# nirschl-lab/stain2stain

Hardware: AMD Instinct MI355X
Metric: paired 256x256 stain tiles/sec (full CFM optimisation step) (higher is better)
Workload: dtype bf16

## Files before the change

include/stain2stain_hip.h:

```cpp
#ifndef STAIN2STAIN_HIP_H
#define STAIN2STAIN_HIP_H

#ifdef __cplusplus
extern "C" {
#endif

#define S2S_OK 0
#define S2S_ERR_SHAPE (-1)
#define S2S_ERR_ALIGN (-2)
#define S2S_ERR_DTYPE (-3)
#define S2S_ERR_LAUNCH (-4)
#define S2S_ERR_NULL (-5)

#define S2S_BF16 0
#define S2S_F32 1

int s2s_conv3x3_stat_blocks(int dtype, int B, int H, int W, int Cout);
int s2s_conv3x3_nhwc(int dtype, const void* x0, int ld0, int c0, const void* x1, int ld1, int c1,
                     const void* w_packed, const float* bias, void* y, int ldy, float* stat_part,
                     const float* ep_scale, const float* ep_shift, int relu, int B, int H, int W, int Cout,
                     void* stream);

int s2s_conv3x3_ksplit(int dtype, int B, int H, int W, int Cout, int cin);
int s2s_conv3x3_nhwc_k(int dtype, const void* x0, int ld0, int c0, const void* x1, int ld1, int c1,
                       const void* w_packed, const float* bias, void* y, int ldy, float* stat_part,
                       const float* ep_scale, const float* ep_shift, int relu, float* kwork, int B, int H, int W,
                       int Cout, void* stream);
int s2s_conv3x3_stat_rows(int dtype, int B, int H, int W, int Cout, int c0, int c1, int ld0, int ld1, int has_bias);
int s2s_conv3x3_staged(int dtype, int B, int H, int W, int Cout, int c0, int c1, int ld0, int ld1, int ldy, int stats);
int s2s_conv3x3_family(int dtype, int B, int H, int W, int Cout, int c0, int c1, int ld0, int ld1, int ldy, int has_bias,
                       int has_affine, int stats, int stat_rows, int kwork);
int s2s_conv3x3_plan(int dtype, int B, int H, int W, int Cout, int c0, int c1, int ld0, int ld1, int ldy, int has_bias,
                     int has_affine, int stats, int stat_rows, int kwork, int* out);
int s2s_conv3x3_nhwc_s(int dtype, const void* x0, int ld0, int c0, const void* x1, int ld1, int c1, const void* w_packed,
                       const float* bias, void* y, int ldy, float* stat_part, int stat_rows, const float* ep_scale,
                       const float* ep_shift, int relu, float* kwork, int B, int H, int W, int Cout, void* stream);
int s2s_debug_conv_clock(long* out_host, int n);

int s2s_conv3x3_wgrad_splits(int dtype, int B, int H, int W, int Cin, int Cout);
int s2s_conv3x3_wgrad_plan(int dtype, int B, int H, int W, int Cin, int Cout, int what);
int s2s_conv3x3_wgrad_nhwc(int dtype, const void* dy, int lddy, int Cout, const void* x0, int ld0, int c0,
                           const void* x1, int ld1, int c1, float* part, float* grad_oihw, int accumulate,
                           int B, int H, int W, void* stream);
int s2s_conv3x3_wgrad_phase(int dtype, const void* dy, int lddy, int Cout, const void* x0, int ld0, int c0,
                            const void* x1, int ld1, int c1, float* part, float* grad_oihw, int accumulate,
                            int B, int H, int W, int phases, void* stream);
int s2s_conv3x3_wgrad_phase_variant(int dtype, const void* dy, int lddy, int Cout, const void* x0, int ld0, int c0,
                                    const void* x1, int ld1, int c1, float* part, float* grad_oihw, int accumulate,
                                    int B, int H, int W, int phases, int variant, void* stream);

int s2s_stem_stat_blocks(int B, int H, int W);
int s2s_stem_conv3x3_fwd(int dtype, const float* x_nchw, const float* w_oihw, const float* bias, void* y, int ldy,
                         float* stat_part, int B, int H, int W, int Cin, int Cout, void* stream);
int s2s_stem_wgrad_blocks(int B, int H, int W);
int s2s_stem_conv3x3_wgrad(int dtype, const void* dy, int lddy, const float* x_nchw, float* part, float* dw_oihw,
                           float* dbias, int accumulate, int B, int H, int W, int Cin, int Cout, void* stream);
int s2s_stem_conv3x3_wgrad_ref(int dtype, const void* dy, int lddy, const float* x_nchw, float* part, float* dw_oihw,
                               float* dbias, int accumulate, int B, int H, int W, int Cin, int Cout, void* stream);
int s2s_stem_wgrad_family(int dtype, int lddy, int B, int H, int W, int Cin, int Cout, int reference);
int s2s_head_family(int dtype, int B, int H, int W, int C, int Cout, int forward);
int s2s_head_conv1x1_fwd(int dtype, const void* x, int ldx, const float* w, const float* bias, float* y_nchw, int B,
                         int H, int W, int C, int Cout, void* stream);
int s2s_head_wgrad_blocks(int B, int H, int W);
int s2s_head_conv1x1_bwd(int dtype, const float* dy_nchw, const void* x, int ldx, const float* w, void* dx, int lddx,
                         float* part, float* dw, float* dbias, int accumulate, int B, int H, int W, int C, int Cout,
                         void* stream);

int s2s_head_loss_blocks(int B, int H, int W);
int s2s_head_loss_family(int dtype, int B, int H, int W, int C, int Cout);
int s2s_head_loss_fused(int dtype, const void* x, int ldx, const float* w, const float* bias, const float* u_nchw,
                        float* v_nchw, void* dx, int lddx, float grad_scale, float* part, double* lpart, float* dw,
                        float* dbias, float* loss, int accumulate, int B, int H, int W, int C, int Cout, void* stream);

int s2s_tail_blocks(int B, int H, int W);
int s2s_tail_family(int dtype, int B, int H, int W, int C, int Cout);
int s2s_tail_fwd_loss(int dtype, const void* raw, int ldx, const float* scale, const float* shift, const float* mean,
                      const float* invstd, const float* w, const float* bias, const float* u_nchw, float* v_nchw,
                      float* g_nchw, float grad_scale, float* part, double* lpart, float* bnwork, float* dw,
                      float* dbias, float* loss, float* dgamma, float* dbeta, float* conv_dbias, int accumulate, int B,
                      int H, int W, int C, int Cout, void* stream);
int s2s_tail_bwd_apply(int dtype, const void* raw, int ldx, const float* g_nchw, const float* w, const float* scale,
                       const float* shift, const float* mean, const float* invstd, const float* gamma,
                       const float* bnwork, void* dx, int lddx, int B, int H, int W, int C, int Cout, void* stream);

int s2s_bn_finalize(const float* part, int nblk, int C, long count, const float* gamma, const float* beta,
                    float* running_mean, float* running_var, long* num_batches_tracked, float momentum, float eps,
                    float* mean, float* invstd, float* scale, float* shift, void* stream);
int s2s_bn_finalize_b(const float* part, int nblk, int C, long count, const float* gamma, const float* beta,
                      float* running_mean, float* running_var, long* num_batches_tracked, float momentum, float eps,
                      float* mean, float* invstd, float* scale, float* shift, const float* conv_bias, void* stream);
int s2s_bn_eval_prepare(int C, const float* gamma, const float* beta, const float* running_mean,
                        const float* running_var, float eps, float* scale, float* shift, void* stream);
int s2s_bn_relu_apply(int dtype, const void* x, int ldx, const float* scale, const float* shift, void* y, int ldy,
                      void* pool, int ldp, int B, int H, int W, int C, void* stream);
int s2s_maxpool2(int dtype, const void* x, int ldx, void* pool, int ldp, int B, int H, int W, int C, void* stream);
int s2s_bn_bwd_blocks(int B, int H, int W, int C);
int s2s_bn_relu_bwd(int dtype, const void* g1, int ldg1, const void* gp, int ldgp, const float* scale,
                    const float* shift, const void* x, int ldx, const float* mean, const float* invstd, const float* gamma, float* dgamma,
                    float* dbeta, float* dbias_conv, int accumulate, void* dx, int lddx, float* work, int B, int H,
                    int W, int C, void* stream);
int s2s_bn_partial_sums(const float* part, int nblk, int C, float* sums, void* stream);
int s2s_bn_relu_bwd_phase(int dtype, const void* g1, int ldg1, const void* gp, int ldgp, const float* scale,
                          const float* shift, const void* x, int ldx, const float* mean, const float* invstd,
                          const float* gamma, float* dgamma, float* dbeta, float* dbias_conv, int accumulate, void* dx,
                          int lddx, float* work, int B, int H, int W, int C, long count_total, int phases, void* stream);

int s2s_upsample2x_bilinear_ac_fwd(int dtype, const void* x, int ldx, const float* bias_nc, void* y, int ldy, int B,
                                   int Hin, int Win, int Hout, int Wout, int C, void* stream);
int s2s_upsample2x_bn_relu_fwd(int dtype, const void* x, int ldx, const float* scale, const float* shift,
                               const float* bias_nc, void* y, int ldy, int B, int Hin, int Win, int Hout, int Wout, int C,
                               void* stream);
int s2s_upsample2x_bilinear_ac_fwd_ref(int dtype, const void* x, int ldx, const float* bias_nc, void* y, int ldy, int B,
                                       int Hin, int Win, int Hout, int Wout, int C, void* stream);
int s2s_upsample2x_fwd_family(int ldx, int ldy, int B, int Hin, int Win, int Hout, int Wout, int C, int reference);
int s2s_upsample2x_bilinear_ac_bwd(int dtype, const void* dy, int lddy, void* dx, int lddx, int B, int Hin, int Win,
                                   int Hout, int Wout, int C, void* stream);
int s2s_upsample2x_bilinear_ac_bwd_ref(int dtype, const void* dy, int lddy, void* dx, int lddx, int B, int Hin,
                                       int Win, int Hout, int Wout, int C, void* stream);
int s2s_upsample2x_bwd_family(int lddy, int lddx, int B, int Hin, int Win, int Hout, int Wout, int C, int reference);
int s2s_pixel_sum(int dtype, const void* x, int ldx, float* out_nc, int B, int HW, int C, int accumulate,
                  void* stream);

int s2s_time_embedding(const float* t, float* out, int B, int dim, void* stream);
int s2s_linear_fwd(const float* x, const float* w, const float* bias, float* y, int B, int K, int N, void* stream);
int s2s_linear_bwd(const float* dy, const float* x, const float* w, float* dx, float* dw, float* db, int accumulate,
                   int B, int K, int N, void* stream);
int s2s_silu_fwd(const float* h, float* a, int n, void* stream);
int s2s_silu_bwd(const float* h, const float* da, float* dh, int n, void* stream);
int s2s_cfm_sample(const float* x0, const float* x1, const float* t, const float* eps, float sigma, float* xt,
                   float* ut, int B, long per_sample, void* stream);
int s2s_mse_loss(const float* v, const float* u, float* dv, float grad_scale, float* loss, double* work, long count,
                 void* stream);
int s2s_ode_error_norm(const float* e, const float* y0, const float* y1, float atol, float rtol, float* out,
                       double* work, long n, void* stream);
int s2s_axpy(float* x, const float* y, float a, long n, void* stream);
int s2s_dp_partials(long n);
int s2s_dp_init(int phase, const float* y, const float* k1, const float* fa, double* state, double* part, float* out,
                float* t_out, int* status, float atol, float rtol, int B, long n, void* stream);
int s2s_dp_stage(int i, const float* y, const float* k1, const float* k2, const float* k3, const float* k4,
                 const float* k5, const float* k6, const double* state, float* out, float* t_out, int B, long n,
                 void* stream);
int s2s_dp_error(const float* k1, const float* k2, const float* k3, const float* k4, const float* k5, const float* k6,
                 const float* k7, const float* y, const float* y_new, const double* state, double* part, float atol,
                 float rtol, int B, long n, void* stream);
int s2s_dp_control(double* state, const double* part, int* status, int max_steps, int B, long n, void* stream);
int s2s_dp_commit(float* y, const float* y_new, float* k1, const float* k7, const double* state, int B, long n,
                  void* stream);
int s2s_rk_stage(const float* x, const float* k1, const float* k2, const float* k3, float c1, float c2, float c3, int nk,
                 float* out, float* t_out, const float* table, const int* counter, int stages, int stage, int table_len,
                 int B, long n, void* stream);
int s2s_rk_combine(float* x, const float* k1, const float* k2, const float* k3, const float* k4, float c1, float c2,
                   float c3, float c4, int nk, int* counter, int B, long n, void* stream);
int s2s_fill_f32(float* x, float v, long n, void* stream);
int s2s_euler_tick(float* t, int n, const float* table, int* counter, void* stream);

int s2s_adam_step(float* p, const float* g, float* m, float* v, long n, int step, float lr, float beta1, float beta2,
                  float eps, float weight_decay, float grad_scale, void* stream);
int s2s_adam_step_dev(float* p, const float* g, float* m, float* v, long n, const float* hyper, void* stream);
long s2s_adam_multi_blocks(long n);
int s2s_adam_multi(const void* desc, int ntensors, long total, int step, float lr, float beta1, float beta2, float eps,
                   float weight_decay, float grad_scale, void* stream);
int s2s_adam_ema_step(float* p, const float* g, float* m, float* v, float* ema, long n, int step, float lr, float beta1,
                      float beta2, float eps, float weight_decay, float grad_scale, float ema_weight, void* stream);
int s2s_adam_ema_step_dev(float* p, const float* g, float* m, float* v, float* ema, long n, const float* hyper,
                          const float* ema_weight, void* stream);
long s2s_ema_multi_blocks(long n);
int s2s_ema_multi(const void* desc, int ntensors, long total, const float* weight, void* stream);
long s2s_pack_conv3x3_fwd_elems(int Cout, int Cin);
long s2s_pack_conv3x3_dgrad_elems(int Cout, int Cin);
int s2s_pack_conv3x3(int dtype, const float* w_oihw, void* w_fwd, void* w_dgrad, int Cout, int Cin, void* stream);
int s2s_pack_conv3x3_batched(int dtype, const void* desc, int nlayers, long total, void* stream);
int s2s_nchw_to_nhwc(int dtype, const float* x_nchw, void* y, int ldy, int B, int C, int H, int W, void* stream);
int s2s_nhwc_to_nchw(int dtype, const void* x, int ldx, float* y_nchw, int accumulate, int B, int C, int H, int W,
                     void* stream);

int s2s_paired_crop_flip_normalize(const void* src_u8, const void* tgt_u8, const int* params, float* out_src,
                                   float* out_tgt, int B, int Hs, int Ws, int S, void* stream);
int s2s_pil_resize_bilinear_normalize(const void* src_u8, void* tmp_u8, const int* bounds_h, const int* kk_h,
                                      int ksize_h, const int* bounds_v, const int* kk_v, int ksize_v, void* out_u8,
                                      float* out_f, int B, int Hs, int Ws, int Ho, int Wo, void* stream);

int s2s_region_gather(const void* img_u8, long pitch, int H, int W, int band_top, int band_h, const int* origins,
                      float* out, int B, int T, void* stream);
int s2s_region_blend(const float* tiles, int c0, const float* tiles1, int c1, const int* origins, int n, int T,
                     int overlap, float* acc, int band_rows, int H, int W, int r0, int r1, void* stream);
int s2s_region_finalize(float* acc, int band_rows, int W, int C, int r0, int r1, void* out_u8, long pitch_u8,
                        float* out_f, long pitch_f, int out_top, void* stream);

// ... 318 lines not shown
```

stain2stain_amd/csrc/conv3x3_mfma.hip:

```cpp
#include "common.h"
#include <stdlib.h>
#include <type_traits>
#include <utility>

#ifdef S2S_ABLATE
#define S2S_ABL(cond) (cond)
#define S2S_DBG_MASK (~0)
#else
#define S2S_ABL(cond) false
#define S2S_DBG_MASK 64
#endif

struct Conv3x3Args {
  const void* x0;
  const void* x1;
  const void* w;
  const float* bias;
  void* y;
  float* stat_part;
  const float* ep_scale;
  const float* ep_shift;
  int ld0, c0, ld1, c1, ldy;
  int B, H, W, Cout, tilesY, tilesX, nchunk;
  int relu;
  int act;
  float act_slope;
  void* y2;
  int ldy2;
  float* kpart;
  int ksplit;
  int lgc;
  int lgh, lgw;
  int bias_mod;
  int xsp, xsn;
  long stat_rows;
  long stat_rows_req;
  int dbg;
};

namespace {

template <int... Is, typename F>
__device__ __forceinline__ void static_for_impl(std::integer_sequence<int, Is...>, F&& f) {
  (f(std::integral_constant<int, Is>{}), ...);
}
template <int N, typename F>
__device__ __forceinline__ void static_for(F&& f) {
  static_for_impl(std::make_integer_sequence<int, N>{}, f);
}

constexpr int ROWB = 80;
constexpr int STEM_HALO_BYTES = 3 * 18 * 18 * 4;

template <typename T> struct Piece;
template <> struct Piece<float> {
  f32x4 a, b;
  __device__ __forceinline__ void zero() {
#pragma unroll
    for (int i = 0; i < 4; ++i) { a[i] = 0.f; b[i] = 0.f; }
  }
  __device__ __forceinline__ void load(const float* p) {
    a = *reinterpret_cast<const f32x4*>(p);
    b = *reinterpret_cast<const f32x4*>(p + 4);
  }
  __device__ __forceinline__ void to_lds(char* hi, int img_stride, int off) const {
    bf16x8 h, m, l;
#pragma unroll
    for (int i = 0; i < 8; ++i) {
      const float x = i < 4 ? a[i] : b[i - 4];
      h[i] = (bf16_t)x;
      const float r1 = x - (float)h[i];
      m[i] = (bf16_t)r1;
      l[i] = (bf16_t)(r1 - (float)m[i]);
    }
    *reinterpret_cast<bf16x8*>(hi + off) = h;
    *reinterpret_cast<bf16x8*>(hi + img_stride + off) = m;
    *reinterpret_cast<bf16x8*>(hi + 2 * img_stride + off) = l;
  }
};

template <typename T, int TH, int TW, int BN, int WM, int WN, int LDS_MAIN>
__device__ __forceinline__ void conv_epilogue(const Conv3x3Args& a, f32x16 (&acc)[(TH * TW / WM) / 32][(BN / WN) / 32],
                                              char* smem, int img, int y0, int x0p, int n0) {
  constexpr bool SPLIT = std::is_same<T, float>::value;
  constexpr int BM = TH * TW, WTM = BM / WM, WTN = BN / WN, MI = WTM / 32, NI = WTN / 32;
  T* __restrict__ yout = static_cast<T*>(a.y);
  const int tid = threadIdx.x, lane = tid & 63, wave = tid >> 6;
  const int wm = wave / WN, wn = wave % WN;
  const int r = lane & 31, h = lane >> 5;
  constexpr int RS = BN * (int)sizeof(T) + (SPLIT ? 16 : 64);
  constexpr int EP = (BM * RS + WM * 2 * BN * 4 <= LDS_MAIN) ? 1 : ((BM / 2) * RS + WM * 2 * BN * 4 <= LDS_MAIN ? 2 : 4);
  static_assert(WM % EP == 0 || EP == 1, "epilogue passes split the wave rows");
  constexpr int PM = BM / EP;
  char* const otile = smem;
  float* const red = reinterpret_cast<float*>(smem + PM * RS);
  const bool want_stats = a.stat_part != nullptr;
  float s1[NI], s2[NI];
#pragma unroll
  for (int ni = 0; ni < NI; ++ni) { s1[ni] = 0.f; s2[ni] = 0.f; }
#pragma unroll
  for (int ep = 0; ep < EP; ++ep) {
    if (ep > 0) __syncthreads();
    if (wm / (WM / EP) == ep || EP == 1) {
#pragma unroll
      for (int ni = 0; ni < NI; ++ni) {
        const int nl = wn * WTN + ni * 32 + r;
        const int n = n0 + nl;
        const bool nok = n < a.Cout;
        const float bias = (nok && a.bias) ? a.bias[n % a.bias_mod] : 0.f;
        const float esc = (nok && a.ep_scale) ? a.ep_scale[n] : 1.f;
        const float esh = (nok && a.ep_shift) ? a.ep_shift[n] : 0.f;
#pragma unroll
        for (int mi = 0; mi < MI; ++mi) {
          float v[16];
#pragma unroll
          for (int j = 0; j < 16; ++j) {
            const int row = (j & 3) + 8 * (j >> 2) + 4 * h;
            const int m = wm * WTM + mi * 32 + row;
            const int py = m / TW, px = m - py * TW;
// ... 434 lines not shown
  constexpr int BM = TH * TW, WTM = BM / WM, WTN = BN / WN, MI = WTM / 16, NI = WTN / 16;
  static_assert(NI % 2 == 0, "channel blocks are exchanged in pairs");
  T* __restrict__ yout = static_cast<T*>(a.y);
  const int lane = tid & 63, wave = tid >> 6;
  const int wm = wave / WN, wn = wave % WN;
  const int cl = lane & 15, q = lane >> 4;
  float esc[NI][4], esh[NI][4];
#pragma unroll
  for (int ni = 0; ni < NI; ++ni)
#pragma unroll
    for (int j = 0; j < 4; ++j) {
      const int n = n0 + wn * WTN + ni * 16 + 4 * q + j;
      const bool nok = n < a.Cout;
      esc[ni][j] = (AFFINE && nok) ? a.ep_scale[n] : 1.f;
      esh[ni][j] = (AFFINE && nok) ? a.ep_shift[n] : 0.f;
    }
  const int nlane = n0 + wn * WTN + (q & 1) * 16 + (q >> 1) * 8;
  float s1l[STATS ? NI / 2 : 1][8], s2l[STATS ? NI / 2 : 1][8];
  float (*const s1)[8] = CARRY ? cs1 : s1l;
  float (*const s2)[8] = CARRY ? cs2 : s2l;
  if constexpr (STATS && !CARRY) {
#pragma unroll
    for (int pr = 0; pr < NI / 2; ++pr)
#pragma unroll
      for (int k = 0; k < 8; ++k) { s1[pr][k] = 0.f; s2[pr][k] = 0.f; }
  }
#pragma unroll
  for (int mi = 0; mi < MI; ++mi) {
    const int m = wm * WTM + mi * 16 + cl;
    const int py = m / TW, px = m - py * TW;
    const int gy = y0 + py, gx = x0p + px;
    const bool pok = gy < a.H && gx < a.W;
    const long opix = ((long)img * om.OH + gy * om.os + om.oy) * om.OW + gx * om.os + om.ox;
#pragma unroll
    for (int ni = 0; ni < NI; ni += 2) {
      unsigned w[2][2];
#pragma unroll
      for (int b = 0; b < 2; ++b) {
        bf16x4 pk;
#pragma unroll
        for (int j = 0; j < 4; ++j) {
          float t = acc[mi][ni + b][j] + bias[ni + b][j];
          if (AFFINE) {
            t = t * esc[ni + b][j] + esh[ni + b][j];
            if (a.relu) t = fmaxf(t, 0.f);
          } else if (a.act) {
            t = t > 0.f ? t : a.act_slope * t;
          }
          pk[j] = (bf16_t)t;
        }
        const uint2 u = __builtin_bit_cast(uint2, pk);
        w[b][0] = u.x; w[b][1] = u.y;
      }
      const auto r0 = __builtin_amdgcn_permlane16_swap(w[0][0], w[1][0], false, false);
      const auto r1 = __builtin_amdgcn_permlane16_swap(w[0][1], w[1][1], false, false);
      const uint4 out = make_uint4(r0[0], r1[0], r0[1], r1[1]);
      const int n = nlane + ni * 16;
      if constexpr (STATS) {
        if (pok && n < a.Cout) {
          const bf16x8 val = __builtin_bit_cast(bf16x8, out);
#pragma unroll
          for (int k = 0; k < 8; ++k) {
            const float t = (float)val[k];
            s1[ni / 2][k] += t;
            s2[ni / 2][k] = fmaf(t, t, s2[ni / 2][k]);
          }
        }
      }
      if (pok && n < a.Cout) {
        if (!S2S_ABL(a.dbg & 8)) *reinterpret_cast<uint4*>(yout + opix * a.ldy + n) = out;
        if (a.y2) {
          const bf16x8 val = __builtin_bit_cast(bf16x8, out);
          bf16x8 r8;
#pragma unroll
          for (int k = 0; k < 8; ++k) r8[k] = (float)val[k] > 0.f ? val[k] : (bf16_t)0.f;
          *reinterpret_cast<bf16x8*>(static_cast<T*>(a.y2) + opix * a.ldy2 + n) = r8;
        }
      }
    }
  }
  if constexpr (STATS && !CARRY) conv_stats_flush<BN, WN>(a, s1, s2, n0, tid, stat_row);
}

__device__ long g_clk[8192 * 4];
template <int TH, int TW, int BN, int WM, int WN, int NS>
__global__ __launch_bounds__(256, 2) void conv3x3_dma16_kernel(Conv3x3Args a) {
  long c0_ = 0, w0_ = 0;
  if ((a.dbg & 64) && threadIdx.x == 0) { c0_ = __builtin_readcyclecounter(); w0_ = wall_clock64(); }
  using T = bf16_t;
  constexpr int HP = TW + 4, HH_ = TH + 2, ROWS = HH_ * HP;
  constexpr int NGA = (ROWS + 15) / 16, HG = (NGA + 3) / 4;
  constexpr int A_BYTES = HG * 4 * 1024;
  constexpr int BG = BN / 64;
  constexpr int B_BYTES = BN * 64;
  constexpr int BM = TH * TW, WTM = BM / WM, WTN = BN / WN, MI = WTM / 16, NI = WTN / 16;
  constexpr int RB = TW / 16;
  static_assert(WM * WN == 4 && BN % 64 == 0 && NS >= 3 && NS <= 8 && TW % 16 == 0 && WTM % TW == 0, "configuration");

  extern __shared__ __attribute__((aligned(16))) char smem[];
  char* const ldsA = smem;
  char* const ldsB = smem + 2 * A_BYTES;

  const T* __restrict__ x0 = static_cast<const T*>(a.x0);
  const T* __restrict__ x1 = static_cast<const T*>(a.x1);
  const char* __restrict__ wp = static_cast<const char*>(a.w);

  const int tid = threadIdx.x, lane = tid & 63;
  const int wave = __builtin_amdgcn_readfirstlane(tid >> 6);
  const int wm = wave / WN, wn = wave % WN;
  const int cl = lane & 15, kp = lane >> 4;

  int bt = blockIdx.x, by = blockIdx.y;
  if (a.xsp) {
    const unsigned L = blockIdx.x + gridDim.x * blockIdx.y;
    const unsigned xcd = L & 7, k = L >> 3;
    const unsigned xp = xcd % (unsigned)a.xsp, xn = xcd / (unsigned)a.xsp;
    const unsigned P = gridDim.x / (unsigned)a.xsp, Nn = gridDim.y / (unsigned)a.xsn;
    const unsigned kp_ = k / Nn, kn_ = k - kp_ * Nn;
    bt = (int)(xp * P + kp_); by = (int)(xn * Nn + kn_);
  }
  const int tile_id = bt;
  const int tx = bt % a.tilesX; bt /= a.tilesX;
  const int ty = bt % a.tilesY;
  const int img = bt / a.tilesY;
  const int y0 = ty * TH, x0p = tx * TW;
  const int n0 = by * BN;
  const int ctot = a.c0 + a.c1;
  const int c_lo = (int)(((long)blockIdx.z * a.nchunk) / gridDim.z), c_hi = (int)(((long)(blockIdx.z + 1) * a.nchunk) / gridDim.z);

  const int drow = lane >> 2, dslot = lane & 3;
  auto akey = [](int col) { return ((col >> 2) & 1) << 1; };
  int apix[HG], apc[HG];
#pragma unroll
  for (int j = 0; j < HG; ++j) {
    const int row = (wave + 4 * j) * 16 + drow;
    const int hy = row / HP, hx = row - hy * HP;
    const int gy = y0 - 1 + hy, gx = x0p - 1 + hx;
    apix[j] = (row < ROWS && hx < TW + 2 && gy >= 0 && gy < a.H && gx >= 0 && gx < a.W)
                  ? (img * a.H + gy) * a.W + gx : -1;
    apc[j] = (dslot ^ akey(hx)) * 8;
  }
  const char* wptr[BG];
  int wstep[BG];
#pragma unroll
  for (int j = 0; j < BG; ++j) {
    const int n = (wave + 4 * j) * 16 + drow;
    const bool ok = n0 + n < a.Cout;
    wptr[j] = ok ? wp + (long)c_lo * 9 * a.Cout * 64 + ((long)(n0 + n) * 32 + ((dslot ^ ((-(n >> 2)) & 3)) * 8)) * 2 : g_zero_page;
    wstep[j] = ok ? a.Cout * 64 : 0;
  }
  auto dma_halo = [&](int c) {
    char* dst = ldsA + (c & 1) * A_BYTES + wave * 1024;
#pragma unroll
    for (int j = 0; j < HG; ++j) {
      const int ch = c * 32 + apc[j];
      const void* g = g_zero_page;
      if (apix[j] >= 0) {
        if (ch < a.c0) g = x0 + (long)apix[j] * a.ld0 + ch;
        else if (ch < ctot) g = x1 + (long)apix[j] * a.ld1 + (ch - a.c0);
      }
      dma16(g, dst + j * 4096);
    }
  };
  auto dma_w = [&](int slot) {
    char* dst = ldsB + slot * B_BYTES + wave * 1024;
#pragma unroll
    for (int j = 0; j < BG; ++j) {
      dma16(wptr[j], dst + j * 4096);
      wptr[j] += wstep[j];
    }
  };

  int aofs[RB][3];
#pragma unroll
  for (int rb = 0; rb < RB; ++rb)
#pragma unroll
    for (int kw = 0; kw < 3; ++kw) {
      const int px = rb * 16 + cl + kw;
      aofs[rb][kw] = ((wm * (WTM / TW)) * HP + px) * 64 + ((kp ^ akey(px)) << 4);
    }
  const int nrow = wn * WTN + cl;
  const int bofs = nrow * 64 + ((kp ^ ((-(nrow >> 2)) & 3)) << 4);

  f32x4 acc[MI][NI];
#pragma unroll
  for (int mi = 0; mi < MI; ++mi)
#pragma unroll
    for (int ni = 0; ni < NI; ++ni)
#pragma unroll
      for (int j = 0; j < 4; ++j) acc[mi][ni][j] = 0.f;

  auto compute = [&](auto tapc, const char* Ab, const char* Bb) {
    constexpr int tap = decltype(tapc)::value;
    constexpr int kh = tap / 3, kw = tap % 3;
    bf16x8 af[MI], bfr[NI];
#pragma unroll
    for (int mi = 0; mi < MI; ++mi)
      af[mi] = *reinterpret_cast<const bf16x8*>(Ab + aofs[mi % RB][kw] + (kh + mi / RB) * HP * 64);
#pragma unroll
    for (int ni = 0; ni < NI; ++ni) bfr[ni] = *reinterpret_cast<const bf16x8*>(Bb + bofs + ni * 1024);
#pragma unroll
    for (int mi = 0; mi < MI; ++mi)
#pragma unroll
      for (int ni = 0; ni < NI; ++ni)
        acc[mi][ni] = __builtin_amdgcn_mfma_f32_16x16x32_bf16(bfr[ni], af[mi], acc[mi][ni], 0, 0, 0);
  };
  dma_halo(c_lo);
  static_for<NS - 1>([&](auto k) { dma_w(decltype(k)::value); });
  wait_vm<0>();
  __builtin_amdgcn_s_barrier();

  int c = c_lo;
  for (; c + 1 < c_hi; ++c) {
    const char* Ab = ldsA + (c & 1) * A_BYTES;
    const int it0 = (c - c_lo) * 9;
    static_for<9>([&](auto tapc) {
      constexpr int tap = decltype(tapc)::value;
      if (tap == 0) { if (!S2S_ABL(a.dbg & 4)) dma_halo(c + 1); else { static_for<HG>([&](auto) { dma16(g_zero_page, ldsA + ((c + 1) & 1) * A_BYTES + wave * 1024); }); } }
      if (!S2S_ABL(a.dbg & 1)) dma_w((it0 + tap + NS - 1) % NS);
      else if (!S2S_ABL(a.dbg & 512)) { static_for<BG>([&](auto) { dma16(g_zero_page, ldsB + wave * 1024); }); }
      if (!S2S_ABL(a.dbg & 2)) compute(tapc, Ab, ldsB + ((it0 + tap) % NS) * B_BYTES);
      __builtin_amdgcn_sched_barrier(0);
      if (!S2S_ABL(a.dbg & 256)) wait_vm<(NS - 2) * BG + (tap <= NS - 3 ? HG : 0)>();
      if (!S2S_ABL(a.dbg & 32)) __builtin_amdgcn_s_barrier();
#ifdef S2S_ABLATE
      if ((a.dbg & 1024) && tap == 8) {
        char* nb = ldsA + ((c + 1) & 1) * A_BYTES;
        const float sc = 1.0f + a.act_slope, sh = a.act_slope, fl = a.act_slope - 3.0e38f;
#pragma unroll
        for (int j = 0; j < HG; ++j) {
          bf16x8* p8 = reinterpret_cast<bf16x8*>(nb + (tid + 256 * j) * 16);
          bf16x8 v = *p8;
#pragma unroll
          for (int k = 0; k < 8; ++k) v[k] = (bf16_t)fmaxf(fmaf((float)v[k], sc, sh), fl);
          *p8 = v;
        }
        asm volatile("s_waitcnt lgkmcnt(0)" ::: "memory");
        __builtin_amdgcn_s_barrier();
      }
#endif
    });
  }
  float biasr[NI][4];
#pragma unroll
  for (int ni = 0; ni < NI; ++ni)
#pragma unroll
    for (int j = 0; j < 4; ++j) {
      const int n = n0 + wn * WTN + ni * 16 + 4 * kp + j;
      biasr[ni][j] = (a.bias && n < a.Cout) ? a.bias[n] : 0.f;
    }
  {
    const char* Ab = ldsA + (c & 1) * A_BYTES;
    const int it0 = (c - c_lo) * 9;
    static_for<9>([&](auto tapc) {
      constexpr int tap = decltype(tapc)::value;
      if (tap + NS - 1 < 9) dma_w((it0 + tap + NS - 1) % NS);
      compute(tapc, Ab, ldsB + ((it0 + tap) % NS) * B_BYTES);
      __builtin_amdgcn_sched_barrier(0);
      constexpr int last_issued = (tap + NS - 1 < 9) ? tap + NS - 1 : 8;
      constexpr int younger = last_issued - (tap + 1) > 0 ? last_issued - (tap + 1) : 0;
      wait_vm<younger * BG>();
      __builtin_amdgcn_s_barrier();
    });
  }
  if (S2S_ABL(a.dbg & 16)) return;
  if (a.kpart) {
    float* const kpz = a.kpart + (long)blockIdx.z * ((long)a.B * a.H * a.W) * a.Cout;
#pragma unroll
    for (int mi = 0; mi < MI; ++mi) {
      const int m = wm * WTM + mi * 16 + cl;
      const int py = m / TW, px = m - py * TW;
      const int gy = y0 + py, gx = x0p + px;
      if (gy < a.H && gx < a.W) {
        float* const row = kpz + (((long)img * a.H + gy) * a.W + gx) * a.Cout;
#pragma unroll
        for (int ni = 0; ni < NI; ++ni) {
          const int n = n0 + wn * WTN + ni * 16 + 4 * kp;
          if (n < a.Cout) *reinterpret_cast<f32x4*>(row + n) = acc[mi][ni];
        }
      }
    }
    return;
  }
  const OutMap om{1, 0, 0, a.H, a.W};
  if (a.stat_part) conv_epilogue16_direct<TH, TW, BN, WM, WN, false, true>(a, acc, biasr, img, y0, x0p, n0, tid, om, (long)tile_id * WM + wm);
  else if (a.ep_scale) conv_epilogue16_direct<TH, TW, BN, WM, WN, true>(a, acc, biasr, img, y0, x0p, n0, tid, om);
  else conv_epilogue16_direct<TH, TW, BN, WM, WN, false>(a, acc, biasr, img, y0, x0p, n0, tid, om);
  if ((a.dbg & 64) && threadIdx.x == 0 && blockIdx.y == 0 && blockIdx.x < 8192) { g_clk[blockIdx.x * 4 + 0] = c0_; g_clk[blockIdx.x * 4 + 1] = __builtin_readcyclecounter(); g_clk[blockIdx.x * 4 + 2] = w0_; g_clk[blockIdx.x * 4 + 3] = wall_clock64(); }
}

template <int TH, int TW, int BN, int WM, int WN, int NS, int STATS>
__global__ __launch_bounds__(256, 2) void conv3x3_pers16_kernel(Conv3x3Args a, int ntiles, int GX, int GY) {
  using T = bf16_t;
  constexpr int HP = TW + 4, HH_ = TH + 2, ROWS = HH_ * HP;
  constexpr int NGA = (ROWS + 15) / 16, HG = (NGA + 3) / 4;
  constexpr int A_BYTES = HG * 4 * 1024;
  constexpr int BG = BN / 64;
  constexpr int B_BYTES = BN * 64;
  constexpr int BM = TH * TW, WTM = BM / WM, WTN = BN / WN, MI = WTM / 16, NI = WTN / 16;
  constexpr int RB = TW / 16;
  constexpr int NST = MI * (NI / 2) + (STATS == 1 ? (NI / 2) * 16 : 0);
  static_assert((NS - 2) * BG + HG + NST <= 63, "vmcnt is a 6-bit counter");
  static_assert(WM * WN == 4 && BN % 64 == 0 && NS == 4 && TW % 16 == 0 && WTM % TW == 0, "configuration");

  extern __shared__ __attribute__((aligned(16))) char smem[];
  char* const ldsA = smem;
  char* const ldsB = smem + 2 * A_BYTES;
  const T* __restrict__ x0 = static_cast<const T*>(a.x0);
  const T* __restrict__ x1 = static_cast<const T*>(a.x1);
  const char* __restrict__ wp = static_cast<const char*>(a.w);

  const int tid = threadIdx.x, lane = tid & 63;
  const int wave = __builtin_amdgcn_readfirstlane(tid >> 6);
  const int wm = wave / WN, wn = wave % WN;
  const int cl = lane & 15, kp = lane >> 4;
  const int ctot = a.c0 + a.c1;
  const int drow = lane >> 2, dslot = lane & 3;

  int ageo[HG];
#pragma unroll
  for (int j = 0; j < HG; ++j) {
    const int row = (wave + 4 * j) * 16 + drow;
    const int hy = row / HP, hx = row - hy * HP;
    ageo[j] = (((row < ROWS && hx < TW + 2) ? hy : 0x4000) << 16) | (hx << 8) | ((dslot ^ (((hx >> 2) & 1) << 1)) * 8);
  }
  int aofs[RB][3];
#pragma unroll
  for (int rb = 0; rb < RB; ++rb)
#pragma unroll
    for (int kw = 0; kw < 3; ++kw) {
      const int px = rb * 16 + cl + kw;
      aofs[rb][kw] = ((wm * (WTM / TW)) * HP + px) * 64 + ((kp ^ (((px >> 2) & 1) << 1)) << 4);
    }
  const int nrow = wn * WTN + cl;
  const int bofs = nrow * 64 + ((kp ^ ((-(nrow >> 2)) & 3)) << 4);
  int wrow_off[BG];
#pragma unroll
  for (int j = 0; j < BG; ++j) {
    const int n = (wave + 4 * j) * 16 + drow;
    wrow_off[j] = (n * 32 + ((dslot ^ ((-(n >> 2)) & 3)) * 8)) * 2;
  }

  struct Tile { int img, y0, x0p, n0, id; };
  auto locate = [&](int L) {
    int bt, by;
    if (a.xsp) {
      const unsigned xcd = (unsigned)L & 7u, k = (unsigned)L >> 3;
      const unsigned xp = xcd % (unsigned)a.xsp, xn = xcd / (unsigned)a.xsp;
// ... 71 lines not shown
  };

  const int G = gridDim.x;
  int L = blockIdx.x;
  Tile cur = locate(L);
  bool has_next = L + G < ntiles;
  Tile nxt = cur;
  if (has_next) nxt = locate(L + G);
  int apix_cur[HG];
  halo_pix(cur, true, apix_cur);
  wq_start(cur.n0, true);
  dma_halo(apix_cur, 0, 0);
  static_for<NS - 1>([&](auto k) { dma_w(decltype(k)::value); });
  wait_vm<0>();
  __builtin_amdgcn_s_barrier();

  int gc = 0;
  auto chunk = [&](auto firstc, int c) {
    constexpr bool FIRST = decltype(firstc)::value;
    const char* Ab = ldsA + (gc & 1) * A_BYTES;
    const int it0 = gc * 9;
    const bool last = c + 1 == a.nchunk;
    static_for<9>([&](auto tapc) {
      constexpr int tap = decltype(tapc)::value;
      if (tap == 0) {
        if (!last) dma_halo(apix_cur, c + 1, (gc + 1) & 1);
        else {
          int apix_nxt[HG];
          halo_pix(nxt, has_next, apix_nxt);
          dma_halo(apix_nxt, 0, (gc + 1) & 1);
        }
      }
      if (tap == 9 - (NS - 1) && last) wq_start(nxt.n0, has_next);
      dma_w((it0 + tap + NS - 1) % NS);
      compute(tapc, Ab, ldsB + ((it0 + tap) % NS) * B_BYTES);
      __builtin_amdgcn_sched_barrier(0);
      wait_vm<(NS - 2) * BG + (tap <= NS - 3 ? HG : 0) + ((FIRST && tap <= 1) ? NST : 0)>();
      __builtin_amdgcn_s_barrier();
    });
    ++gc;
  };
  float cs1[STATS == 2 ? NI / 2 : 1][8], cs2[STATS == 2 ? NI / 2 : 1][8];
  if constexpr (STATS == 2) {
#pragma unroll
    for (int pr = 0; pr < NI / 2; ++pr)
#pragma unroll
      for (int k = 0; k < 8; ++k) { cs1[pr][k] = 0.f; cs2[pr][k] = 0.f; }
  }
  for (;;) {
    __builtin_amdgcn_sched_barrier(0);
#pragma unroll
    for (int mi = 0; mi < MI; ++mi)
#pragma unroll
      for (int ni = 0; ni < NI; ++ni)
#pragma unroll
        for (int j = 0; j < 4; ++j) acc[mi][ni][j] = 0.f;
    __builtin_amdgcn_sched_barrier(0);
    chunk(std::true_type{}, 0);
    for (int c = 1; c < a.nchunk; ++c) chunk(std::false_type{}, c);
    {
      const OutMap om{1, 0, 0, a.H, a.W};
      const float nobias[NI][4] = {};
      if constexpr (STATS == 2)
        conv_epilogue16_direct<TH, TW, BN, WM, WN, false, true, true>(a, acc, nobias, cur.img, cur.y0, cur.x0p, cur.n0, tid, om, -1, cs1, cs2);
      else
        conv_epilogue16_direct<TH, TW, BN, WM, WN, false, STATS == 1>(a, acc, nobias, cur.img, cur.y0, cur.x0p, cur.n0, tid, om, (long)cur.id * WM + wm);
      if (!(cur.y0 + TH <= a.H && cur.x0p + TW <= a.W && cur.n0 + BN <= a.Cout)) wait_vm<0>();
    }
    if (!has_next) break;
    L += G;
    cur = nxt;
    halo_pix(cur, true, apix_cur);
    has_next = L + G < ntiles;
    if (has_next) nxt = locate(L + G);
  }
  if constexpr (STATS == 2) conv_stats_flush<BN, WN>(a, cs1, cs2, cur.n0, tid, (long)blockIdx.x * WM + wm);
}

struct TileCfg { int th, tw, bn, wm; bool pers; };
constexpr TileCfg kBf16Cfg[8] = {{8, 32, 128, 2, false}, {8, 32, 64, 4, true}, {4, 32, 128, 2, true}, {4, 32, 64, 2, true},
                                 {16, 16, 128, 2, false}, {16, 16, 64, 4, true}, {8, 16, 128, 2, true}, {8, 16, 64, 2, true}};
constexpr TileCfg kF32Cfg[2] = {{4, 32, 64, 2, false}, {8, 16, 64, 2, false}};
constexpr int kMinBlocks = 448;

inline long cfg_blocks(const TileCfg& c, int B, int H, int W, int Cout) {
  return (long)B * cdiv(H, c.th) * cdiv(W, c.tw) * cdiv(Cout, c.bn);
}

int select_cfg(int dtype, int B, int H, int W, int Cout) {
  if (dtype == S2S_F32) return W <= 16 ? 1 : 0;
  const int first = W <= 16 ? 4 : 0;
  int best = -1;
  long best_blocks = -1;
  for (int i = first; i < first + 4; ++i) {
    const TileCfg& c = kBf16Cfg[i];
    if (c.bn == 128 && (Cout <= 64 || (Cout % 128 != 0 && Cout % 128 <= 64 && Cout < 512))) continue;
    const long nb = cfg_blocks(c, B, H, W, Cout);
    if (nb >= kMinBlocks) return i;
    if (nb > best_blocks) { best_blocks = nb; best = i; }
  }
  return best;
}

enum Conv3x3Family {
  kStageResident,
  kStageStream,
  kPersCarry,
  kPers,
  kTap,
  kSplitF32,
};
struct Conv3x3Plan {
  int rc;
  int family;
  int cfg;
  int gx, gy;
  int grid;
  int xsp, xsn;
  int ksplit;
  long stat_rows;
};

template <int ID>
int launch_pers16(Conv3x3Args& a, const Conv3x3Plan& p, hipStream_t s) {
  constexpr TileCfg c = kBf16Cfg[ID];
  constexpr int TH = c.th, TW = c.tw, BN = c.bn, WM = c.wm, WN = 4 / WM, NS = 4;
  constexpr int ROWS = (TH + 2) * (TW + 4);
  constexpr int HG = ((ROWS + 15) / 16 + 3) / 4;
  constexpr int lds = 2 * HG * 4 * 1024 + NS * BN * 64;
  static_assert(lds <= 80 * 1024, "two workgroups per CU");
  a.tilesY = cdiv(a.H, TH);
  a.tilesX = cdiv(a.W, TW);
  auto kern_s = conv3x3_pers16_kernel<TH, TW, BN, WM, WN, NS, 1>;
  auto kern_c = conv3x3_pers16_kernel<TH, TW, BN, WM, WN, NS, 2>;
  auto kern_d = conv3x3_pers16_kernel<TH, TW, BN, WM, WN, NS, 0>;
  static unsigned long long attr_s = 0, attr_c = 0, attr_d = 0;
  if (int rc = s2s_allow_dyn_lds(reinterpret_cast<const void*>(kern_s), lds, &attr_s)) return rc;
  if (int rc = s2s_allow_dyn_lds(reinterpret_cast<const void*>(kern_c), lds, &attr_c)) return rc;
  if (int rc = s2s_allow_dyn_lds(reinterpret_cast<const void*>(kern_d), lds, &attr_d)) return rc;
  auto kern = p.family == kPersCarry ? kern_c : a.stat_part ? kern_s : kern_d;
  hipLaunchKernelGGL(kern, dim3(p.grid), dim3(256), lds, s, a, p.gx * p.gy, p.gx, p.gy);
  S2S_LAUNCH_CHECK();
  return S2S_OK;
}

template <int STATS, bool DEFER_EP, bool RESIDENT, bool AFFINE = false>
__global__ __launch_bounds__(512, 1) void conv3x3_stage_kernel(Conv3x3Args a, int njobs, int GX, int GY) {
  using T = bf16_t;
  constexpr int TH = 16, TW = 32, BN = 64, WM = 8, WN = 1;
  constexpr int HP = TW + 4, ROWS = (TH + 2) * HP;
  constexpr int NGA = (ROWS + 15) / 16, HG = (NGA + WM - 1) / WM;
  constexpr int A_BYTES = NGA * 1024;
  constexpr int B_BYTES = BN * 64, NGB = 9 * 4, BGW = (NGB + WM - 1) / WM;
  constexpr int STAGE = A_BYTES + 9 * B_BYTES;
  constexpr int WTM = TH * TW / WM, MI = WTM / 16, NI = BN / 16, RB = TW / 16;
  constexpr int NST = MI * (NI / 2);
  static_assert(NST <= 8, "one deferred store unit per tap");

  extern __shared__ __attribute__((aligned(16))) char smem[];
  const T* __restrict__ x0 = static_cast<const T*>(a.x0);
  const T* __restrict__ x1 = static_cast<const T*>(a.x1);
  const char* __restrict__ wp = static_cast<const char*>(a.w);

  const int tid = threadIdx.x, lane = tid & 63;
  const int wave = __builtin_amdgcn_readfirstlane(tid >> 6);
  const int wm = wave;
  const int cl = lane & 15, kp = lane >> 4;
  const int drow = lane >> 2, dslot = lane & 3;
  const int ctot = a.c0 + a.c1;

  int ageo[HG];
#pragma unroll
  for (int j = 0; j < HG; ++j) {
    const int row = (wave + WM * j) * 16 + drow;
    const int hy = row / HP, hx = row - hy * HP;
    ageo[j] = (((row < ROWS && hx < TW + 2) ? hy : 0x4000) << 16) | (hx << 8) | ((dslot ^ (((hx >> 2) & 1) << 1)) * 8);
  }
  int aofs[RB][3];
#pragma unroll
  for (int rb = 0; rb < RB; ++rb)
#pragma unroll
    for (int kw = 0; kw < 3; ++kw) {
      const int px = rb * 16 + cl + kw;
      aofs[rb][kw] = ((wm * (WTM / TW)) * HP + px) * 64 + ((kp ^ (((px >> 2) & 1) << 1)) << 4);
    }
  int bofs = cl * 64 + ((kp ^ ((-(cl >> 2)) & 3)) << 4);

  struct Tile { int img, y0, x0p, n0; };
  auto locate = [&](int L) {
    int bt, by;
    if (a.xsp) {
      const unsigned xcd = (unsigned)L & 7u, k = (unsigned)L >> 3, P = (unsigned)GX >> 3;
      if constexpr (RESIDENT) { by = (int)(k / P); bt = (int)(xcd * P + (k - (unsigned)by * P)); }
      else { const unsigned kq = k / (unsigned)GY; by = (int)(k - kq * (unsigned)GY); bt = (int)(xcd * P + kq); }
    } else if constexpr (RESIDENT) {
      by = L / GX; bt = L - by * GX;
    } else {
      bt = L / GY; by = L - bt * GY;
    }
    Tile t;
    const int tx = bt % a.tilesX; bt /= a.tilesX;
    const int ty = bt % a.tilesY;
    t.img = bt / a.tilesY;
    t.y0 = ty * TH; t.x0p = tx * TW; t.n0 = by * BN;
    return t;
  };
  constexpr unsigned OOB = 0xffffff00u;
  const __amdgpu_buffer_rsrc_t rs_w = __builtin_amdgcn_make_buffer_rsrc(const_cast<char*>(wp), 0, (int)((long)a.nchunk * 9 * a.Cout * 64), 0x00020000);
  const __amdgpu_buffer_rsrc_t rs_x0 = __builtin_amdgcn_make_buffer_rsrc(const_cast<T*>(x0), 0, (int)((((long)a.B * a.H * a.W - 1) * a.ld0 + a.c0) * 2), 0x00020000);
  const __amdgpu_buffer_rsrc_t rs_x1 = __builtin_amdgcn_make_buffer_rsrc(const_cast<T*>(a.c1 ? x1 : x0), 0, a.c1 ? (int)((((long)a.B * a.H * a.W - 1) * a.ld1 + a.c1) * 2) : 0, 0x00020000);
  const int wrow = (wave & 3) * 16 + drow;
  const unsigned wsw = (unsigned)wrow * 64u + (unsigned)((dslot ^ ((-(wrow >> 2)) & 3)) << 4);
  auto dma_weights = [&](int n0, int c, int st) {
    char* dst = smem + st * STAGE + A_BYTES + wave * 1024;
    const unsigned voff = n0 + wrow < a.Cout ? wsw : OOB;
#pragma unroll
    for (int j = 0; j < BGW; ++j) {
      if (wave + WM * j >= NGB || S2S_ABL(a.dbg & 1)) continue;
      const int tap = (wave >> 2) + (WM / 4) * j;
      __builtin_amdgcn_raw_ptr_buffer_load_lds(rs_w, (lds_void_t*)(dst + j * (WM * 1024)), 16, voff,
                                               ((c * 9 + tap) * a.Cout + n0) * 64, 0, 0);
    }
  };
  auto halo_pix = [&](const Tile& t, int (&apix)[HG]) {
#pragma unroll
    for (int j = 0; j < HG; ++j) {
      const int gy = t.y0 - 1 + (ageo[j] >> 16), gx = t.x0p - 1 + ((ageo[j] >> 8) & 0xff);
      apix[j] = (gy >= 0 && gy < a.H && gx >= 0 && gx < a.W) ? (t.img * a.H + gy) * a.W + gx : -1;
    }
  };
  auto dma_halo = [&](const int (&apix)[HG], int c, int st) {
    char* dst = smem + st * STAGE + wave * 1024;
    const bool second = c * 32 >= a.c0;
    const int ld2 = (second ? a.ld1 : a.ld0) * 2, ch0 = c * 32 - (second ? a.c0 : 0);
    const int left = ctot - c * 32;
#pragma unroll
    for (int j = 0; j < HG; ++j) {
      if (wave + WM * j >= NGA || S2S_ABL(a.dbg & 4)) continue;
      const int pc = ageo[j] & 0xff;
      const unsigned voff = (apix[j] >= 0 && pc < left) ? (unsigned)apix[j] * (unsigned)ld2 + (unsigned)(pc * 2) : OOB;
      if (second) __builtin_amdgcn_raw_ptr_buffer_load_lds(rs_x1, (lds_void_t*)(dst + j * (WM * 1024)), 16, voff, ch0 * 2, 0, 0);
      else __builtin_amdgcn_raw_ptr_buffer_load_lds(rs_x0, (lds_void_t*)(dst + j * (WM * 1024)), 16, voff, ch0 * 2, 0, 0);
    }
  };

  f32x4 acc[MI][NI];
  auto afrag = [&](auto tapc, int mi) {
    constexpr int tap = decltype(tapc)::value;
    constexpr int kh = tap / 3, kw = tap % 3;
    return *reinterpret_cast<const bf16x8*>(smem + aofs[mi % RB][kw] + (kh + mi / RB) * HP * 64);
  };
  auto bfrag = [&](auto tapc, int ni) {
    constexpr int tap = decltype(tapc)::value;
    return *reinterpret_cast<const bf16x8*>(smem + bofs + (A_BYTES + tap * B_BYTES + ni * 1024));
  };

  T* __restrict__ yout = static_cast<T*>(a.y);
  uint4 outv[MI][NI / 2];
  float cs1[STATS == 2 ? NI / 2 : 1][8], cs2[STATS == 2 ? NI / 2 : 1][8];
  auto stats_zero = [&]() {
    if constexpr (STATS == 2) {
#pragma unroll
      for (int pr = 0; pr < NI / 2; ++pr)
#pragma unroll
        for (int k = 0; k < 8; ++k) { cs1[pr][k] = 0.f; cs2[pr][k] = 0.f; }
    }
  };
  stats_zero();
  float esc[AFFINE ? NI : 1][4], esh[AFFINE ? NI : 1][4];
  auto load_affine = [&](int n0) {
    if constexpr (AFFINE) {
#pragma unroll
      for (int ni = 0; ni < NI; ++ni) {
        const int n = n0 + ni * 16 + 4 * kp;
        const bool ok = n < a.Cout;
        const f32x4 sc = ok ? *reinterpret_cast<const f32x4*>(a.ep_scale + n) : f32x4{1.f, 1.f, 1.f, 1.f};
        const f32x4 sh = ok ? *reinterpret_cast<const f32x4*>(a.ep_shift + n) : f32x4{0.f, 0.f, 0.f, 0.f};
        const f32x4 bi = (ok && a.bias) ? *reinterpret_cast<const f32x4*>(a.bias + n) : f32x4{0.f, 0.f, 0.f, 0.f};
#pragma unroll
        for (int j = 0; j < 4; ++j) { esc[ni][j] = sc[j]; esh[ni][j] = fmaf(bi[j], sc[j], sh[j]); }
      }
    }
  };
  auto pack = [&]() {
#pragma unroll
    for (int mi = 0; mi < MI; ++mi)
#pragma unroll
      for (int pr = 0; pr < NI / 2; ++pr) {
        unsigned w[2][2];
#pragma unroll
        for (int b = 0; b < 2; ++b) {
          bf16x4 pk;
#pragma unroll
          for (int j = 0; j < 4; ++j) {
            float t = acc[mi][2 * pr + b][j];
            if constexpr (AFFINE) {
              t = fmaf(t, esc[2 * pr + b][j], esh[2 * pr + b][j]);
              if (a.relu) t = fmaxf(t, 0.f);
            }
            pk[j] = (bf16_t)t;
          }
          const uint2 u = __builtin_bit_cast(uint2, pk);
          w[b][0] = u.x; w[b][1] = u.y;
        }
        const auto r0 = __builtin_amdgcn_permlane16_swap(w[0][0], w[1][0], false, false);
        const auto r1 = __builtin_amdgcn_permlane16_swap(w[0][1], w[1][1], false, false);
        outv[mi][pr] = make_uint4(r0[0], r1[0], r0[1], r1[1]);
      }
  };
  typedef unsigned u32x4_t __attribute__((ext_vector_type(4)));
  const __amdgpu_buffer_rsrc_t rs_y = __builtin_amdgcn_make_buffer_rsrc(yout, 0, (int)((((long)a.B * a.H * a.W - 1) * a.ldy + a.Cout) * 2), 0x00020000);
  const int nl = (kp & 1) * 16 + (kp >> 1) * 8;
  const unsigned vst = (unsigned)(cl * a.ldy + nl) * 2u;
  auto store_unit = [&](auto uc, const Tile& t) {
    constexpr int u = decltype(uc)::value, mi = u / (NI / 2), pr = u % (NI / 2);
    const int gy = t.y0 + wm * (WTM / TW) + mi / RB, gx0 = t.x0p + (mi % RB) * 16, nb = t.n0 + pr * 32;
    const bool ok = gy < a.H && gx0 + cl < a.W && nb + nl < a.Cout;
    if constexpr (STATS == 2) {
      const bf16x8 val = __builtin_bit_cast(bf16x8, outv[mi][pr]);
#pragma unroll
      for (int k = 0; k < 8; ++k) {
        const float v = ok ? (float)val[k] : 0.f;
        cs1[pr][k] += v;
        cs2[pr][k] = fmaf(v, v, cs2[pr][k]);
      }
    }
    if (!S2S_ABL(a.dbg & 8))
      __builtin_amdgcn_raw_buffer_store_b128(__builtin_bit_cast(u32x4_t, outv[mi][pr]), rs_y, ok ? vst : OOB,
                                             (((t.img * a.H + gy) * a.W + gx0) * a.ldy + nb) * 2, 0);
  };

  auto chunk = [&](auto deferc, const Tile& prv) {
    constexpr bool DEFER = decltype(deferc)::value;
    bf16x8 af[2][MI], bfr[NI];
    using T0 = std::integral_constant<int, 0>;
#pragma unroll
    for (int ni = 0; ni < NI; ++ni) bfr[ni] = bfrag(T0{}, ni);
#pragma unroll
    for (int mi = 0; mi < MI; ++mi) af[0][mi] = afrag(T0{}, mi);
    __builtin_amdgcn_sched_group_barrier(0x100, MI + NI, 0);
    static_for<9>([&](auto tapc) {
      constexpr int tap = decltype(tapc)::value, cb = tap & 1;
      using TN = std::integral_constant<int, (tap < 8 ? tap + 1 : 8)>;
#pragma unroll
      for (int ni = 0; ni < NI; ++ni) {
#pragma unroll
        for (int mi = 0; mi < MI; ++mi) {
          acc[mi][ni] = __builtin_amdgcn_mfma_f32_16x16x32_bf16(bfr[ni], af[cb][mi], acc[mi][ni], 0, 0, 0);
          if (tap < 8 && ni == 0) af[cb ^ 1][mi] = afrag(TN{}, mi);
        }
        if (tap < 8) bfr[ni] = bfrag(TN{}, ni);
      }
      if constexpr (DEFER && tap < NST) store_unit(std::integral_constant<int, (tap < NST ? tap : 0)>{}, prv);
      if constexpr (tap < 8) {
#pragma unroll
        for (int k = 0; k < MI; ++k) {
          __builtin_amdgcn_sched_group_barrier(0x008, 1, 0);
          __builtin_amdgcn_sched_group_barrier(0x100, 1, 0);
        }
        __builtin_amdgcn_sched_group_barrier(0x100, 1, 0);
#pragma unroll
        for (int k = 1; k < NI; ++k) {
          __builtin_amdgcn_sched_group_barrier(0x008, MI, 0);
          __builtin_amdgcn_sched_group_barrier(0x100, 1, 0);
        }
      }
    });
  };

  for (int i = 0, d = 3 * (int)((blockIdx.x >> 3) & 15); i < d; ++i) __builtin_amdgcn_s_sleep(8);
  const int G = gridDim.x;
  int L = blockIdx.x;
  Tile cur = locate(L);
  bool has_next = L + G < njobs;
  Tile nxt = cur, prv = cur;
  if (has_next) nxt = locate(L + G);
  int apix[HG];
  halo_pix(cur, apix);
  dma_halo(apix, 0, 0);
  dma_weights(cur.n0, 0, 0);
  if constexpr (RESIDENT) dma_weights(cur.n0, a.nchunk > 1 ? 1 : 0, 1);
  load_affine(cur.n0);
  bool pend = false, pend_full = false;
  bool ynst = false;
  int st = 0;
  unsigned long long seen = 0;

  auto step = [&](int c, auto mayc) {
    constexpr bool MAY_DEFER = decltype(mayc)::value;
    if (ynst) wait_vm<NST>(); else wait_vm<0>();
    __builtin_amdgcn_s_barrier();
    ynst = false;
    if (c + 1 < a.nchunk) {
      dma_halo(apix, c + 1, st ^ 1);
      if constexpr (!RESIDENT) dma_weights(cur.n0, c + 1, st ^ 1);
    } else if (has_next) {
      halo_pix(nxt, apix);
      dma_halo(apix, 0, st ^ 1);
      if constexpr (!RESIDENT) dma_weights(nxt.n0, 0, st ^ 1);
    }
    if (S2S_ABL(a.dbg & 2)) {
    } else if (MAY_DEFER && pend) {
      chunk(std::true_type{}, prv);
      ynst = pend_full;
      pend = false;
    } else {
      chunk(std::false_type{}, prv);
    }
    __builtin_amdgcn_sched_barrier(0);
    {
      const int d = st ? -STAGE : STAGE;
#pragma unroll
      for (int rb = 0; rb < RB; ++rb)
#pragma unroll
        for (int kw = 0; kw < 3; ++kw) aofs[rb][kw] += d;
      bofs += d;
    }
    st ^= 1;
  };
  for (;;) {
    __builtin_amdgcn_sched_barrier(0);
#pragma unroll
    for (int mi = 0; mi < MI; ++mi)
#pragma unroll
      for (int ni = 0; ni < NI; ++ni)
#pragma unroll
        for (int j = 0; j < 4; ++j) acc[mi][ni][j] = 0.f;
    __builtin_amdgcn_sched_barrier(0);
    step(0, std::integral_constant<bool, DEFER_EP>{});
    for (int c = 1; c < a.nchunk; ++c) step(c, std::false_type{});
    if (!S2S_ABL(a.dbg & 16)) {
      pack();
      prv = cur;
      const bool full = cur.y0 + TH <= a.H && cur.x0p + TW <= a.W && cur.n0 + BN <= a.Cout;
      if constexpr (DEFER_EP) {
        pend = true;
        pend_full = full;
      } else {
        static_for<NST>([&](auto uc) { store_unit(uc, prv); });
        ynst = full;
      }
    }
    if (!has_next) break;
    if (nxt.n0 != cur.n0) {
      load_affine(nxt.n0);
      if constexpr (STATS == 2) {
        conv_stats_flush<BN, WN>(a, cs1, cs2, cur.n0, tid, (long)blockIdx.x * WM + wm);
        seen |= 1ull << (cur.n0 / BN);
        stats_zero();
        ynst = false;
      }
      if constexpr (RESIDENT) {
        __builtin_amdgcn_s_barrier();
        dma_weights(nxt.n0, 0, 0);
        dma_weights(nxt.n0, a.nchunk > 1 ? 1 : 0, 1);
        ynst = false;
      }
    }
    L += G;
    cur = nxt;
    has_next = L + G < njobs;
    if (has_next) nxt = locate(L + G);
  }
  if (pend) static_for<NST>([&](auto uc) { store_unit(uc, prv); });
  if constexpr (STATS == 2) {
    conv_stats_flush<BN, WN>(a, cs1, cs2, cur.n0, tid, (long)blockIdx.x * WM + wm);
    seen |= 1ull << (cur.n0 / BN);
    stats_zero();
    for (int by = 0; by < GY; ++by) {
      if (!((seen >> by) & 1)) conv_stats_flush<BN, WN>(a, cs1, cs2, by * BN, tid, (long)blockIdx.x * WM + wm);
    }
  }
}

inline int stage_grid(const Conv3x3Args& a, bool stats, bool split) {
  static const int on = [] { const char* e = getenv("S2S_CONV_STAGE"); return e ? atoi(e) : 1; }();
  if (!on || (a.c1 && a.c0 % 32) || (a.bias && !a.ep_scale) || (a.ep_scale && stats) || split || a.act || a.y2 ||
      (a.dbg & 64)) return 0;
  if ((double)a.B * a.H * a.W * a.ld0 * 2 >= 4.0e9 || (double)a.B * a.H * a.W * (a.c1 ? a.ld1 : 0) * 2 >= 4.0e9 ||
      (double)a.B * a.H * a.W * a.ldy * 2 >= 2.0e9) return 0;
  const long GX = (long)a.B * cdiv(a.H, 16) * cdiv(a.W, 32), GY = cdiv(a.Cout, 64);
  const long njobs = GX * GY;
  constexpr int slots = 256;
  if (njobs < 2L * slots || njobs > 0x7fffffffL) return 0;
  if (a.c0 + a.c1 > 64 && GY > 1 && on < 2) return 0;
  if (stats && a.c0 + a.c1 > 64 && (GY > 32 || (32 % GY))) return 0;
  if (stats && GY > 64) return 0;
  return slots;
}

inline int launch_stage(Conv3x3Args& a, const Conv3x3Plan& p, hipStream_t s) {
  constexpr int lds = 2 * (41 * 1024 + 9 * 4096);
  static_assert(lds <= 160 * 1024, "LDS budget");
  a.tilesY = cdiv(a.H, 16);
  a.tilesX = cdiv(a.W, 32);
  const bool resident = p.family == kStageResident;
  const int form = a.stat_part ? 1 : (a.ep_scale ? 2 : 0);
  auto kern = form == 1 ? (resident ? conv3x3_stage_kernel<2, false, true> : conv3x3_stage_kernel<2, false, false>)
            : form == 2 ? (resident ? conv3x3_stage_kernel<0, false, true, true> : conv3x3_stage_kernel<0, false, false, true>)
                        : (resident ? conv3x3_stage_kernel<0, true, true> : conv3x3_stage_kernel<0, true, false>);
  static unsigned long long attr[6] = {0, 0, 0, 0, 0, 0};
  if (int rc = s2s_allow_dyn_lds(reinterpret_cast<const void*>(kern), lds, &attr[form * 2 + (resident ? 1 : 0)])) return rc;
  hipLaunchKernelGGL(kern, dim3(p.grid), dim3(512), lds, s, a, p.gx * p.gy, p.gx, p.gy);
  S2S_LAUNCH_CHECK();
  return S2S_OK;
}

template <int ID>
int launch_dma16(Conv3x3Args& a, const Conv3x3Plan& p, hipStream_t s) {
  constexpr TileCfg c = kBf16Cfg[ID];
  constexpr int TH = c.th, TW = c.tw, BN = c.bn, WM = c.wm, WN = 4 / WM, NS = 4;
  constexpr int ROWS = (TH + 2) * (TW + 4);
  constexpr int HG = ((ROWS + 15) / 16 + 3) / 4;
  constexpr int lds = 2 * HG * 4 * 1024 + NS * BN * 64;
  static_assert(lds <= 160 * 1024, "LDS budget");
  a.tilesY = cdiv(a.H, TH);
  a.tilesX = cdiv(a.W, TW);
  auto kern = conv3x3_dma16_kernel<TH, TW, BN, WM, WN, NS>;
  static unsigned long long attr_devs = 0;
  if (int rc = s2s_allow_dyn_lds(reinterpret_cast<const void*>(kern), lds, &attr_devs)) return rc;
  hipLaunchKernelGGL(kern, dim3(p.gx, p.gy, p.ksplit), dim3(256), lds, s, a);
  S2S_LAUNCH_CHECK();
  return S2S_OK;
}

template <int TH, int TW, int BN, int WM, int WN, int NS, int KS, int PAD, int MODE = 0, bool SPARSE = false>
__global__ __launch_bounds__(256, 2) void convkxk_dma16_kernel(Conv3x3Args a) {
  static_assert(MODE == 0 || KS == 2, "the fused layouts exist for the 2x2-tap forms");
  using T = bf16_t;
  constexpr int TAPS = KS * KS;
  static_assert(KS >= 2 && KS <= 5, "the halo row has four spare columns");
  constexpr int HP = TW + 4, HH_ = TH + KS - 1, ROWS = HH_ * HP;
  constexpr int NGA = (ROWS + 15) / 16, HG = (NGA + 3) / 4;
  constexpr int A_BYTES = HG * 4 * 1024;
  constexpr int BG = BN / 64;
  constexpr int B_BYTES = BN * 64;
  constexpr int BM = TH * TW, WTM = BM / WM, WTN = BN / WN, MI = WTM / 16, NI = WTN / 16;
  constexpr int RB = TW / 16;
  static_assert(WM * WN == 4 && BN % 64 == 0 && NS == 4 && TW % 16 == 0 && WTM % TW == 0, "configuration");

  extern __shared__ __attribute__((aligned(16))) char smem[];
  char* const ldsA = smem;
  char* const ldsB = smem + 2 * A_BYTES;
  const T* __restrict__ x0 = static_cast<const T*>(a.x0);
  const char* __restrict__ wp = static_cast<const char*>(a.w);

  const int tid = threadIdx.x, lane = tid & 63;
  const int wave = __builtin_amdgcn_readfirstlane(tid >> 6);
  const int wm = wave / WN, wn = wave % WN;
  const int cl = lane & 15, kp = lane >> 4;
  int bt = blockIdx.x;
  const int tx = bt % a.tilesX; bt /= a.tilesX;
  const int ty = bt % a.tilesY;
  const int img = bt / a.tilesY;
  const int y0 = ty * TH, x0p = tx * TW;
  const int n0 = blockIdx.y * BN;
  const int phase = MODE == 2 ? (int)blockIdx.z / a.ksplit : 0, zk = (int)blockIdx.z - phase * a.ksplit;
  const int pad_y = MODE == 2 ? (phase >> 1) : PAD, pad_x = MODE == 2 ? (phase & 1) : PAD;
  const int Hi = MODE == 2 ? a.H : a.H + KS - 1 - 2 * PAD, Wi = MODE == 2 ? a.W : a.W + KS - 1 - 2 * PAD;
  const int c_lo = (int)(((long)zk * a.nchunk) / a.ksplit), c_hi = (int)(((long)(zk + 1) * a.nchunk) / a.ksplit);
  const int wrows = MODE == 2 ? 4 * a.Cout : a.Cout, wrow0 = (MODE == 2 ? phase * a.Cout : 0) + n0;

  const int drow = lane >> 2, dslot = lane & 3;
  int apix[HG], apc[HG];
#pragma unroll
  for (int j = 0; j < HG; ++j) {
    const int row = (wave + 4 * j) * 16 + drow;
    const int hy = row / HP, hx = row - hy * HP;
    const int gy = y0 - pad_y + hy, gx = x0p - pad_x + hx;
    const bool inside = row < ROWS && hx < TW + KS - 1 && gy >= 0 && gy < Hi && gx >= 0 && gx < Wi;
    if (MODE == 1) apix[j] = inside ? ((gy << 16) | gx) : -1;
    else apix[j] = inside ? (img * Hi + gy) * Wi + gx : -1;
    apc[j] = (dslot ^ (((hx >> 2) & 1) << 1)) * 8;
  }
  const char* wptr[BG];
  int wstep[BG];
#pragma unroll
  for (int j = 0; j < BG; ++j) {
    const int n = (wave + 4 * j) * 16 + drow;
    const bool ok = n0 + n < a.Cout;
    wptr[j] = ok ? wp + (long)c_lo * TAPS * wrows * 64 + ((long)(wrow0 + n) * 32 + ((dslot ^ ((-(n >> 2)) & 3)) * 8)) * 2 : g_zero_page;
    wstep[j] = ok ? wrows * 64 : 0;
  }
  auto dma_halo = [&](int c) {
    char* dst = ldsA + (c & 1) * A_BYTES + wave * 1024;
#pragma unroll
    for (int j = 0; j < HG; ++j) {
      const int ch = c * 32 + apc[j];
      const void* g = g_zero_page;
      if (MODE == 1) {
        if (apix[j] >= 0 && ch < a.c0) {
          const int rs = ch >> a.lgc, cc = ch & ((1 << a.lgc) - 1);
          const int py = 2 * (apix[j] >> 16) + (rs >> 1) - 1, px = 2 * (apix[j] & 0xffff) + (rs & 1) - 1;
          if ((unsigned)py < (unsigned)(2 * a.H) && (unsigned)px < (unsigned)(2 * a.W))
            g = x0 + ((long)(img * 2 * a.H + py) * (2 * a.W) + px) * a.ld0 + cc;
        }
      } else if (apix[j] >= 0 && ch < a.c0) {
        g = x0 + (long)apix[j] * a.ld0 + ch;
      }
      dma16(g, dst + j * 4096);
// ... 463 lines not shown
        if constexpr (SPLIT) {
          acc[mi][ni] = __builtin_amdgcn_mfma_f32_32x32x16_bf16(af[1][mi], bfr[1][ni], acc[mi][ni], 0, 0, 0);
          acc[mi][ni] = __builtin_amdgcn_mfma_f32_32x32x16_bf16(af[2][mi], bfr[0][ni], acc[mi][ni], 0, 0, 0);
          acc[mi][ni] = __builtin_amdgcn_mfma_f32_32x32x16_bf16(af[0][mi], bfr[2][ni], acc[mi][ni], 0, 0, 0);
          acc[mi][ni] = __builtin_amdgcn_mfma_f32_32x32x16_bf16(af[1][mi], bfr[0][ni], acc[mi][ni], 0, 0, 0);
          acc[mi][ni] = __builtin_amdgcn_mfma_f32_32x32x16_bf16(af[0][mi], bfr[1][ni], acc[mi][ni], 0, 0, 0);
        }
        acc[mi][ni] = __builtin_amdgcn_mfma_f32_32x32x16_bf16(af[0][mi], bfr[0][ni], acc[mi][ni], 0, 0, 0);
      }
  }
  __syncthreads();
  }
  conv_epilogue<T, TH, TW, BN, WM, WN, LDS_MAIN>(a, acc, smem, img, y0, x0p, n0);
}

template <typename T>
int launch_stem(Conv3x3Args& a, const float* x, const float* w, int Cin, hipStream_t s) {
  constexpr bool SPLIT = std::is_same<T, float>::value;
  constexpr int NIMG = SPLIT ? 3 : 1, BN = 64;
  constexpr int lds_main = NIMG * (256 + BN) * ROWB + STEM_HALO_BYTES;
  constexpr int RS_ = BN * (int)sizeof(T) + (SPLIT ? 16 : 64);
  constexpr int red_ = 4 * 2 * BN * 4;
  constexpr int EP_ = (256 * RS_ + red_ <= lds_main) ? 1 : (128 * RS_ + red_ <= lds_main ? 2 : 4);
  constexpr int lds_epi = (256 / EP_) * RS_ + red_;
  constexpr int lds = lds_main > lds_epi ? lds_main : lds_epi;
  a.tilesY = cdiv(a.H, 16);
  a.tilesX = cdiv(a.W, 16);
  auto kern = stem_mfma_kernel<T, BN>;
  static unsigned long long attr_devs = 0;
  if (int rc = s2s_allow_dyn_lds(reinterpret_cast<const void*>(kern), lds, &attr_devs)) return rc;
  dim3 grid(a.B * a.tilesY * a.tilesX, cdiv(a.Cout, BN));
  hipLaunchKernelGGL(kern, grid, dim3(256), lds, s, a, x, w, Cin);
  S2S_LAUNCH_CHECK();
  return S2S_OK;
}

inline bool pers_eligible(const Conv3x3Args& a, int id, bool split) {
  static const int pers = [] { const char* e = getenv("S2S_CONV_PERS"); return e ? atoi(e) : 1; }();
  const TileCfg& tc = kBf16Cfg[id];
  if (!tc.pers) return false;
  const bool many = cfg_blocks(tc, a.B, a.H, a.W, a.Cout) >= (pers > 1 ? pers : 1024);
  return pers && many && !a.bias && !a.ep_scale && !split && !a.act && !a.y2 && a.nchunk >= 2 && !(a.dbg & 64) &&
         a.c0 % 32 == 0 &&
         (double)a.B * a.H * a.W * a.ld0 * 2 < 4.0e9 && (double)a.B * a.H * a.W * (a.c1 ? a.ld1 : 0) * 2 < 4.0e9;
}

inline void xcd_cut(const Conv3x3Args& a, int GX, int GY, Conv3x3Plan& p) {
  const double act = 2.0 * a.B * a.H * a.W * (a.c0 + a.c1), wb = 2.0 * 9 * (a.c0 + a.c1) * a.Cout;
  double best = 0;
  for (int sp = 8; sp >= 1; sp >>= 1) {
    const int sn = 8 / sp;
    if (GX % sp || GY % sn) continue;
    const double cost = sn * act + sp * wb;
    if (!p.xsp || cost < best) { best = cost; p.xsp = sp; p.xsn = sn; }
  }
}

inline int split_count(long tiles, int nchunk) {
  if (tiles >= 128 || nchunk < 8) return 1;
  long sp = (512 + tiles - 1) / tiles;
  if (sp > nchunk / 4) sp = nchunk / 4;
  if (sp > 16) sp = 16;
  return sp < 2 ? 1 : (int)sp;
}

constexpr long kAnyRows = -1;

Conv3x3Plan conv3x3_plan(int dtype, const Conv3x3Args& a) {
  const bool stats = a.stat_part != nullptr;
  const long req = a.stat_rows_req;
  Conv3x3Plan p{};
  p.rc = S2S_OK; p.xsn = 1; p.ksplit = 1;
  p.cfg = select_cfg(dtype, a.B, a.H, a.W, a.Cout);
  const TileCfg& c = dtype == S2S_F32 ? kF32Cfg[p.cfg] : kBf16Cfg[p.cfg];
  p.gx = a.B * cdiv(a.H, c.th) * cdiv(a.W, c.tw);
  p.gy = cdiv(a.Cout, c.bn);
  if (dtype == S2S_F32) {
    p.family = kSplitF32;
    p.stat_rows = p.gx;
    return p;
  }
  if (a.kpart && !stats) p.ksplit = split_count((long)p.gx * p.gy, a.nchunk);
  const bool split = p.ksplit > 1;
  if (const int wg = stage_grid(a, stats, split)) {
    if (!stats || req == kAnyRows || req == (long)wg * 8) {
      p.family = a.c0 + a.c1 <= 64 ? kStageResident : kStageStream;
      p.gx = a.B * cdiv(a.H, 16) * cdiv(a.W, 32);
      p.gy = cdiv(a.Cout, 64);
      p.grid = wg;
      p.xsp = p.gx % 8 == 0 ? 8 : 0;
      p.stat_rows = (long)wg * 8;
      return p;
    }
  }
  if (pers_eligible(a, p.cfg, split)) {
    const long ntiles = (long)p.gx * p.gy;
    if (ntiles % 8 == 0) xcd_cut(a, p.gx, p.gy, p);
    constexpr int slots = 512;
    int grid = (int)(ntiles < slots ? ntiles : slots);
    if (p.xsp && grid > 8) grid -= grid % 8;
    p.grid = grid < 1 ? 1 : grid;
    const bool carry = stats && p.gy == 1 && (req == kAnyRows || req == (long)p.grid * c.wm);
    p.family = carry ? kPersCarry : kPers;
    p.stat_rows = (long)(carry ? p.grid : p.gx) * c.wm;
  } else {
    static const int xcd_aware = [] { const char* e = getenv("S2S_CONV_XCD"); return e ? atoi(e) : 1; }();
    p.family = kTap;
    p.stat_rows = (long)p.gx * c.wm;
    if (xcd_aware && !split && ((long)p.gx * p.gy) % 8 == 0) xcd_cut(a, p.gx, p.gy, p);
  }
  if (stats && req > 0 && req != p.stat_rows) p.rc = S2S_ERR_SHAPE;
  return p;
}

template <int ID = 0, typename F>
int with_cfg(int id, F&& f) {
  if constexpr (ID < 8) return id == ID ? f(std::integral_constant<int, ID>{}) : with_cfg<ID + 1>(id, f);
  else return S2S_ERR_SHAPE;
}

int dispatch(int dtype, Conv3x3Args& a, hipStream_t s) {
  const Conv3x3Plan p = conv3x3_plan(dtype, a);
  if (p.rc != S2S_OK) return p.rc;
  a.xsp = p.xsp; a.xsn = p.xsn; a.ksplit = p.ksplit; a.stat_rows = p.stat_rows;
  if (p.ksplit == 1) a.kpart = nullptr;
  switch (p.family) {
    case kSplitF32:
      return p.cfg == 1 ? launch_cfg<float, 8, 16, 64, 2, 2>(a, s) : launch_cfg<float, 4, 32, 64, 2, 2>(a, s);
    case kStageResident:
    case kStageStream: return launch_stage(a, p, s);
    case kPersCarry:
    case kPers:
      return with_cfg(p.cfg, [&](auto id) {
        constexpr int ID = decltype(id)::value;
        if constexpr (kBf16Cfg[ID].pers) return launch_pers16<ID>(a, p, s);
        else return S2S_ERR_SHAPE;
      });
    default: return with_cfg(p.cfg, [&](auto id) { return launch_dma16<decltype(id)::value>(a, p, s); });
  }
}

}

int s2s_internal_stem_fwd(int dtype, const float* x_nchw, const float* w_oihw, const float* bias, void* y, int ldy,
                          float* stat_part, int B, int H, int W, int Cin, int Cout, hipStream_t s) {
  Conv3x3Args a{};
  a.x0 = a.x1 = a.w = nullptr; a.bias = bias; a.y = y; a.stat_part = stat_part;
  a.ep_scale = a.ep_shift = nullptr; a.act = 0; a.act_slope = 0.f; a.y2 = nullptr; a.ldy2 = 8; a.bias_mod = Cout;
  a.ld0 = a.c0 = a.ld1 = a.c1 = 0; a.ldy = ldy;
  a.B = B; a.H = H; a.W = W; a.Cout = Cout; a.nchunk = 1; a.relu = 0; a.dbg = 0;
  a.tilesX = a.tilesY = 0;
  if (dtype == S2S_BF16) return launch_stem<bf16_t>(a, x_nchw, w_oihw, Cin, s);
  if (dtype == S2S_F32) return launch_stem<float>(a, x_nchw, w_oihw, Cin, s);
  return S2S_ERR_DTYPE;
}

extern "C" int s2s_debug_conv_clock(long* out, int n) {
  if (!out) return S2S_ERR_NULL;
  if (n <= 0 || n > 8192) return S2S_ERR_SHAPE;
  return hipMemcpyFromSymbol(out, HIP_SYMBOL(g_clk), (size_t)n * 4 * sizeof(long)) == hipSuccess ? S2S_OK
                                                                                                  : S2S_ERR_LAUNCH;
}

static void conv3x3_fill_args(Conv3x3Args& a, int ld0, int c0, int ld1, int c1, const float* bias, int B, int H, int W,
                              int Cout) {
  a.bias = bias;
  a.act = 0; a.act_slope = 0.f; a.y2 = nullptr; a.ldy2 = 8; a.bias_mod = Cout; a.kpart = nullptr; a.ksplit = 1; a.lgc = 0; a.lgh = a.lgw = 0;
  a.ld0 = ld0; a.c0 = c0; a.ld1 = ld1; a.c1 = c1;
  a.B = B; a.H = H; a.W = W; a.Cout = Cout; a.nchunk = cdiv(c0 + c1, 32);
  a.tilesX = a.tilesY = 0;
  { static const int dbg = [] { const char* e = getenv("S2S_CONV_DBG"); return (e ? atoi(e) : 0) & S2S_DBG_MASK; }(); a.dbg = dbg; }
}

static Conv3x3Plan conv3x3_query(int dtype, int B, int H, int W, int Cout, int c0, int c1, int ld0, int ld1, int ldy,
                                 bool bias, bool stats, long stat_rows_req, bool kwork) {
  static float present;
  Conv3x3Args a{};
  conv3x3_fill_args(a, ld0, c0, ld1, c1, bias ? &present : nullptr, B, H, W, Cout);
  a.ldy = ldy;
  a.stat_part = stats ? &present : nullptr;
  a.stat_rows_req = stat_rows_req;
  a.kpart = kwork ? &present : nullptr;
  return conv3x3_plan(dtype, a);
}

extern "C" int s2s_conv3x3_stat_blocks(int dtype, int B, int H, int W, int Cout) {
  if (B <= 0 || H <= 0 || W <= 0 || Cout <= 0) return S2S_ERR_SHAPE;
  if (dtype != S2S_BF16 && dtype != S2S_F32) return S2S_ERR_DTYPE;
  return (int)conv3x3_query(dtype, B, H, W, Cout, 0, 0, 0, 0, 0, false, true, 0, false).stat_rows;
}

extern "C" int s2s_conv3x3_nhwc_k(int dtype, const void* x0, int ld0, int c0, const void* x1, int ld1, int c1,
                                  const void* w_packed, const float* bias, void* y, int ldy, float* stat_part,
                                  const float* ep_scale, const float* ep_shift, int relu, float* kwork, int B, int H,
                                  int W, int Cout, void* stream);
extern "C" int s2s_conv3x3_nhwc_s(int dtype, const void* x0, int ld0, int c0, const void* x1, int ld1, int c1,
                                  const void* w_packed, const float* bias, void* y, int ldy, float* stat_part, int stat_rows,
                                  const float* ep_scale, const float* ep_shift, int relu, float* kwork, int B, int H,
                                  int W, int Cout, void* stream);

extern "C" int s2s_conv3x3_ksplit(int dtype, int B, int H, int W, int Cout, int cin) {
  if (B <= 0 || H <= 0 || W <= 0 || Cout <= 0 || cin <= 0) return S2S_ERR_SHAPE;
  if (dtype != S2S_BF16) return 1;
  return conv3x3_query(dtype, B, H, W, Cout, cin, 0, 0, 0, 0, false, false, 0, true).ksplit;
}

extern "C" int s2s_conv3x3_nhwc(int dtype, const void* x0, int ld0, int c0, const void* x1, int ld1, int c1,
                                const void* w_packed, const float* bias, void* y, int ldy, float* stat_part,
                                const float* ep_scale, const float* ep_shift, int relu, int B, int H, int W,
                                int Cout, void* stream) {
  return s2s_conv3x3_nhwc_k(dtype, x0, ld0, c0, x1, ld1, c1, w_packed, bias, y, ldy, stat_part, ep_scale, ep_shift, relu,
                            nullptr, B, H, W, Cout, stream);
}

extern "C" int s2s_conv3x3_stat_rows(int dtype, int B, int H, int W, int Cout, int c0, int c1, int ld0, int ld1,
                                     int has_bias) {
  const int tiles = s2s_conv3x3_stat_blocks(dtype, B, H, W, Cout);
  if (tiles < 0 || c0 <= 0 || c1 < 0) return tiles;
  return (int)conv3x3_query(dtype, B, H, W, Cout, c0, c1, ld0, ld1, 0, has_bias, true, kAnyRows, false).stat_rows;
}

extern "C" int s2s_conv3x3_staged(int dtype, int B, int H, int W, int Cout, int c0, int c1, int ld0, int ld1, int ldy,
                                  int stats) {
  if (B <= 0 || H <= 0 || W <= 0 || Cout <= 0 || c0 <= 0 || c1 < 0) return S2S_ERR_SHAPE;
  if (dtype != S2S_BF16) return 0;
  const int f = conv3x3_query(dtype, B, H, W, Cout, c0, c1, ld0, ld1, ldy, false, stats != 0, kAnyRows, false).family;
  return f == kStageResident ? 2 : f == kStageStream ? 1 : 0;
}

static Conv3x3Plan conv3x3_query_ep(int dtype, int B, int H, int W, int Cout, int c0, int c1, int ld0, int ld1, int ldy,
                                    int has_bias, int has_affine, int stats, int stat_rows, int kwork) {
  static float present;
  Conv3x3Args a{};
  conv3x3_fill_args(a, ld0, c0, ld1, c1, has_bias ? &present : nullptr, B, H, W, Cout);
  a.ldy = ldy;
  a.ep_scale = has_affine ? &present : nullptr;
  a.ep_shift = a.ep_scale;
  a.stat_part = stats ? &present : nullptr;
  a.stat_rows_req = stat_rows;
  a.kpart = kwork ? &present : nullptr;
  return conv3x3_plan(dtype, a);
}

extern "C" int s2s_conv3x3_family(int dtype, int B, int H, int W, int Cout, int c0, int c1, int ld0, int ld1, int ldy,
                                  int has_bias, int has_affine, int stats, int stat_rows, int kwork) {
  if (B <= 0 || H <= 0 || W <= 0 || Cout <= 0 || c0 <= 0 || c1 < 0) return S2S_ERR_SHAPE;
  if (dtype != S2S_BF16 && dtype != S2S_F32) return S2S_ERR_DTYPE;
  const Conv3x3Plan p = conv3x3_query_ep(dtype, B, H, W, Cout, c0, c1, ld0, ld1, ldy, has_bias, has_affine, stats,
                                         stat_rows, kwork);
  return p.rc != S2S_OK ? p.rc : p.family;
}

extern "C" int s2s_conv3x3_plan(int dtype, int B, int H, int W, int Cout, int c0, int c1, int ld0, int ld1, int ldy,
                                int has_bias, int has_affine, int stats, int stat_rows, int kwork, int* out) {
  if (!out) return S2S_ERR_NULL;
  if (B <= 0 || H <= 0 || W <= 0 || Cout <= 0 || c0 <= 0 || c1 < 0) return S2S_ERR_SHAPE;
  if (dtype != S2S_BF16 && dtype != S2S_F32) return S2S_ERR_DTYPE;
  const Conv3x3Plan p = conv3x3_query_ep(dtype, B, H, W, Cout, c0, c1, ld0, ld1, ldy, has_bias, has_affine, stats,
                                         stat_rows, kwork);
  if (p.rc != S2S_OK) return p.rc;
  const int v[9] = {p.family, p.cfg, p.gx, p.gy, p.grid, p.xsp, p.xsn, p.ksplit, (int)p.stat_rows};
  for (int i = 0; i < 9; ++i) out[i] = v[i];
  return S2S_OK;
}

extern "C" int s2s_conv3x3_nhwc_k(int dtype, const void* x0, int ld0, int c0, const void* x1, int ld1, int c1,
                                  const void* w_packed, const float* bias, void* y, int ldy, float* stat_part,
                                  const float* ep_scale, const float* ep_shift, int relu, float* kwork, int B, int H,
                                  int W, int Cout, void* stream) {
  return s2s_conv3x3_nhwc_s(dtype, x0, ld0, c0, x1, ld1, c1, w_packed, bias, y, ldy, stat_part, 0, ep_scale, ep_shift, relu,
                            kwork, B, H, W, Cout, stream);
}

extern "C" int s2s_conv3x3_nhwc_s(int dtype, const void* x0, int ld0, int c0, const void* x1, int ld1, int c1,
                                  const void* w_packed, const float* bias, void* y, int ldy, float* stat_part, int stat_rows,
                                  const float* ep_scale, const float* ep_shift, int relu, float* kwork, int B, int H,
                                  int W, int Cout, void* stream) {
  if (!x0 || !w_packed || !y) return S2S_ERR_NULL;
  if (B <= 0 || H <= 0 || W <= 0 || Cout <= 0 || c0 <= 0 || c1 < 0) return S2S_ERR_SHAPE;
  if ((c0 % 8) || (c1 % 8) || (ld0 % 8) || (ld1 % 8) || (c1 > 0 && !x1)) return S2S_ERR_SHAPE;
  if ((Cout % 8) || (ldy % 8) || ldy < Cout) return S2S_ERR_SHAPE;
  if ((ep_scale == nullptr) != (ep_shift == nullptr)) return S2S_ERR_NULL;
  const uintptr_t al = 15;
  if (((uintptr_t)x0 & al) || ((uintptr_t)x1 & al) || ((uintptr_t)w_packed & al) || ((uintptr_t)y & al)) return S2S_ERR_ALIGN;
  if (stat_rows < 0) return S2S_ERR_SHAPE;
  Conv3x3Args a{};
  conv3x3_fill_args(a, ld0, c0, ld1, c1, bias, B, H, W, Cout);
  a.x0 = x0; a.x1 = x1; a.w = w_packed; a.y = y; a.stat_part = stat_part; a.stat_rows_req = stat_part ? stat_rows : 0;
  a.ep_scale = ep_scale; a.ep_shift = ep_shift; a.ldy = ldy; a.relu = relu;
  hipStream_t s = static_cast<hipStream_t>(stream);
  if (dtype != S2S_BF16 && dtype != S2S_F32) return S2S_ERR_DTYPE;
  if (dtype == S2S_BF16 && relu && !ep_scale) { a.act = 1; a.act_slope = 0.f; }
  a.kpart = kwork;
  const int rc = dispatch(dtype, a, s);
  if (rc != S2S_OK || !a.kpart) return rc;
  const long npix = (long)B * H * W, pieces = npix * (Cout / 8);
  long nb = (pieces + 255) / 256;
  if (nb > 4096) nb = 4096;
  hipLaunchKernelGGL(convk_splitk_reduce_kernel<bf16_t>, dim3((unsigned)nb), dim3(256), 0, s, a, npix);
  S2S_LAUNCH_CHECK();
  return S2S_OK;
}
extern "C" int s2s_convkxk_stat_blocks(int dtype, int B, int H, int W, int Cout, int ks) {
  if (B <= 0 || H <= 0 || W <= 0 || Cout <= 0 || (ks != 2 && ks != 4)) return S2S_ERR_SHAPE;
  if (dtype == S2S_F32) return W > 16 ? B * cdiv(H, 4) * cdiv(W, 32) : B * cdiv(H, 8) * cdiv(W, 16);
  if (dtype != S2S_BF16) return S2S_ERR_DTYPE;
  if (ks == 2) return B * cdiv(H, 8) * cdiv(W, W > 16 ? 32 : 16);
  return W > 16 ? B * cdiv(H, 4) * cdiv(W, 32) : B * cdiv(H, 8) * cdiv(W, 16);
}

extern "C" int s2s_convkxk_ksplit(int dtype, int B, int H, int W, int Cout, int cin, int ks) {
  if (B <= 0 || H <= 0 || W <= 0 || Cout <= 0 || cin <= 0 || (ks != 2 && ks != 4)) return S2S_ERR_SHAPE;
  if (dtype != S2S_BF16) return 1;
  const bool wide = W > 16, big = Cout > 64;
  const int th = (ks == 4 && wide) ? 4 : 8, tw = wide ? 32 : 16, bn = big ? 128 : 64;
  const long base = (long)B * cdiv(H, th) * cdiv(W, tw) * cdiv(Cout, bn);
  const int nchunk = cdiv(cin, 32);
  const long target = Cout <= 16 ? 1024 : 512;
  if (base >= (Cout <= 16 ? 512 : 192) || nchunk < 8) return 1;
  long sp = (target + base - 1) / base;
  if (sp > nchunk / 4) sp = nchunk / 4;
  if (sp > 32) sp = 32;
  return sp < 2 ? 1 : (int)sp;
}

extern "C" int s2s_convkxk_nhwc(int dtype, const void* x, int ldx, int cin, const void* w_packed, const float* bias,
                                int bias_mod, void* y, int ldy, void* y2, int ldy2, int act, float act_slope,
                                float* stat_part, float* kwork, int B, int H, int W, int Cout, int ks, int pad,
                                void* stream) {
  if (!x || !w_packed || !y) return S2S_ERR_NULL;
  if (dtype != S2S_BF16 && dtype != S2S_F32) return S2S_ERR_DTYPE;
  if (B <= 0 || H <= 0 || W <= 0 || Cout <= 0 || cin <= 0 || (cin % 8) || (ldx % 8) || (Cout % 8) || (ldy % 8) || ldy < Cout) return S2S_ERR_SHAPE;
  if (y2 && ((ldy2 % 8) || ldy2 < Cout)) return S2S_ERR_SHAPE;
  if (bias_mod < 0 || (bias_mod > 0 && Cout % bias_mod)) return S2S_ERR_SHAPE;
  if (!((ks == 2 && (pad == 0 || pad == 1)) || (ks == 4 && (pad == 1 || pad == 2)))) return S2S_ERR_SHAPE;
  if (H + ks - 1 - 2 * pad < 1 || W + ks - 1 - 2 * pad < 1) return S2S_ERR_SHAPE;
  if (((uintptr_t)x & 15) || ((uintptr_t)w_packed & 15) || ((uintptr_t)y & 15) || ((uintptr_t)y2 & 15)) return S2S_ERR_ALIGN;
  if ((long)B * (H + 3) * (W + 3) >= (1L << 31)) return S2S_ERR_SHAPE;
  Conv3x3Args a{};
  a.x0 = x; a.x1 = nullptr; a.w = w_packed; a.bias = bias; a.y = y; a.stat_part = stat_part;
  a.ep_scale = a.ep_shift = nullptr; a.act = act ? 1 : 0; a.act_slope = act_slope; a.y2 = y2; a.ldy2 = ldy2;
  a.bias_mod = bias_mod > 0 ? bias_mod : Cout;
  a.ksplit = kwork ? s2s_convkxk_ksplit(dtype, B, H, W, Cout, cin, ks) : 1;
  a.kpart = a.ksplit > 1 ? kwork : nullptr;
  if (a.kpart && stat_part) return S2S_ERR_SHAPE;
  a.ld0 = ldx; a.c0 = cin; a.ld1 = 8; a.c1 = 0; a.ldy = ldy;
  a.B = B; a.H = H; a.W = W; a.Cout = Cout; a.nchunk = cdiv(cin, 32); a.relu = 0; a.dbg = 0;
  a.tilesX = a.tilesY = 0;
  hipStream_t s = static_cast<hipStream_t>(stream);
  const bool wide = W > 16, big = Cout > 64;
  const int form = ks * 4 + pad;
  if (dtype == S2S_F32) {
    switch (form) {
      case 8:  return wide ? launch_cfg<float, 4, 32, 64, 2, 2, 2, 0>(a, s) : launch_cfg<float, 8, 16, 64, 2, 2, 2, 0>(a, s);
      case 9:  return wide ? launch_cfg<float, 4, 32, 64, 2, 2, 2, 1>(a, s) : launch_cfg<float, 8, 16, 64, 2, 2, 2, 1>(a, s);
      case 17: return wide ? launch_cfg<float, 4, 32, 64, 2, 2, 4, 1>(a, s) : launch_cfg<float, 8, 16, 64, 2, 2, 4, 1>(a, s);
      default: return wide ? launch_cfg<float, 4, 32, 64, 2, 2, 4, 2>(a, s) : launch_cfg<float, 8, 16, 64, 2, 2, 4, 2>(a, s);
    }
  }
  int rc;
  switch (form) {
    case 8:
      if (wide) rc = big ? launch_convkxk<8, 32, 128, 2, 2, 2, 0>(a, s) : launch_convkxk<8, 32, 64, 4, 1, 2, 0>(a, s);
      else rc = big ? launch_convkxk<8, 16, 128, 2, 2, 2, 0>(a, s) : launch_convkxk<8, 16, 64, 2, 2, 2, 0>(a, s);
      break;
    case 9:
      if (wide) rc = big ? launch_convkxk<8, 32, 128, 2, 2, 2, 1>(a, s) : launch_convkxk<8, 32, 64, 4, 1, 2, 1>(a, s);
      else rc = big ? launch_convkxk<8, 16, 128, 2, 2, 2, 1>(a, s) : launch_convkxk<8, 16, 64, 2, 2, 2, 1>(a, s);
      break;
    case 17:
      if (wide) rc = big ? launch_convkxk<4, 32, 128, 2, 2, 4, 1>(a, s) : launch_convkxk<4, 32, 64, 2, 2, 4, 1>(a, s);
      else rc = big ? launch_convkxk<8, 16, 128, 2, 2, 4, 1>(a, s) : launch_convkxk<8, 16, 64, 2, 2, 4, 1>(a, s);
      break;
    default:
      if (wide) rc = big ? launch_convkxk<4, 32, 128, 2, 2, 4, 2>(a, s) : launch_convkxk<4, 32, 64, 2, 2, 4, 2>(a, s);
      else rc = big ? launch_convkxk<8, 16, 128, 2, 2, 4, 2>(a, s) : launch_convkxk<8, 16, 64, 2, 2, 4, 2>(a, s);
  }
  if (rc != S2S_OK || !a.kpart) return rc;
  const long npix = (long)B * H * W, pieces = npix * (Cout / 8);
  long nb = (pieces + 255) / 256;
  if (nb > 4096) nb = 4096;
  hipLaunchKernelGGL(convk_splitk_reduce_kernel<bf16_t>, dim3((unsigned)nb), dim3(256), 0, s, a, npix);
  S2S_LAUNCH_CHECK();
  return S2S_OK;
// ... 171 lines not shown
```

stain2stain_amd/csrc/norm_act.hip:

```cpp
#include "common.h"
#include <type_traits>

namespace {

constexpr int RED_ROWS = 8;

constexpr int PRE_R = 16;
__global__ __launch_bounds__(1024) void prereduce_rows_kernel(float* __restrict__ part, int nrows, int ncols) {
  __shared__ double s1[32][33];
  const int cl = threadIdx.x & 31, rg = threadIdx.x >> 5;
  const int c = blockIdx.x * 32 + cl, r = blockIdx.y;
  double a = 0.0;
  if (c < ncols)
    for (int i = r + PRE_R * rg; i < nrows; i += PRE_R * 32) a += (double)part[(long)i * ncols + c];
  s1[rg][cl] = a;
  __syncthreads();
  if (rg == 0 && c < ncols) {
    for (int k = 1; k < 32; ++k) a += s1[k][cl];
    part[(long)r * ncols + c] = (float)a;
  }
}

inline int prereduce(float* part, int nrows, int ncols, hipStream_t s) {
  if (nrows <= 4 * PRE_R) return nrows;
// ... 615 lines not shown
  return S2S_OK;
}

extern "C" int s2s_maxpool2(int dtype, const void* x, int ldx, void* pool, int ldp, int B, int H, int W, int C,
                            void* stream) {
  if (!x || !pool) return S2S_ERR_NULL;
  if (B <= 0 || H < 2 || W < 2 || C <= 0 || (C % 8) || (ldx % 8) || (ldp % 8)) return S2S_ERR_SHAPE;
  const long total = (long)B * (H / 2) * (W / 2) * (C / 8);
  hipStream_t s = (hipStream_t)stream;
  if (dtype == S2S_BF16)
    hipLaunchKernelGGL(maxpool2_kernel<bf16_t>, dim3(ew_grid(total)), dim3(256), 0, s, (const bf16_t*)x, ldx,
                       (bf16_t*)pool, ldp, B, H, W, C);
  else if (dtype == S2S_F32)
    hipLaunchKernelGGL(maxpool2_kernel<float>, dim3(ew_grid(total)), dim3(256), 0, s, (const float*)x, ldx,
                       (float*)pool, ldp, B, H, W, C);
  else return S2S_ERR_DTYPE;
  S2S_LAUNCH_CHECK();
  return S2S_OK;
}

extern "C" int s2s_bn_bwd_blocks(int B, int H, int W, int C) {
  if (B <= 0 || H <= 0 || W <= 0 || C <= 0) return S2S_ERR_SHAPE;
  return red_blocks(B, H, W, C);
}

extern "C" int s2s_bn_relu_bwd_phase(int dtype, const void* g1, int ldg1, const void* gp, int ldgp, const float* scale,
                               const float* shift, const void* x, int ldx, const float* mean, const float* invstd, const float* gamma,
                               float* dgamma, float* dbeta, float* dbias_conv, int accumulate, void* dx, int lddx,
                               float* work, int B, int H, int W, int C, long count_total, int phases, void* stream) {
  if (phases < 1 || phases > 3 || count_total < (long)B * H * W) return S2S_ERR_SHAPE;
  if ((!g1 && !gp) || !scale || !shift || !x || !mean || !invstd || !gamma || !dgamma || !dbeta || !dx || !work) return S2S_ERR_NULL;
  if (B <= 0 || H <= 0 || W <= 0 || C <= 0 || (C % 8) || (ldx % 8) || (lddx % 8) ||
      (g1 && (ldg1 % 8)) || (gp && (ldgp % 8)))
    return S2S_ERR_SHAPE;
  if ((long)B * ((H + 1) / 2) * ((W + 1) / 2) >= (1L << 31) - (1 << 20)) return S2S_ERR_SHAPE;
  const int nb = red_blocks(B, H, W, C);
  float* part = work;
  float* part2 = work + (long)nb * 2 * C;
  float* c1 = part2 + (long)nb * 2 * C;
  float* c2 = c1 + C;
  const double count = (double)count_total;
  hipStream_t s = (hipStream_t)stream;
  float* const dbias_zero = (dbias_conv && !accumulate) ? dbias_conv : nullptr;
  dbias_conv = nullptr;
  dim3 grid(cdiv(C / 8, host_pcb(C)), nb);
  constexpr int bn_rev = 1;
#define S2S_BN_BWD(TT)                                                                                             \
  if (!(phases & 1)) {                                                                                             \
  } else if (gp) {                                                                                                 \
    hipLaunchKernelGGL(bn_relu_bwd_reduce_kernel<TT>, grid, dim3(256), 0, s, (const TT*)g1, ldg1, (const TT*)gp,   \
                       ldgp, scale, shift, (const TT*)x, ldx, mean, invstd, part, B, H, W, C);                \
  } else {                                                                                                         \
    hipLaunchKernelGGL(bn_relu_bwd_reduce_flat_kernel<TT>, grid, dim3(256), 0, s, (const TT*)g1, ldg1,             \
                       scale, shift, (const TT*)x, ldx, mean, invstd, part, (long)B * H * W, C);              \
  }                                                                                                                \
  if (!(phases & 1)) {                                                                                             \
  } else if (finalize_tpc(nb) == 256)                                                                              \
    hipLaunchKernelGGL(bn_bwd_finalize_kernel<256>, dim3(C), dim3(256), 0, s, part, nb, C, count, dgamma, dbeta,   \
                       accumulate, c1, c2, dbias_zero);                                                            \
  else                                                                                                             \
    hipLaunchKernelGGL(bn_bwd_finalize_kernel<64>, dim3(cdiv(C, 4)), dim3(256), 0, s, part, nb, C, count, dgamma,  \
                       dbeta, accumulate, c1, c2, dbias_zero);                                                     \
  if (!(phases & 2)) {                                                                                             \
  } else if (gp) {                                                                                                 \
    hipLaunchKernelGGL(bn_relu_bwd_apply_kernel<TT>, grid, dim3(256), 0, s, (const TT*)g1, ldg1, (const TT*)gp,    \
                       ldgp, scale, shift, (const TT*)x, ldx, mean, invstd, gamma, c1, c2, (TT*)dx, lddx,     \
                       dbias_conv ? part2 : nullptr, B, H, W, C);                                                  \
  } else {                                                                                                         \
    hipLaunchKernelGGL(bn_relu_bwd_apply_flat_kernel<TT>, grid, dim3(256), 0, s, (const TT*)g1, ldg1,              \
                       scale, shift, (const TT*)x, ldx, mean, invstd, gamma, c1, c2, (TT*)dx, lddx,           \
                       dbias_conv ? part2 : nullptr, (long)B * H * W, C, bn_rev);                                  \
  }
  if (dtype == S2S_BF16) { S2S_BN_BWD(bf16_t) }
  else if (dtype == S2S_F32) { S2S_BN_BWD(float) }
  else return S2S_ERR_DTYPE;
#undef S2S_BN_BWD
  if (dbias_conv && (phases & 2))
    hipLaunchKernelGGL(colsum_finalize_kernel, dim3(cdiv(C, 32)), dim3(1024), 0, s, part2, prereduce(part2, nb, C, s),
                       C, dbias_conv, accumulate);
  S2S_LAUNCH_CHECK();
  return S2S_OK;
}

int s2s_internal_tail_bn_sums(int dtype, const void* raw, int ldx, const float* g_nchw, const float* w, const float* scale,
                              const float* shift, const float* mean, const float* invstd, float* work, float* dgamma,
                              float* dbeta, float* zero_out, int accumulate, int B, int H, int W, int C, int Cout,
                              hipStream_t s) {
  const int nb = red_blocks(B, H, W, C);
  float* const c1 = work + (long)2 * C * nb;
  const long npix = (long)B * H * W;
  dim3 grid(cdiv(C / 8, host_pcb(C)), nb);
  if (dtype == S2S_BF16)
    hipLaunchKernelGGL(bn_relu_bwd_reduce_tail_kernel<bf16_t>, grid, dim3(256), 0, s, g_nchw, w, Cout, H * W, scale, shift,
                       (const bf16_t*)raw, ldx, mean, invstd, work, npix, C);
  else if (dtype == S2S_F32)
    hipLaunchKernelGGL(bn_relu_bwd_reduce_tail_kernel<float>, grid, dim3(256), 0, s, g_nchw, w, Cout, H * W, scale, shift,
                       (const float*)raw, ldx, mean, invstd, work, npix, C);
  else return S2S_ERR_DTYPE;
  if (finalize_tpc(nb) == 256)
    hipLaunchKernelGGL(bn_bwd_finalize_kernel<256>, dim3(C), dim3(256), 0, s, work, nb, C, (double)npix, dgamma, dbeta,
                       accumulate, c1, c1 + C, zero_out);
  else
    hipLaunchKernelGGL(bn_bwd_finalize_kernel<64>, dim3(cdiv(C, 4)), dim3(256), 0, s, work, nb, C, (double)npix, dgamma,
                       dbeta, accumulate, c1, c1 + C, zero_out);
  return S2S_OK;
}

extern "C" int s2s_bn_relu_bwd(int dtype, const void* g1, int ldg1, const void* gp, int ldgp, const float* scale,
                               const float* shift, const void* x, int ldx, const float* mean, const float* invstd, const float* gamma,
                               float* dgamma, float* dbeta, float* dbias_conv, int accumulate, void* dx, int lddx,
                               float* work, int B, int H, int W, int C, void* stream) {
  return s2s_bn_relu_bwd_phase(dtype, g1, ldg1, gp, ldgp, scale, shift, x, ldx, mean, invstd, gamma, dgamma, dbeta,
                               dbias_conv, accumulate, dx, lddx, work, B, H, W, C, (long)B * H * W, 3, stream);
}
```

stain2stain_amd/engine.py:

```python
from __future__ import annotations

from dataclasses import dataclass, field
from typing import Dict, List, Optional, Sequence, Tuple

import contextlib
import threading

import torch
import torch.distributed as dist

from . import ops

BN_EPS = 1e-5
BN_MOMENTUM = 0.1


class SyncBNExchange:

    def __init__(self, process_group=None):
        if not (dist.is_available() and dist.is_initialized()):
            raise RuntimeError("stain2stain_amd: SyncBatchNorm needs an initialised torch.distributed process group")
        self.pg = process_group
        self.world = dist.get_world_size(process_group)
        self._host = dist.get_backend(process_group) != "nccl"
# ... 245 lines not shown


def _conv_bn_relu(cb: ConvBN, x0, x1, dtype, training: bool, want_pool: bool = False, stem: bool = False):
    bias = cb.conv.bias.detach() if cb.conv.bias is not None else None
    if training:
        raw, st, count, sx = _conv_bn_stats(cb, x0, x1, dtype, stem)
        act, pooled = ops.bn_relu_apply(raw, st[2], st[3], want_pool=want_pool)
        return LayerCtx(x0, x1, raw, act, st, count if sx is not None else None, sx), act, pooled
    ss = cb.eval_affine()
    if stem and _stem_as_conv(x0, dtype):
        act, _ = ops.conv3x3(_stem_image(x0, dtype), None, cb.packed(dtype)[0], bias, cb.cout, scale=ss[0], shift=ss[1], relu=True)
        pooled = ops.maxpool2(act) if want_pool else None
    elif stem:
        raw, _ = ops.stem_fwd(x0, cb.conv.weight.detach(), bias, dtype, want_stats=False)
        act, pooled = ops.bn_relu_apply(raw, ss[0], ss[1], want_pool=want_pool)
    else:
        act, _ = ops.conv3x3(x0, x1, cb.packed(dtype)[0], bias, cb.cout, scale=ss[0], shift=ss[1], relu=True)
        pooled = ops.maxpool2(act) if want_pool else None
    return None, act, pooled


def _conv_bn_lazy(cb: ConvBN, x0, x1, dtype):
    raw, st, count, sx = _conv_bn_stats(cb, x0, x1, dtype)
    return LayerCtx(x0, x1, raw, None, st, count if sx is not None else None, sx), LazyAct(raw, st[2], st[3])


def _upsample_into(x, up: torch.Tensor, tbias) -> None:
    if isinstance(x, LazyAct):
        ops.upsample2x_fwd(x.raw, up, tbias, bn_relu=(x.scale, x.shift))
    else:
        ops.upsample2x_fwd(x, up, tbias)


class _SideState(threading.local):
    stream: Optional[torch.cuda.Stream] = None
    keep: Optional[List[torch.Tensor]] = None


_side = _SideState()


@contextlib.contextmanager
def side_scope(stream: Optional[torch.cuda.Stream]):
    prev = _side.stream, _side.keep
    _side.stream, _side.keep = stream, []
    try:
        yield
    finally:
        try:
            join_side(stream)
        finally:
            _side.stream, _side.keep = prev


def current_side() -> Optional[torch.cuda.Stream]:
    return _side.stream


def run_on_side(fn, keep=()) -> None:
    side = _side.stream
    if side is None:
        fn()
        return
    ev = torch.cuda.Event()
    ev.record()
    with torch.cuda.stream(side):
        side.wait_event(ev)
        fn()
    _side.keep.extend(t for t in keep if t is not None)


def join_side(side: Optional[torch.cuda.Stream]) -> None:
    if side is not None:
        torch.cuda.current_stream().wait_stream(side)


def _g(grads: Dict[str, torch.Tensor], name: str) -> torch.Tensor:
    try:
        return grads[name]
    except KeyError as e:
        raise RuntimeError(f"stain2stain_amd: no gradient buffer for parameter {name!r}") from e


def _conv_bn_relu_bwd(cb: ConvBN, lc: LayerCtx, g1, gp, grads, accumulate: bool, need_dx: bool, stem: bool = False):
    p = cb.prefix
    i_conv, i_bn = cb.idx
    dgamma = _g(grads, f"{p}.{i_bn}.weight")
    dbeta = _g(grads, f"{p}.{i_bn}.bias")
    dbias = _g(grads, f"{p}.{i_conv}.bias") if cb.conv.bias is not None else None
    draw = ops.bn_relu_bwd(g1, gp, lc.raw, lc.stats, cb.bn.weight.detach(), dgamma, dbeta, dbias, accumulate,
                           exchange=lc.sync, count_total=lc.count)
    dw = _g(grads, f"{p}.{i_conv}.weight")
    if stem:
        run_on_side(lambda: ops.stem_wgrad(draw, lc.x0, dw, None, accumulate), (draw,))
        return None
    run_on_side(lambda: ops.conv3x3_wgrad(draw, lc.x0, lc.x1, dw, accumulate), (draw,))
    if not need_dx:
        return None
    dx, _ = ops.conv3x3(draw, None, cb.packed(draw.dtype)[1], None, cb.cin)
    return dx


def _conv_bn_tail(cb: ConvBN, x0, dtype):
    raw, st, count, sx = _conv_bn_stats(cb, x0, None, dtype)
    if sx is not None:
        act, _ = ops.bn_relu_apply(raw, st[2], st[3])
        return LayerCtx(x0, None, raw, act, st, count, sx), act
    return LayerCtx(x0, None, raw, None, st), None


def decoder_tail_loss(dec, ctx: DecCtx, u_nchw: torch.Tensor, grads: Dict[str, torch.Tensor], want_v: bool = False,
                      accumulate: bool = False):
    cb = dec.up_blocks[-1][1]
    lc = ctx.layers[-1][1]
    p = cb.prefix
    i_conv, i_bn = cb.idx
    loss, g, v, work = ops.tail_fwd_loss(
        lc.raw, lc.stats, dec.outc.weight.detach(), dec.outc.bias.detach() if dec.outc.bias is not None else None,
        u_nchw, _g(grads, "outc.weight"), _g(grads, "outc.bias") if dec.outc.bias is not None else None,
        _g(grads, f"{p}.{i_bn}.weight"), _g(grads, f"{p}.{i_bn}.bias"),
        _g(grads, f"{p}.{i_conv}.bias") if cb.conv.bias is not None else None, want_v=want_v, accumulate=accumulate)
    ctx.tail = (g, work)
    ctx.v = v
    return loss, v


def _conv_bn_tail_bwd(dec, cb: ConvBN, lc: LayerCtx, tail, grads, accumulate: bool):
    g, work = tail
    draw = ops.tail_bwd_apply(lc.raw, lc.stats, dec.outc.weight.detach(), g, cb.bn.weight.detach(), work)
    dw = _g(grads, f"{cb.prefix}.{cb.idx[0]}.weight")
    run_on_side(lambda: ops.conv3x3_wgrad(draw, lc.x0, lc.x1, dw, accumulate), (draw,))
    dx, _ = ops.conv3x3(draw, None, cb.packed(draw.dtype)[1], None, cb.cin)
    return dx


def encoder_forward(blocks: Sequence[Tuple[ConvBN, ConvBN]], x_nchw: torch.Tensor, dtype: torch.dtype,
                    training: bool, lazy_up: bool = False) -> EncCtx:
    ctx = EncCtx(dtype, x_nchw)
    nlev = len(blocks)
    repack_stale([cb for l, pair in enumerate(blocks) for j, cb in enumerate(pair)
                  if (l, j) != (0, 0) or _stem_as_conv(x_nchw, dtype)], dtype)
    inp = x_nchw
    for l, (c1, c2) in enumerate(blocks):
        lc1, a1, _ = _conv_bn_relu(c1, inp, None, dtype, training, stem=(l == 0))
        if lazy_up and training and nlev > 1 and l == nlev - 1:
            (lc2, a2), pooled = _conv_bn_lazy(c2, a1, None, dtype), None
        else:
            lc2, a2, pooled = _conv_bn_relu(c2, a1, None, dtype, training, want_pool=(l + 1 < nlev))
        ctx.layers.append((lc1, lc2))
        ctx.feats.append(a2)
        inp = pooled
    return ctx


def encoder_backward(blocks: Sequence[Tuple[ConvBN, ConvBN]], ctx: EncCtx, dfeats: Sequence[Optional[torch.Tensor]],
                     grads: Dict[str, torch.Tensor], accumulate: bool = False, on_group_done=None) -> None:
    gpool = None
    nlev = len(blocks)
    for l in range(len(blocks) - 1, -1, -1):
        c1, c2 = blocks[l]
        lc1, lc2 = ctx.layers[l]
        g1 = dfeats[l]
        if g1 is None and gpool is None:
            raise RuntimeError("stain2stain_amd: encoder level without any incoming gradient")
        ga1 = _conv_bn_relu_bwd(c2, lc2, g1, gpool, grads, accumulate, need_dx=True)
        if on_group_done is not None:
            on_group_done()
        gpool = _conv_bn_relu_bwd(c1, lc1, ga1, None, grads, accumulate, need_dx=(l > 0), stem=(l == 0))
        if on_group_done is not None:
            on_group_done()


def decoder_forward(dec, bottleneck: torch.Tensor, skips: Sequence[torch.Tensor], t_emb: torch.Tensor,
                    dtype: torch.dtype, training: bool, with_head: bool = True, fuse_tail: bool = False,
                    lazy_up: bool = False) -> DecCtx:
    fuse_tail = (fuse_tail and training and not with_head and len(dec.up_blocks) > 0
                 and ops.tail_fusable(dec.up_blocks[-1][1].cout, dec.outc.weight.shape[0]))
    ctx = DecCtx(dtype, t_emb)
    repack_stale([cb for pair in dec.up_blocks for cb in pair], dtype)
    tbias = None
    if getattr(dec, "time_mlp", None) is not None:
        l0, l2 = dec.time_mlp[0], dec.time_mlp[2]
        ctx.h1 = ops.linear_fwd(t_emb, l0.weight.detach(), l0.bias.detach())
        ctx.a1 = ops.silu_fwd(ctx.h1)
        ctx.h2 = ops.linear_fwd(ctx.a1, l2.weight.detach(), l2.bias.detach())
        tbias = ops.linear_fwd(ctx.h2, dec.time_proj.weight.detach(), dec.time_proj.bias.detach())
    x = bottleneck
    for i, ((c1, c2), skip) in enumerate(zip(dec.up_blocks, skips)):
        B, Hs, Ws, _ = skip.shape
        up = torch.empty((B, Hs, Ws, x.shape[3]), dtype=dtype, device=skip.device)
        _upsample_into(x, up, tbias if i == 0 else None)
        lc1, a1, _ = _conv_bn_relu(c1, skip, up, dtype, training)
        if fuse_tail and i == len(dec.up_blocks) - 1:
            lc2, a2 = _conv_bn_tail(c2, a1, dtype)
        elif lazy_up and training and i < len(dec.up_blocks) - 1:
            lc2, a2 = _conv_bn_lazy(c2, a1, None, dtype)
        else:
            lc2, a2, _ = _conv_bn_relu(c2, a1, None, dtype, training)
        ctx.lows.append(x); ctx.ups.append(up); ctx.skips.append(skip); ctx.layers.append((lc1, lc2))
        x = a2
    if isinstance(x, LazyAct):
        x = x.materialise()
    ctx.lows.append(x)
    if not with_head:
        return ctx
    ctx.v = ops.head_fwd(x, dec.outc.weight.detach(), dec.outc.bias.detach() if dec.outc.bias is not None else None)
    return ctx


def decoder_backward(dec, ctx: DecCtx, dv: Optional[torch.Tensor], grads: Dict[str, torch.Tensor],
                     accumulate: bool = False, need_dt_emb: bool = False, on_group_done=None,
                     g_head: Optional[torch.Tensor] = None):
    if ctx.tail is not None:
        g = None
    elif g_head is not None:
        g = g_head
    else:
        g = ops.head_bwd(dv, ctx.lows[-1], dec.outc.weight.detach(), _g(grads, "outc.weight"),
                         _g(grads, "outc.bias") if dec.outc.bias is not None else None, accumulate)
    if on_group_done is not None:
        on_group_done()
    nup = len(ctx.layers)
    dskips: List[torch.Tensor] = [None] * len(ctx.layers)
    for i in range(len(ctx.layers) - 1, -1, -1):
        c1, c2 = dec.up_blocks[i]
        lc1, lc2 = ctx.layers[i]
        if ctx.tail is not None and i == nup - 1:
            ga1 = _conv_bn_tail_bwd(dec, c2, lc2, ctx.tail, grads, accumulate)
        else:
            ga1 = _conv_bn_relu_bwd(c2, lc2, g, None, grads, accumulate, need_dx=True)
        if on_group_done is not None:
            on_group_done()
        dcat = _conv_bn_relu_bwd(c1, lc1, ga1, None, grads, accumulate, need_dx=True)
        cs = ctx.skips[i].shape[3]
        dskips[i] = dcat[..., :cs]
        low = ctx.lows[i]
        g = ops.upsample2x_bwd(dcat[..., cs:], low.shape[1], low.shape[2])
        if on_group_done is not None:
            on_group_done()
    dbott = g
    if getattr(dec, "time_mlp", None) is None:
        return dbott, dskips, None
    dtb = ops.pixel_sum(g)
    l0, l2 = dec.time_mlp[0], dec.time_mlp[2]
    dh2 = ops.linear_bwd(dtb, ctx.h2, dec.time_proj.weight.detach(), _g(grads, "time_proj.weight"),
                         _g(grads, "time_proj.bias"), True, accumulate)
    da1 = ops.linear_bwd(dh2, ctx.a1, l2.weight.detach(), _g(grads, "time_mlp.2.weight"),
                         _g(grads, "time_mlp.2.bias"), True, accumulate)
    dh1 = ops.silu_bwd(ctx.h1, da1)
    dt_emb = ops.linear_bwd(dh1, ctx.t_emb, l0.weight.detach(), _g(grads, "time_mlp.0.weight"),
                            _g(grads, "time_mlp.0.bias"), need_dt_emb, accumulate)
    if on_group_done is not None:
        on_group_done()
    return dbott, dskips, dt_emb
```

stain2stain_amd/multitask_trainer.py:

```python
from __future__ import annotations

from typing import Dict, List, Optional, Tuple

import torch
import torch.distributed as dist

from . import engine, evaluation, morphology, ops
from .components import FlowMatchingDecoder, SegmentationDecoder, SharedEncoder
from .ddp import all_reduce_mean_scalar
from .ema import TrainerEMA
from .fused_step import FlatParams


def _layer_groups(named: Dict[str, torch.nn.Parameter], prefix: str, owner: str) -> List[List[Tuple[str, torch.nn.Parameter]]]:
    out = []
    for idx in (("3.", "4."), ("0.", "1.")):
        out.append([(f"{owner}.{n}", p) for n, p in named.items() if any(n.startswith(prefix + i) for i in idx)])
    return out


def _decoder_groups(dec, owner: str) -> List[List[Tuple[str, torch.nn.Parameter]]]:
    named = dict(dec.named_parameters())
    groups = [[(f"{owner}.{n}", p) for n, p in named.items() if n.startswith("outc.")]]
    for i in range(len(dec.ups) - 1, -1, -1):
        groups += _layer_groups(named, f"ups.{i}.conv.double_conv.", owner)
    if getattr(dec, "time_mlp", None) is not None:
        groups.append([(f"{owner}.{n}", p) for n, p in named.items() if n.startswith("time_")])
    return groups


def _encoder_groups(enc, owner: str) -> List[List[Tuple[str, torch.nn.Parameter]]]:
    named = dict(enc.named_parameters())
    groups = []
    for i in range(len(enc.downs) - 1, -1, -1):
        groups += _layer_groups(named, f"downs.{i}.maxpool_conv.1.double_conv.", owner)
    return groups + _layer_groups(named, "inc.double_conv.", owner)


class MultiTaskTrainer:

    def __init__(self, encoder: SharedEncoder, flow_decoder: FlowMatchingDecoder, seg_decoder: SegmentationDecoder,
                 time_emb_dim: int = 256, lr: float = 1e-4, weight_decay: float = 1e-5,
                 betas: Tuple[float, float] = (0.9, 0.999), eps: float = 1e-8, seg_loss_weight: float = 1.0,
                 dice_weight: float = 0.5, dice_smooth: float = 1.0, num_classes: Optional[int] = None,
                 ignore_index: int = -100, sigma: float = 0.0, bucket_mb: float = 4.0, process_group=None,
                 sync_loss: bool = True, max_bucket_mb: float = 16.0, sharded_optimizer: bool = False,
                 ema_decay: Optional[float] = None, ema_buffers: bool = True):
        dev = next(encoder.parameters()).device
        if dev.type != "cuda":
            raise RuntimeError("stain2stain_amd: MultiTaskTrainer needs the networks on a GPU (HIP-only implementation)")
        if not (encoder.compute_dtype == flow_decoder.compute_dtype == seg_decoder.compute_dtype):
            raise ValueError("encoder and decoders must share one precision")
        self.encoder, self.flow_decoder, self.seg_decoder = encoder, flow_decoder, seg_decoder
        self.time_emb_dim, self.sigma = time_emb_dim, sigma
        self.lr, self.wd, self.betas, self.eps = lr, weight_decay, tuple(betas), eps
        self.seg_loss_weight, self.dice_weight, self.dice_smooth = seg_loss_weight, dice_weight, dice_smooth
        self.num_classes, self.ignore_index = num_classes, ignore_index
        self.pg, self.sync_loss = process_group, sync_loss
        self._dtype = encoder.compute_dtype
        groups = _decoder_groups(seg_decoder, "seg_decoder") + _decoder_groups(flow_decoder, "flow_decoder") \
            + _encoder_groups(encoder, "encoder")
        n_named = sum(1 for m in (encoder, flow_decoder, seg_decoder) for _ in m.parameters())
        if sum(len(g) for g in groups) != n_named or any(not g for g in groups):
            raise RuntimeError("parameter grouping does not cover the networks")
        self.fp = FlatParams(groups, bucket_mb, process_group, max_bucket_mb, sharded_optimizer)
        gr = self.fp.grads
        self.grads_enc = {k[len("encoder."):]: v for k, v in gr.items() if k.startswith("encoder.")}
        self.grads_flow = {k[len("flow_decoder."):]: v for k, v in gr.items() if k.startswith("flow_decoder.")}
        self.grads_seg = {k[len("seg_decoder."):]: v for k, v in gr.items() if k.startswith("seg_decoder.")}
        from .ddp import broadcast_from_rank0
        broadcast_from_rank0([b for m in (encoder, flow_decoder, seg_decoder) for b in m.buffers()], process_group)
        self.packer = engine.Conv3x3Packer(list(encoder._blocks) + list(flow_decoder.up_blocks)
                                           + list(seg_decoder.up_blocks), self._dtype)
        self._side = ops.side_stream_for(dev)
        self.overlap_wgrad = True
        self.fuse_tail = True
        self.lazy_up = True
        self._group = 0
        self._eval_owner = object()
        self._generation = evaluation.GenerationEval()
        self._ema = None
        if ema_decay is not None:
            self.fp.enable_ema(ema_decay)
            self._ema = TrainerEMA(self.fp, [encoder, flow_decoder, seg_decoder], ema_buffers)

    @property
    def step_count(self) -> int:
        return self.fp.step_count

    def _group_done(self) -> None:
        self.fp.bucketer.mark_ready_ordered(self._group, self._side if self.overlap_wgrad else None)
        self._group += 1

    def forward_backward(self, source: torch.Tensor, target: torch.Tensor, mask: torch.Tensor,
                         t: Optional[torch.Tensor] = None, want_outputs: bool = False):
        enc, fdec, sdec = self.encoder, self.flow_decoder, self.seg_decoder
        dt = self._dtype
        x0, x1 = source.float().contiguous(), target.float().contiguous()
        B = x0.shape[0]
        if t is None:
            t = torch.rand(B, device=x0.device, dtype=torch.float32)
        t = t.float().contiguous()
        eps_noise = torch.randn_like(x0) if self.sigma != 0.0 else None
        xt, ut = ops.cfm_sample(x0, x1, t, self.sigma, eps_noise)
        lazy = self.lazy_up and not want_outputs
        ectx1 = engine.encoder_forward(enc._blocks, xt, dt, True)
        temb = ops.time_embedding(t, self.time_emb_dim)
        f1 = ectx1.feats
        dctx_f = engine.decoder_forward(fdec, f1[-1], f1[:-1][::-1], temb, dt, True, with_head=False,
                                        fuse_tail=self.fuse_tail and not want_outputs, lazy_up=lazy)
        ectx2 = engine.encoder_forward(enc._blocks, x0, dt, True)
        f2 = ectx2.feats
        dctx_s = engine.decoder_forward(sdec, f2[-1], f2[:-1][::-1], None, dt, True, lazy_up=lazy)
        logits = dctx_s.v
        if dctx_f.lows[-1] is None:
            g_head = None
            flow, v = engine.decoder_tail_loss(fdec, dctx_f, ut, self.grads_flow, want_v=want_outputs)
        else:
            flow, g_head, v = ops.head_loss_fused(dctx_f.lows[-1], fdec.outc.weight.detach(),
                                                  fdec.outc.bias.detach() if fdec.outc.bias is not None else None, ut,
                                                  self.grads_flow["outc.weight"], self.grads_flow.get("outc.bias"),
                                                  want_v=want_outputs)
        w = float(self.seg_loss_weight)
        if self.num_classes is not None:
            tgt = mask[:, 0] if (mask.dim() == 4 and mask.shape[1] == 1) else mask
            seg3, dz = ops.seg_loss_multiclass(logits, tgt.long(), self.ignore_index, self.dice_smooth, self.dice_weight,
                                               want_grad=True, grad_scale=w, validate=False)
        else:
            seg3, dz = ops.seg_loss(logits, mask.float().reshape(logits.shape), self.dice_smooth, self.dice_weight,
                                    want_grad=True, grad_scale=w)
        total = flow + w * seg3[0]
        self.fp.bucketer.start_step()
        self._group = 0
        with engine.side_scope(self._side if self.overlap_wgrad else None):
            L = len(f1) - 1
            dbs, dss, _ = engine.decoder_backward(sdec, dctx_s, dz, self.grads_seg, on_group_done=self._group_done)
            dbf, dsf, _ = engine.decoder_backward(fdec, dctx_f, None, self.grads_flow, g_head=g_head,
                                                  on_group_done=self._group_done)
            engine.encoder_backward(enc._blocks, ectx2, [dss[L - 1 - l] for l in range(L)] + [dbs], self.grads_enc)
            engine.encoder_backward(enc._blocks, ectx1, [dsf[L - 1 - l] for l in range(L)] + [dbf], self.grads_enc,
                                    accumulate=True, on_group_done=self._group_done)
        second = "seg_ce" if self.num_classes is not None else "seg_bce"
        losses = {"total": total, "flow": flow, "seg": seg3[0], "seg_dice": seg3[1], second: seg3[2]}
        return losses, ({"v": v, "logits": logits} if want_outputs else None)

    def optimizer_step(self) -> None:
        engine.join_side(self._side)
        self.fp.adam(self.lr, self.betas, self.eps, self.wd)
        if self._ema is not None:
            self._ema.update_buffers()
        self.packer.repack()
        engine.mutation_epoch[0] += 1
        if self._ema is not None:
            self._ema.after_step()

    def _ema_on(self) -> TrainerEMA:
        if self._ema is None:
            raise RuntimeError("stain2stain_amd: this trainer keeps no EMA (construct it with ema_decay=...)")
        return self._ema

    def ema_model(self) -> Tuple[SharedEncoder, FlowMatchingDecoder, SegmentationDecoder]:
        return tuple(self._ema_on().modules())

    def _ema_container(self) -> torch.nn.ModuleDict:
        enc, fdec, sdec = self._ema_on().copies
        return torch.nn.ModuleDict(dict(encoder=enc, flow_decoder=fdec, seg_decoder=sdec))

    def ema_state_dict(self) -> Dict[str, torch.Tensor]:
        ema = self._ema_on()
        ema.modules()
        return ema.state_dict(self._ema_container().state_dict())

    def load_ema_state_dict(self, sd: Dict[str, torch.Tensor]) -> None:
        self._ema_on().load_state_dict(sd, self._ema_container())

    def step(self, source: torch.Tensor, target: torch.Tensor, mask: torch.Tensor,
             t: Optional[torch.Tensor] = None) -> torch.Tensor:
        losses, _ = self.forward_backward(source, target, mask, t)
        total = losses["total"]
        work = all_reduce_mean_scalar(total, self.pg) if self.sync_loss else None
        self.optimizer_step()
        if work is not None:
            work.wait()
            total = total / dist.get_world_size(self.pg)
        return total

    def evaluate(self, source: torch.Tensor, target: torch.Tensor, mask: torch.Tensor, t: Optional[torch.Tensor] = None,
                 accumulator: Optional[evaluation.EvalAccumulator] = None,
                 use_ema: bool = False, boundary: Optional[dict] = None) -> Dict[str, torch.Tensor]:
        if boundary is not None:
            if self.num_classes is not None:
                raise ValueError("MultiTaskTrainer.evaluate: boundary metrics are defined for the binary mask head only")
            morphology._check_agreement(**{"tolerance": 2, "percentile": 95, **boundary}, what="MultiTaskTrainer.evaluate")
        with ops.workspace_owner(self._eval_owner), evaluation.eval_grad_mode():
            x0, x1 = source.float().contiguous(), target.float().contiguous()
            if t is None:
                t = torch.rand(x0.shape[0], device=x0.device, dtype=torch.float32)
            t = t.float().contiguous()
            eps_noise = torch.randn_like(x0) if self.sigma != 0.0 else None
            xt, ut = ops.cfm_sample(x0, x1, t, self.sigma, eps_noise)
            enc, fdec, sdec = self.ema_model() if use_ema else (self.encoder, self.flow_decoder, self.seg_decoder)
            flow = evaluation.flow_loss(enc, fdec, self.time_emb_dim, xt, t, ut)
            logits = evaluation.mask_logits(enc, sdec, x0)
            d = evaluation.segmentation_values(logits, mask, self.num_classes, self.ignore_index, self.dice_smooth,
                                               self.dice_weight)
            second = "seg_ce" if self.num_classes is not None else "seg_bce"
            out = {"loss": flow + float(self.seg_loss_weight) * d["seg"], "flow_loss": flow, "seg_loss": d["seg"],
                   "seg_dice": d["seg_dice"], second: d[second], "dice_coef": d["dice_coef"], "iou": d["iou"]}
            if boundary is not None:
                B, H, W = logits.shape[0], logits.shape[-2], logits.shape[-1]
                a = morphology.mask_boundary_agreement((logits > 0).reshape(B, H, W), (mask > 0).reshape(B, H, W),
                                                       **boundary)
                out.update({f"boundary/{k}": a[k].mean() for k in ("hd", "assd", "surface_dice")})
        if accumulator is not None:
            accumulator.add(out, x0.shape[0])
        return out

    def evaluate_generation(self, source: torch.Tensor, target: torch.Tensor, num_steps: int = 50,
                            method: str = "euler", graph: bool = False, use_ema: bool = False,
                            accumulator: Optional[evaluation.EvalAccumulator] = None,
                            quantize: bool = True, stain: Optional[dict] = None) -> Dict[str, torch.Tensor]:
        enc, fdec, _ = self.ema_model() if use_ema else (self.encoder, self.flow_decoder, self.seg_decoder)
        with ops.workspace_owner(self._eval_owner), evaluation.eval_grad_mode():
            return evaluation.generation_values(self._generation, bool(use_ema), enc, fdec, self.time_emb_dim, source,
# ... 12 lines not shown
```

stain2stain_amd/ops.py:

```python
from __future__ import annotations

import contextlib
import ctypes
import os
import sys
from typing import Optional, Tuple

import torch

from . import _native
from ._regionio import gpu_rows

BF16, F32 = 0, 1


def _dt(t: torch.Tensor) -> int:
    if t.dtype == torch.bfloat16:
        return BF16
    if t.dtype == torch.float32:
        return F32
    raise RuntimeError(f"stain2stain_amd: unsupported activation dtype {t.dtype}")


_raw_stream = getattr(torch._C, "_cuda_getCurrentRawStream", None)
# ... 145 lines not shown
    return torch.cuda.Stream(device=device)


_SHARED_SIDE = {}


def shared_side_stream(device) -> Optional[torch.cuda.Stream]:
    dev = torch.device(device)
    key = dev.index if dev.index is not None else torch.cuda.current_device()
    if key not in _SHARED_SIDE:
        _SHARED_SIDE[key] = side_stream_for(dev)
    return _SHARED_SIDE[key]


class TimingEvent:

    def __init__(self):
        out = ctypes.c_long(0)
        _native.check(_L().s2s_event_create(1, ctypes.addressof(out)), "event_create")
        self._e = out.value

    def record(self) -> None:
        _native.check(_L().s2s_event_record(self._e, _stream()), "event_record")

    def elapsed_time(self, end: "TimingEvent") -> float:
        ms = ctypes.c_float(0.0)
        _native.check(_L().s2s_event_synchronize(end._e), "event_synchronize")
        _native.check(_L().s2s_event_elapsed_ms(self._e, end._e, ctypes.addressof(ms)), "event_elapsed")
        return float(ms.value)

    def __del__(self):
        try:
            if self._e and not sys.is_finalizing():
                _L().s2s_event_destroy(self._e)
        except Exception:
            pass


def _timing_event():
    if os.environ.get("S2S_TIMING_EVENTS", "1") == "0":
        return torch.cuda.Event(enable_timing=True)
    return TimingEvent()


def profile_stop() -> list:
    global _PROFILE
    out, _PROFILE = _PROFILE or [], None
    return out


def _timed(name: str, work_fn=None):
    def deco(fn):
        def wrapped(*args, **kwargs):
            if _PROFILE is None or (_PROFILE_ONLY is not None and name not in _PROFILE_ONLY):
                return fn(*args, **kwargs)
            e0 = _timing_event()
            e1 = _timing_event()
            e0.record()
            out = fn(*args, **kwargs)
            e1.record()
            _PROFILE.append((name + ("@" + PROFILE_TAG if PROFILE_TAG else ""), work_fn(*args, **kwargs) if work_fn else 0.0, e0, e1))
            return out
        wrapped.__name__ = fn.__name__
        wrapped.__doc__ = fn.__doc__
        return wrapped
    return deco


def _conv_flops(x0, x1, w_packed, bias, cout, **kw) -> float:
    B, H, W, c0 = x0.shape
    cin = c0 + (x1.shape[3] if x1 is not None else 0)
    return 2.0 * B * H * W * cout * 9 * cin


def _wgrad_flops(dy, x0, x1, grad_oihw, accumulate=False) -> float:
    B, H, W, cout = dy.shape
    cin = x0.shape[3] + (x1.shape[3] if x1 is not None else 0)
    return 2.0 * B * H * W * cout * 9 * cin


@_timed("conv3x3_mfma", _conv_flops)
def conv3x3(x0: torch.Tensor, x1: Optional[torch.Tensor], w_packed: torch.Tensor, bias: Optional[torch.Tensor],
            cout: int, *, want_stats: bool = False, scale: Optional[torch.Tensor] = None,
            shift: Optional[torch.Tensor] = None, relu: bool = False, out: Optional[torch.Tensor] = None):
    B, H, W, c0 = x0.shape
    dt = _dt(x0)
    p0, ld0 = _nhwc(x0)
    p1, ld1, c1 = 0, 8, 0
    if x1 is not None:
        if x1.shape[:3] != x0.shape[:3] or x1.dtype != x0.dtype:
            raise RuntimeError("stain2stain_amd: conv3x3 sources disagree in shape/dtype")
        p1, ld1 = _nhwc(x1)
        c1 = x1.shape[3]
    if w_packed.dtype != x0.dtype or w_packed.numel() != _L().s2s_pack_conv3x3_fwd_elems(cout, c0 + c1):
        raise RuntimeError("stain2stain_amd: packed weight does not match (cout, cin, dtype)")
    if out is None:
        out = torch.empty((B, H, W, cout), dtype=x0.dtype, device=x0.device)
    elif out.shape != (B, H, W, cout) or out.dtype != x0.dtype:
        raise RuntimeError("stain2stain_amd: conv3x3 output buffer mismatch")
    py, ldy = _nhwc(out)
    stat, nb = None, 0
    if want_stats:
        nb = _L().s2s_conv3x3_stat_rows(dt, B, H, W, cout, c0, c1, ld0, ld1, int(bias is not None))
        _native.check(min(nb, 0), "conv3x3_stat_rows")
        stat = torch.empty((2, cout, nb), dtype=torch.float32, device=x0.device)
    kwork = None
    if not want_stats:
        nsplit = _L().s2s_conv3x3_ksplit(dt, B, H, W, cout, c0 + c1)
        if nsplit > 1:
            kwork = torch.empty((nsplit, B * H * W, cout), dtype=torch.float32, device=x0.device)
    rc = _L().s2s_conv3x3_nhwc_s(dt, p0, ld0, c0, p1, ld1, c1, _ptr(w_packed), _f32(bias), py, ldy, _f32(stat), nb,
                                 _f32(scale), _f32(shift), int(relu), _f32(kwork), B, H, W, cout, _stream())
    _native.check(rc, "conv3x3")
    return out, stat


CONV3X3_PLAN_FIELDS = ("family", "cfg", "gx", "gy", "grid", "xsp", "xsn", "ksplit", "stat_rows")


def conv3x3_plan(dtype: torch.dtype, B: int, H: int, W: int, c0: int, c1: int, cout: int, *, ld0: Optional[int] = None,
                 ld1: Optional[int] = None, ldy: Optional[int] = None, bias: bool = False, affine: bool = False,
                 stats: bool = False, stat_rows: int = -1, kwork: bool = False) -> dict:
    dt = BF16 if dtype == torch.bfloat16 else F32
    out = (ctypes.c_int * len(CONV3X3_PLAN_FIELDS))()
    rc = _L().s2s_conv3x3_plan(dt, B, H, W, cout, c0, c1, c0 if ld0 is None else ld0, max(c1, 8) if ld1 is None else ld1,
                               cout if ldy is None else ldy, int(bias), int(affine), int(stats),
                               stat_rows if stats else 0, int(kwork), ctypes.cast(out, ctypes.c_void_p))
    _native.check(rc, "conv3x3_plan")
    return dict(zip(CONV3X3_PLAN_FIELDS, (int(v) for v in out)))


def conv3x3_wgrad(dy: torch.Tensor, x0: torch.Tensor, x1: Optional[torch.Tensor], grad_oihw: torch.Tensor,
                  accumulate: bool = False, _reference: bool = False, _phases: int = 3,
                  _part: Optional[torch.Tensor] = None) -> None:
    B, H, W, cout = dy.shape
    c0 = x0.shape[3]
    dt = _dt(dy)
    if x0.dtype != dy.dtype or x0.shape[:3] != dy.shape[:3]:
        raise RuntimeError("stain2stain_amd: conv3x3_wgrad operand mismatch")
    pdy, lddy = _nhwc(dy)
    p0, ld0 = _nhwc(x0)
    p1, ld1, c1 = 0, 8, 0
    if x1 is not None:
        p1, ld1 = _nhwc(x1)
        c1 = x1.shape[3]
    if tuple(grad_oihw.shape) != (cout, c0 + c1, 3, 3):
        raise RuntimeError("stain2stain_amd: conv3x3_wgrad gradient buffer has the wrong shape")
    s = _L().s2s_conv3x3_wgrad_splits(dt, B, H, W, c0 + c1, cout)
    if _reference or _phases != 3 or _part is not None:
        if _part is None:
            _part = _workspace(dy.device, s * 9 * cout * (c0 + c1), "wgrad")
        elif _part.dtype != torch.float32 or _part.numel() < s * 9 * cout * (c0 + c1) or not _part.is_contiguous():
            raise RuntimeError("stain2stain_amd: conv3x3_wgrad slab buffer is too small")
        rc = _L().s2s_conv3x3_wgrad_phase_variant(dt, pdy, lddy, cout, p0, ld0, c0, p1, ld1, c1, _f32(_part),
                                                  _f32(grad_oihw), int(accumulate), B, H, W, _phases, int(_reference),
                                                  _stream())
        _native.check(rc, "conv3x3_wgrad")
        return
    part = _workspace(dy.device, s * 9 * cout * (c0 + c1), "wgrad")
    if _PROFILE is not None and (_PROFILE_ONLY is None or "conv3x3_wgrad_mfma" in _PROFILE_ONLY):
        for name, phase, work in (("conv3x3_wgrad_mfma", 1, _wgrad_flops(dy, x0, x1, grad_oihw)), ("wgrad_fold", 2, 0.0)):
            e0 = _timing_event()
            e1 = _timing_event()
            e0.record()
            rc = _L().s2s_conv3x3_wgrad_phase(dt, pdy, lddy, cout, p0, ld0, c0, p1, ld1, c1, _f32(part), _f32(grad_oihw),
                                              int(accumulate), B, H, W, phase, _stream())
            e1.record()
            _native.check(rc, "conv3x3_wgrad")
            _PROFILE.append((name, work, e0, e1))
        return
    rc = _L().s2s_conv3x3_wgrad_nhwc(dt, pdy, lddy, cout, p0, ld0, c0, p1, ld1, c1, _f32(part), _f32(grad_oihw),
                                     int(accumulate), B, H, W, _stream())
    _native.check(rc, "conv3x3_wgrad")


def conv3x3_wgrad_plan(dtype: torch.dtype, B: int, H: int, W: int, cin: int, cout: int) -> dict:
    dt = BF16 if dtype == torch.bfloat16 else F32
    plan = {}
    for what, name in enumerate(("splits", "tiles", "xcd", "fold", "kernel")):
        plan[name] = _L().s2s_conv3x3_wgrad_plan(dt, B, H, W, cin, cout, what)
        _native.check(min(plan[name], 0), "conv3x3_wgrad_plan")
    return plan


HEAD_FALLBACK_MO4, HEAD_FALLBACK_MO8 = 104, 108


def head_family(dtype: torch.dtype, B: int, H: int, W: int, C: int, cout: int, forward: bool) -> int:
    return _L().s2s_head_family(BF16 if dtype == torch.bfloat16 else F32, B, H, W, C, cout, int(forward))


@_timed("stem_fwd")
def stem_fwd(x_nchw: torch.Tensor, w: torch.Tensor, bias: Optional[torch.Tensor], dtype: torch.dtype,
             want_stats: bool = True):
    B, cin, H, W = x_nchw.shape
    cout = w.shape[0]
    if tuple(w.shape) != (cout, cin, 3, 3):
        raise RuntimeError("stain2stain_amd: stem weight shape")
    y = torch.empty((B, H, W, cout), dtype=dtype, device=x_nchw.device)
    stat = None
    if want_stats:
        stat = torch.empty((2, cout, _L().s2s_stem_stat_blocks(B, H, W)), dtype=torch.float32, device=y.device)
    rc = _L().s2s_stem_conv3x3_fwd(_dt(y), _f32(x_nchw), _f32(w), _f32(bias), y.data_ptr(), cout, _f32(stat), B, H, W,
                                   cin, cout, _stream())
    _native.check(rc, "stem_conv3x3_fwd")
    return y, stat
# ... 121 lines not shown
                                _f32(dbias_conv), int(accumulate), B, H, W, C, cout, _stream())
    _native.check(rc, "tail_fwd_loss")
    return loss, g, v, work


@_timed("tail_bwd_apply")
def tail_bwd_apply(raw: torch.Tensor, stats: torch.Tensor, w: torch.Tensor, g: torch.Tensor, gamma: torch.Tensor,
                   work: torch.Tensor) -> torch.Tensor:
    B, H, W, C = raw.shape
    cout = w.shape[0]
    px, ldx = _nhwc(raw)
    if tuple(g.shape) != (B, cout, H, W) or work.numel() != 2 * C * _L().s2s_bn_bwd_blocks(B, H, W, C) + 2 * C:
        raise RuntimeError("stain2stain_amd: tail_bwd_apply operands do not belong to this tail_fwd_loss")
    dx = torch.empty((B, H, W, C), dtype=raw.dtype, device=raw.device)
    rc = _L().s2s_tail_bwd_apply(_dt(raw), px, ldx, _f32(g), _f32(w.reshape(cout, C)), stats[2].data_ptr(),
                                 stats[3].data_ptr(), stats[0].data_ptr(), stats[1].data_ptr(), _f32(gamma),
                                 _f32(work), dx.data_ptr(), C, B, H, W, C, cout, _stream())
    _native.check(rc, "tail_bwd_apply")
    return dx


@_timed("bn_finalize")
def bn_finalize(stat: torch.Tensor, count: int, gamma, beta, running_mean, running_var, num_batches,
                momentum: float = 0.1, eps: float = 1e-5, conv_bias: Optional[torch.Tensor] = None):
    _, C, nblk = stat.shape
    dev = stat.device
    out = torch.empty((4, C), dtype=torch.float32, device=dev)
    rc = _L().s2s_bn_finalize_b(_f32(stat), nblk, C, count, _f32(gamma), _f32(beta), _f32(running_mean),
                                _f32(running_var), 0 if num_batches is None else num_batches.data_ptr(), momentum, eps,
                                out[0].data_ptr(), out[1].data_ptr(), out[2].data_ptr(), out[3].data_ptr(),
                                _f32(conv_bias), _stream())
    _native.check(rc, "bn_finalize")
    return out


def bn_partial_sums(stat: torch.Tensor) -> torch.Tensor:
    _, C, nblk = stat.shape
    sums = torch.empty((2, C), dtype=torch.float32, device=stat.device)
    _native.check(_L().s2s_bn_partial_sums(_f32(stat), nblk, C, _f32(sums), _stream()), "bn_partial_sums")
    return sums


def bn_eval_prepare(gamma, beta, rmean, rvar, eps: float = 1e-5):
    C = gamma.numel()
    out = torch.empty((2, C), dtype=torch.float32, device=gamma.device)
    rc = _L().s2s_bn_eval_prepare(C, _f32(gamma), _f32(beta), _f32(rmean), _f32(rvar), eps, out[0].data_ptr(),
                                  out[1].data_ptr(), _stream())
    _native.check(rc, "bn_eval_prepare")
    return out


@_timed("bn_relu_apply")
def bn_relu_apply(x: torch.Tensor, scale: torch.Tensor, shift: torch.Tensor, out: Optional[torch.Tensor] = None,
                  pool: Optional[torch.Tensor] = None, want_pool: bool = False):
    B, H, W, C = x.shape
    px, ldx = _nhwc(x)
    if out is None:
        out = torch.empty((B, H, W, C), dtype=x.dtype, device=x.device)
    py, ldy = _nhwc(out)
    pp, ldp = 0, 8
    if want_pool and pool is None:
        pool = torch.empty((B, H // 2, W // 2, C), dtype=x.dtype, device=x.device)
    if pool is not None:
        pp, ldp = _nhwc(pool)
    rc = _L().s2s_bn_relu_apply(_dt(x), px, ldx, _f32(scale), _f32(shift), py, ldy, pp, ldp, B, H, W, C, _stream())
    _native.check(rc, "bn_relu_apply")
    return out, pool


@_timed("maxpool2")
def maxpool2(x: torch.Tensor) -> torch.Tensor:
    B, H, W, C = x.shape
    px, ldx = _nhwc(x)
    pool = torch.empty((B, H // 2, W // 2, C), dtype=x.dtype, device=x.device)
    rc = _L().s2s_maxpool2(_dt(x), px, ldx, pool.data_ptr(), C, B, H, W, C, _stream())
    _native.check(rc, "maxpool2")
    return pool


@_timed("bn_relu_bwd")
def bn_relu_bwd(g1: Optional[torch.Tensor], gp: Optional[torch.Tensor], x: torch.Tensor,
                stats: torch.Tensor, gamma: torch.Tensor, dgamma: torch.Tensor, dbeta: torch.Tensor,
                dbias_conv: Optional[torch.Tensor], accumulate: bool = False, exchange=None,
                count_total: Optional[int] = None) -> torch.Tensor:
    B, H, W, C = x.shape
    px, ldx = _nhwc(x)
    p1, ld1 = (0, 8) if g1 is None else _nhwc(g1)
    p2, ld2 = (0, 8) if gp is None else _nhwc(gp)
    dx = torch.empty((B, H, W, C), dtype=x.dtype, device=x.device)
    nb = _L().s2s_bn_bwd_blocks(B, H, W, C)
    work = torch.empty((4 * nb * C + 2 * C,), dtype=torch.float32, device=x.device)
    if exchange is not None:
        for phase in (1, 2):
            rc = _L().s2s_bn_relu_bwd_phase(_dt(x), p1, ld1, p2, ld2, stats[2].data_ptr(), stats[3].data_ptr(), px, ldx,
                                            stats[0].data_ptr(), stats[1].data_ptr(),
                                            _f32(gamma), _f32(dgamma), _f32(dbeta), _f32(dbias_conv), int(accumulate),
                                            dx.data_ptr(), C, _f32(work), B, H, W, C,
                                            int(count_total if count_total is not None else B * H * W), phase, _stream())
            _native.check(rc, "bn_relu_bwd")
            if phase == 1:
                exchange(work[4 * nb * C:])
        return dx
    rc = _L().s2s_bn_relu_bwd(_dt(x), p1, ld1, p2, ld2, stats[2].data_ptr(), stats[3].data_ptr(), px, ldx,
                              stats[0].data_ptr(), stats[1].data_ptr(),
                              _f32(gamma), _f32(dgamma), _f32(dbeta), _f32(dbias_conv), int(accumulate),
                              dx.data_ptr(), C, _f32(work), B, H, W, C, _stream())
    _native.check(rc, "bn_relu_bwd")
    return dx


@_timed("upsample2x_fwd")
def upsample2x_fwd(x: torch.Tensor, out: torch.Tensor, bias_nc: Optional[torch.Tensor] = None,
                   _reference: bool = False, bn_relu: Optional[Tuple[torch.Tensor, torch.Tensor]] = None) -> None:
    B, Hin, Win, C = x.shape
    _, Hout, Wout, Co = out.shape
    if Co != C or out.dtype != x.dtype:
        raise RuntimeError("stain2stain_amd: upsample output slice mismatch")
    if bn_relu is not None:
        scale, shift = bn_relu
        if scale.numel() != C or shift.numel() != C:
            raise RuntimeError("stain2stain_amd: upsample scale / shift do not match the channel count")
        if _reference or upsample2x_fwd_family(x, out) != 1:
            x, _ = bn_relu_apply(x, scale, shift)
        else:
            px, ldx = _nhwc(x)
            py, ldy = _nhwc(out)
            rc = _L().s2s_upsample2x_bn_relu_fwd(_dt(x), px, ldx, _f32(scale), _f32(shift), _f32(bias_nc), py, ldy, B,
                                                 Hin, Win, Hout, Wout, C, _stream())
            _native.check(rc, "upsample2x_fwd")
            return
    px, ldx = _nhwc(x)
    py, ldy = _nhwc(out)
    fn = _L().s2s_upsample2x_bilinear_ac_fwd_ref if _reference else _L().s2s_upsample2x_bilinear_ac_fwd
    rc = fn(_dt(x), px, ldx, _f32(bias_nc), py, ldy, B, Hin, Win, Hout, Wout, C, _stream())
    _native.check(rc, "upsample2x_fwd")


def upsample2x_fwd_family(x: torch.Tensor, out: torch.Tensor, _reference: bool = False) -> int:
    B, Hin, Win, C = x.shape
    _, Hout, Wout, _ = out.shape
    rc = _L().s2s_upsample2x_fwd_family(_nhwc(x)[1], _nhwc(out)[1], B, Hin, Win, Hout, Wout, C, int(_reference))
    if rc < 0:
        _native.check(rc, "upsample2x_fwd_family")
    return rc


@_timed("upsample2x_bwd")
def upsample2x_bwd(dy: torch.Tensor, hin: int, win: int, _reference: bool = False) -> torch.Tensor:
    B, Hout, Wout, C = dy.shape
    pdy, lddy = _nhwc(dy)
    dx = torch.empty((B, hin, win, C), dtype=dy.dtype, device=dy.device)
    fn = _L().s2s_upsample2x_bilinear_ac_bwd_ref if _reference else _L().s2s_upsample2x_bilinear_ac_bwd
    rc = fn(_dt(dy), pdy, lddy, dx.data_ptr(), C, B, hin, win, Hout, Wout, C, _stream())
    _native.check(rc, "upsample2x_bwd")
    return dx


def upsample2x_bwd_family(dy: torch.Tensor, hin: int, win: int, _reference: bool = False) -> int:
    B, Hout, Wout, C = dy.shape
    rc = _L().s2s_upsample2x_bwd_family(dy.stride(2), C, B, hin, win, Hout, Wout, C, int(_reference))
    if rc < 0:
        _native.check(rc, "upsample2x_bwd_family")
    return rc


def pixel_sum(x: torch.Tensor) -> torch.Tensor:
    B, H, W, C = x.shape
    px, ldx = _nhwc(x)
    out = torch.empty((B, C), dtype=torch.float32, device=x.device)
    rc = _L().s2s_pixel_sum(_dt(x), px, ldx, _f32(out), B, H * W, C, 0, _stream())
    _native.check(rc, "pixel_sum")
    return out


# ... 1242 lines not shown
```

stain2stain_amd/trainer.py:

```python
from __future__ import annotations

from typing import Dict, List, Optional, Tuple

import torch
import torch.distributed as dist

from . import engine, evaluation, ops
from .components import FlowUNet
from .ema import TrainerEMA
from .ddp import all_reduce_mean_scalar, broadcast_from_rank0
from .fused_step import CapturedStep, FlatParams


def _param_groups(net: FlowUNet) -> List[List[Tuple[str, str, torch.nn.Parameter]]]:
    dec, enc = net.flow_decoder, net.encoder
    dnamed = dict(dec.named_parameters())
    enamed = dict(enc.named_parameters())
    groups: List[List[Tuple[str, str, torch.nn.Parameter]]] = []

    def layer(owner, named, prefix):
        for idx in (("3.", "4."), ("0.", "1.")):
            groups.append([(owner, n, p) for n, p in named.items()
                           if any(n.startswith(prefix + i) for i in idx)])

    groups.append([("dec", n, p) for n, p in dnamed.items() if n.startswith("outc.")])
    for i in range(len(dec.ups) - 1, -1, -1):
        layer("dec", dnamed, f"ups.{i}.conv.double_conv.")
    groups.append([("dec", n, p) for n, p in dnamed.items() if n.startswith("time_")])
    for i in range(len(enc.downs) - 1, -1, -1):
        layer("enc", enamed, f"downs.{i}.maxpool_conv.1.double_conv.")
    layer("enc", enamed, "inc.double_conv.")
    groups = [g for g in groups if g] if getattr(dec, "time_mlp", None) is None else groups
    seen = sum(len(g) for g in groups)
    if seen != len(dnamed) + len(enamed) or any(not g for g in groups):
        raise RuntimeError("parameter grouping does not cover the network")
    return groups


class FusedAdamHandle(torch.optim.Optimizer):

    def __init__(self, trainer: "CFMTrainer", lr, betas, eps, weight_decay):
        self._trainer = trainer
        super().__init__([trainer.fp.p], dict(lr=lr, betas=tuple(betas), eps=eps, weight_decay=weight_decay))

    @torch.no_grad()
    def step(self, closure=None):
        loss = closure() if closure is not None else None
        self._trainer.optimizer_step()
        return loss

    def zero_grad(self, set_to_none: bool = False) -> None:
        pass

    def state_dict(self):
        return self._trainer.optimizer_state_dict()

    def load_state_dict(self, state_dict) -> None:
        self._trainer.load_optimizer_state_dict(state_dict)


class CFMTrainer:
    def __init__(self, net: FlowUNet, lr: float = 1e-4, weight_decay: float = 1e-5,
                 betas: Tuple[float, float] = (0.9, 0.999), eps: float = 1e-8, sigma: float = 0.0,
                 bucket_mb: float = 4.0, process_group=None, sync_loss: bool = True, max_bucket_mb: float = 16.0,
                 sharded_optimizer: bool = False, sync_batchnorm: bool = False, graph: bool = False,
                 ema_decay: Optional[float] = None, ema_buffers: bool = True):
        dev = next(net.parameters()).device
        if dev.type != "cuda":
            raise RuntimeError("stain2stain_amd: CFMTrainer needs the network on a GPU (HIP-only implementation)")
        self.net = net
        self.sigma = sigma
        self.pg = process_group
        self.sync_loss = sync_loss
        groups = [[(f"{owner}.{name}", p) for owner, name, p in g] for g in _param_groups(net)]
        self.fp = FlatParams(groups, bucket_mb, process_group, max_bucket_mb, sharded_optimizer)
        self.grads_enc = {k[len("enc."):]: v for k, v in self.fp.grads.items() if k.startswith("enc.")}
        self.grads_dec = {k[len("dec."):]: v for k, v in self.fp.grads.items() if k.startswith("dec.")}
        names = {id(p): name for g in groups for name, p in g}
        self._names = [names[id(p)] for p in net.parameters()]
        self.optimizer = FusedAdamHandle(self, lr, betas, eps, weight_decay)
        self.n_params = sum(p.numel() for g in groups for _, p in g)
        self._group = 0
        self._sync_bn = engine.SyncBNExchange(process_group) if sync_batchnorm and self.bucketer.enabled else None
        broadcast_from_rank0(list(net.buffers()), process_group)
        self._dtype = net.encoder.compute_dtype
        self.packer = engine.Conv3x3Packer(list(net.encoder._blocks) + list(net.flow_decoder.up_blocks), self._dtype)
        self._side = ops.side_stream_for(dev)
        self.overlap_wgrad = True
        self.fuse_tail = True
        self.lazy_up = True
        self.graph = graph
        self._graph_step = CapturedStep()
        self._ema = None
        if ema_decay is not None:
            self.fp.enable_ema(ema_decay)
            self._ema = TrainerEMA(self.fp, [net], ema_buffers)
        self._eval_owner = object()
        self._generation = evaluation.GenerationEval()

    step_count = property(lambda self: self.fp.step_count)
    bucketer = property(lambda self: self.fp.bucketer)
    flat_p = property(lambda self: self.fp.p)
    flat_g = property(lambda self: self.fp.g)
    _captured = property(lambda self: self._graph_step.graph)

    @property
    def _hp(self):
        return self.optimizer.param_groups[0]

    lr = property(lambda self: self._hp["lr"], lambda self, v: self._hp.__setitem__("lr", v))
    wd = property(lambda self: self._hp["weight_decay"], lambda self, v: self._hp.__setitem__("weight_decay", v))
    betas = property(lambda self: self._hp["betas"], lambda self, v: self._hp.__setitem__("betas", tuple(v)))
    eps = property(lambda self: self._hp["eps"], lambda self, v: self._hp.__setitem__("eps", v))

    def forward_backward(self, x0: torch.Tensor, x1: torch.Tensor, t: Optional[torch.Tensor] = None,
                         want_v: bool = True):
        net = self.net
        enc, dec = net.encoder, net.flow_decoder
        dt = enc.compute_dtype
        B = x0.shape[0]
        x0, x1 = x0.float().contiguous(), x1.float().contiguous()
        if t is None:
            t = torch.rand(B, device=x0.device, dtype=torch.float32)
        t = t.float().contiguous()
        eps_noise = torch.randn_like(x0) if self.sigma != 0.0 else None
        xt, ut = ops.cfm_sample(x0, x1, t, self.sigma, eps_noise)
        with engine.sync_batchnorm(self._sync_bn):
            lazy = self.lazy_up and not want_v
            ectx = engine.encoder_forward(enc._blocks, xt, dt, True, lazy_up=lazy)
            temb = ops.time_embedding(t, net.time_embedding.dim)
            feats = ectx.feats
            dctx = engine.decoder_forward(dec, feats[-1], feats[:-1][::-1], temb, dt, True, with_head=False,
                                          fuse_tail=self.fuse_tail and not want_v, lazy_up=lazy)
        if dctx.lows[-1] is None:
            g_head = None
            loss, v = engine.decoder_tail_loss(dec, dctx, ut, self.grads_dec, want_v=want_v)
        else:
            loss, g_head, v = ops.head_loss_fused(dctx.lows[-1], dec.outc.weight.detach(),
                                                  dec.outc.bias.detach() if dec.outc.bias is not None else None, ut,
                                                  self.grads_dec["outc.weight"], self.grads_dec.get("outc.bias"),
                                                  want_v=want_v)
            dctx.v = v
        self.bucketer.start_step()
        self._group = 0
        with engine.side_scope(self._side if self.overlap_wgrad else None):
            dbott, dskips, _ = engine.decoder_backward(dec, dctx, None, self.grads_dec, g_head=g_head,
                                                       on_group_done=self._group_done)
            L = len(feats) - 1
            dfeats = [dskips[L - 1 - l] for l in range(L)] + [dbott]
            engine.encoder_backward(enc._blocks, ectx, dfeats, self.grads_enc, on_group_done=self._group_done)
        return loss, dctx.v

    def _group_done(self) -> None:
        self.bucketer.mark_ready_ordered(self._group, self._side if self.overlap_wgrad else None)
        self._group += 1

    def optimizer_step(self) -> None:
        self._enqueue_optimizer(None)
        self._after_step()

    def _after_step(self) -> None:
        engine.mutation_epoch[0] += 1
        if self._ema is not None:
            self._ema.after_step()

    def _enqueue_optimizer(self, hyper_dev: Optional[torch.Tensor]) -> None:
        engine.join_side(self._side)
        self.fp.adam(self.lr, self.betas, self.eps, self.wd, hyper_dev)
        if self._ema is not None:
            self._ema.update_buffers()
        self._repack()

    def _repack(self) -> None:
        self.packer.repack()

    def optimizer_state_dict(self) -> Dict:
        sd = self.fp.state_dict()
        state = {}
        if self.step_count > 0:
            for i, name in enumerate(self._names):
                state[i] = {"step": torch.tensor(float(self.step_count)),
                            "exp_avg": sd["exp_avg"][name], "exp_avg_sq": sd["exp_avg_sq"][name]}
        group = {"lr": self.lr, "betas": tuple(self.betas), "eps": self.eps, "weight_decay": self.wd,
                 "amsgrad": False, "maximize": False, "foreach": None, "capturable": False, "differentiable": False,
                 "fused": None, "params": list(range(len(self._names)))}
        return {"state": state, "param_groups": [group]}

    def load_optimizer_state_dict(self, sd: Dict) -> None:
        groups = sd["param_groups"]
        if len(groups) != 1 or len(groups[0]["params"]) != len(self._names):
            raise ValueError("optimizer state does not match this network (one group over net.parameters() expected)")
        if groups[0].get("amsgrad", False) or groups[0].get("maximize", False):
            raise ValueError("amsgrad / maximize Adam states are not supported")
        g = groups[0]
        self.lr, self.betas, self.eps, self.wd = g["lr"], tuple(g["betas"]), g["eps"], g["weight_decay"]
        steps = set()
        fp = self.fp
        fp.m.zero_()
        fp.v.zero_()
        for i, (p, name) in enumerate(zip(self.net.parameters(), self._names)):
            st = sd["state"].get(i, sd["state"].get(str(i)))
            if st is None:
                continue
            o, n = fp.slot[name]
            if tuple(st["exp_avg"].shape) != tuple(p.shape):
                raise ValueError(f"optimizer state {i}: shape {tuple(st['exp_avg'].shape)} != {tuple(p.shape)}")
            fp.m[o:o + n].copy_(st["exp_avg"].reshape(-1))
            fp.v[o:o + n].copy_(st["exp_avg_sq"].reshape(-1))
            steps.add(int(float(st["step"])))
        if len(steps) > 1:
            raise ValueError("per-parameter step counts differ; the flat Adam kernel keeps one")
        fp.step_count = steps.pop() if steps else 0

    def step(self, x0: torch.Tensor, x1: torch.Tensor, t: Optional[torch.Tensor] = None) -> torch.Tensor:
        with ops.workspace_owner(self):
            if self.graph and ops._PROFILE is None:
                if t is None:
                    t = torch.rand(x0.shape[0], device=x0.device, dtype=torch.float32)
                if self.sigma != 0.0:
                    raise NotImplementedError("graph=True with sigma != 0: the path noise is drawn inside forward_backward")
                loss = self._graph_step.run((tuple(x0.shape), x0.device, self.overlap_wgrad), (x0, x1, t),
                                            self._step_body, [self.fp], (self.lr, self.betas, self.eps, self.wd))
            else:
                loss = self._step_body(x0, x1, t, None)
            self._after_step()
            return loss

    def _step_body(self, x0, x1, t, hyper_dev) -> torch.Tensor:
        loss, _ = self.forward_backward(x0, x1, t, want_v=False)
        work = all_reduce_mean_scalar(loss, self.pg) if self.sync_loss else None
        self._enqueue_optimizer(hyper_dev)
        if work is not None:
            work.wait()
# ... 57 lines not shown
```

Before: 2349.

## Fuse BatchNorm-backward reduction sums into the dgrad conv epilogue

Adds a variant of the 3x3 conv dgrad kernels (tap and staged families) that, while writing the input-gradient tile, also reads the saved pre-BN activation and accumulates the per-channel ReLU-masked dy and dy*xhat sums. A new presummed BN-ReLU backward entry then uses these partials instead of running its own reduction pass over the gradient and activation. This is meant to remove a full extra read of both tensors and a reduction kernel per BN layer in the backward pass. In exchange the conv epilogue loads an extra tensor and keeps extra LDS constants, which could lower occupancy or lengthen the epilogue. Some tile configs are excluded.

```diff
diff --git a/include/stain2stain_hip.h b/include/stain2stain_hip.h
--- a/include/stain2stain_hip.h
+++ b/include/stain2stain_hip.h
@@ -35,6 +35,13 @@
 int s2s_conv3x3_nhwc_s(int dtype, const void* x0, int ld0, int c0, const void* x1, int ld1, int c1, const void* w_packed,
                        const float* bias, void* y, int ldy, float* stat_part, int stat_rows, const float* ep_scale,
                        const float* ep_shift, int relu, float* kwork, int B, int H, int W, int Cout, void* stream);
+int s2s_conv3x3_bnsum_rows(int dtype, int B, int H, int W, int Cout, int c0, int ld0, int ldy, int ldraw);
+int s2s_conv3x3_plan_bns(int dtype, int B, int H, int W, int Cout, int c0, int c1, int ld0, int ld1, int ldy, int has_bias,
+                         int has_affine, int stats, int stat_rows, int kwork, int bnsums, int* out);
+int s2s_conv3x3_nhwc_bns(int dtype, const void* x0, int ld0, int c0, const void* w_packed, void* y, int ldy,
+                         float* stat_part, int stat_rows, const void* raw, int ldraw, const float* scale,
+                         const float* shift, const float* mean, const float* invstd, int B, int H, int W, int Cout,
+                         void* stream);
 int s2s_debug_conv_clock(long* out_host, int n);
 
 int s2s_conv3x3_wgrad_splits(int dtype, int B, int H, int W, int Cin, int Cout);
@@ -104,6 +111,10 @@
                           const float* shift, const void* x, int ldx, const float* mean, const float* invstd,
                           const float* gamma, float* dgamma, float* dbeta, float* dbias_conv, int accumulate, void* dx,
                           int lddx, float* work, int B, int H, int W, int C, long count_total, int phases, void* stream);
+int s2s_bn_relu_bwd_presummed(int dtype, const void* g1, int ldg1, const float* part, int nblk, const float* scale,
+                              const float* shift, const void* x, int ldx, const float* mean, const float* invstd,
+                              const float* gamma, float* dgamma, float* dbeta, float* dbias_conv, int accumulate, void* dx,
+                              int lddx, float* work, int B, int H, int W, int C, void* stream);
 
 int s2s_upsample2x_bilinear_ac_fwd(int dtype, const void* x, int ldx, const float* bias_nc, void* y, int ldy, int B,
                                    int Hin, int Win, int Hout, int Wout, int C, void* stream);
diff --git a/stain2stain_amd/csrc/conv3x3_mfma.hip b/stain2stain_amd/csrc/conv3x3_mfma.hip
--- a/stain2stain_amd/csrc/conv3x3_mfma.hip
+++ b/stain2stain_amd/csrc/conv3x3_mfma.hip
@@ -35,6 +35,12 @@
   int xsp, xsn;
   long stat_rows;
   long stat_rows_req;
+  const void* bn_raw;
+  int ldraw;
+  const float* bn_scale;
+  const float* bn_shift;
+  const float* bn_mean;
+  const float* bn_invstd;
   int dbg;
 };
 
@@ -635,8 +641,107 @@
   if constexpr (STATS && !CARRY) conv_stats_flush<BN, WN>(a, s1, s2, n0, tid, stat_row);
 }
 
+template <int BN, int NT>
+__device__ __forceinline__ void bnsum_stage_consts(const Conv3x3Args& a, float* kc, int n0, int tid) {
+  for (int i = tid; i < BN; i += NT) {
+    const int c = n0 + i;
+    const bool in = c < a.Cout;
+    kc[i] = in ? a.bn_scale[c] : 0.f;
+    kc[BN + i] = in ? a.bn_shift[c] : 0.f;
+    kc[2 * BN + i] = in ? a.bn_mean[c] : 0.f;
+    kc[3 * BN + i] = in ? a.bn_invstd[c] : 0.f;
+  }
+  asm volatile("s_waitcnt lgkmcnt(0)" ::: "memory");
+}
+
+template <int BN>
+__device__ __forceinline__ void bnsum_accumulate(const bf16x8 val, const bf16x8 b, const float* kc8, float (&s1)[8], float (&s2)[8]) {
+  const f32x4 sc0 = *reinterpret_cast<const f32x4*>(kc8), sc1 = *reinterpret_cast<const f32x4*>(kc8 + 4);
+  const f32x4 sh0 = *reinterpret_cast<const f32x4*>(kc8 + BN), sh1 = *reinterpret_cast<const f32x4*>(kc8 + BN + 4);
+  const f32x4 mu0 = *reinterpret_cast<const f32x4*>(kc8 + 2 * BN), mu1 = *reinterpret_cast<const f32x4*>(kc8 + 2 * BN + 4);
+  const f32x4 is0 = *reinterpret_cast<const f32x4*>(kc8 + 3 * BN), is1 = *reinterpret_cast<const f32x4*>(kc8 + 3 * BN + 4);
+#pragma unroll
+  for (int k = 0; k < 8; ++k) {
+    const float bk = (float)b[k];
+    const float sc = k < 4 ? sc0[k & 3] : sc1[k & 3], sh = k < 4 ? sh0[k & 3] : sh1[k & 3];
+    const float mu = k < 4 ? mu0[k & 3] : mu1[k & 3], is = k < 4 ? is0[k & 3] : is1[k & 3];
+    const float dz = fmaf(bk, sc, sh) > 0.f ? (float)val[k] : 0.f;
+    s1[k] += dz;
+    s2[k] += dz * ((bk - mu) * is);
+  }
+}
+
+template <int TH, int TW, int BN, int WM, int WN>
+__device__ __forceinline__ void conv_epilogue16_bnsums(const Conv3x3Args& a, f32x4 (&acc)[(TH * TW / WM) / 16][(BN / WN) / 16],
+                                                       const float (&bias)[(BN / WN) / 16][4], const float* kc, int img,
+                                                       int y0, int x0p, int n0, int tid, long stat_row) {
+  using T = bf16_t;
+  constexpr int BM = TH * TW, WTM = BM / WM, WTN = BN / WN, MI = WTM / 16, NI = WTN / 16;
+  static_assert(NI % 2 == 0, "channel blocks are exchanged in pairs");
+  T* __restrict__ yout = static_cast<T*>(a.y);
+  const T* __restrict__ raw = static_cast<const T*>(a.bn_raw);
+  const int lane = tid & 63, wave = tid >> 6;
+  const int wm = wave / WN, wn = wave % WN;
+  const int cl = lane & 15, q = lane >> 4;
+  const int nloc = wn * WTN + (q & 1) * 16 + (q >> 1) * 8;
+#pragma unroll
+  for (int pr = 0; pr < NI / 2; ++pr) {
+    const int n = n0 + nloc + pr * 32;
+    const bool nok = n < a.Cout;
+    bf16x8 bv[MI];
+#pragma unroll
+    for (int mi = 0; mi < MI; ++mi) {
+      const int m = wm * WTM + mi * 16 + cl;
+      const int py = m / TW, px = m - py * TW;
+      const int gy = y0 + py, gx = x0p + px;
+#pragma unroll
+      for (int k = 0; k < 8; ++k) bv[mi][k] = (bf16_t)0.f;
+      if (nok && gy < a.H && gx < a.W)
+        bv[mi] = *reinterpret_cast<const bf16x8*>(raw + (((long)img * a.H + gy) * a.W + gx) * a.ldraw + n);
+    }
+    float s1[8], s2[8];
+#pragma unroll
+    for (int k = 0; k < 8; ++k) { s1[k] = 0.f; s2[k] = 0.f; }
+#pragma unroll
+    for (int mi = 0; mi < MI; ++mi) {
+      const int m = wm * WTM + mi * 16 + cl;
+      const int py = m / TW, px = m - py * TW;
+      const int gy = y0 + py, gx = x0p + px;
+      const bool pok = gy < a.H && gx < a.W;
+      const long opix = ((long)img * a.H + gy) * a.W + gx;
+      unsigned w[2][2];
+#pragma unroll
+      for (int b = 0; b < 2; ++b) {
+        bf16x4 pk;
+#pragma unroll
+        for (int j = 0; j < 4; ++j) pk[j] = (bf16_t)(acc[mi][2 * pr + b][j] + bias[2 * pr + b][j]);
+        const uint2 u = __builtin_bit_cast(uint2, pk);
+        w[b][0] = u.x; w[b][1] = u.y;
+      }
+      const auto r0 = __builtin_amdgcn_permlane16_swap(w[0][0], w[1][0], false, false);
+      const auto r1 = __builtin_amdgcn_permlane16_swap(w[0][1], w[1][1], false, false);
+      const uint4 out = make_uint4(r0[0], r1[0], r0[1], r1[1]);
+      if (pok && nok) {
+        *reinterpret_cast<uint4*>(yout + opix * a.ldy + n) = out;
+        bnsum_accumulate<BN>(__builtin_bit_cast(bf16x8, out), bv[mi], kc + nloc + pr * 32, s1, s2);
+      }
+    }
+#pragma unroll
+    for (int k = 0; k < 8; ++k) {
+      float u = s1[k], w2 = s2[k];
+      u = row_ror_add<8>(u); u = row_ror_add<4>(u); u = row_ror_add<2>(u); u = row_ror_add<1>(u);
+      w2 = row_ror_add<8>(w2); w2 = row_ror_add<4>(w2); w2 = row_ror_add<2>(w2); w2 = row_ror_add<1>(w2);
+      if (cl == 0 && n + k < a.Cout) {
+        a.stat_part[((long)n + k) * a.stat_rows + stat_row] = u;
+        a.stat_part[((long)a.Cout + n + k) * a.stat_rows + stat_row] = w2;
+      }
+    }
+    __builtin_amdgcn_sched_barrier(0);
+  }
+}
+
 __device__ long g_clk[8192 * 4];
-template <int TH, int TW, int BN, int WM, int WN, int NS>
+template <int TH, int TW, int BN, int WM, int WN, int NS, bool BNS = false>
 __global__ __launch_bounds__(256, 2) void conv3x3_dma16_kernel(Conv3x3Args a) {
   long c0_ = 0, w0_ = 0;
   if ((a.dbg & 64) && threadIdx.x == 0) { c0_ = __builtin_readcyclecounter(); w0_ = wall_clock64(); }
@@ -760,6 +865,8 @@
   };
   dma_halo(c_lo);
   static_for<NS - 1>([&](auto k) { dma_w(decltype(k)::value); });
+  float* const kc = reinterpret_cast<float*>(smem + 2 * A_BYTES + NS * B_BYTES);
+  if constexpr (BNS) bnsum_stage_consts<BN, 256>(a, kc, n0, tid);
   wait_vm<0>();
   __builtin_amdgcn_s_barrier();
 
@@ -817,6 +924,10 @@
     });
   }
   if (S2S_ABL(a.dbg & 16)) return;
+  if constexpr (BNS) {
+    conv_epilogue16_bnsums<TH, TW, BN, WM, WN>(a, acc, biasr, kc, img, y0, x0p, n0, tid, (long)tile_id * WM + wm);
+    return;
+  }
   if (a.kpart) {
     float* const kpz = a.kpart + (long)blockIdx.z * ((long)a.B * a.H * a.W) * a.Cout;
 #pragma unroll
@@ -1054,6 +1165,8 @@
                                  {16, 16, 128, 2, false}, {16, 16, 64, 4, true}, {8, 16, 128, 2, true}, {8, 16, 64, 2, true}};
 constexpr TileCfg kF32Cfg[2] = {{4, 32, 64, 2, false}, {8, 16, 64, 2, false}};
 constexpr int kMinBlocks = 448;
+
+constexpr bool bns_tile(const TileCfg& c) { return !(c.bn == 128 && c.th * c.tw == 256); }
 
 inline long cfg_blocks(const TileCfg& c, int B, int H, int W, int Cout) {
   return (long)B * cdiv(H, c.th) * cdiv(W, c.tw) * cdiv(Cout, c.bn);
@@ -1091,6 +1204,7 @@
   int xsp, xsn;
   int ksplit;
   long stat_rows;
+  bool bns;
 };
 
 template <int ID>
@@ -1116,8 +1230,9 @@
   return S2S_OK;
 }
 
-template <int STATS, bool DEFER_EP, bool RESIDENT, bool AFFINE = false>
+template <int STATS, bool DEFER_EP, bool RESIDENT, bool AFFINE = false, bool BNS = false>
 __global__ __launch_bounds__(512, 1) void conv3x3_stage_kernel(Conv3x3Args a, int njobs, int GX, int GY) {
+  static_assert(!BNS || (STATS == 2 && !DEFER_EP && !AFFINE), "the sums ride on the carried statistics of the in-place epilogue");
   using T = bf16_t;
   constexpr int TH = 16, TW = 32, BN = 64, WM = 8, WN = 1;
   constexpr int HP = TW + 4, ROWS = (TH + 2) * HP;
@@ -1284,11 +1399,27 @@
   const __amdgpu_buffer_rsrc_t rs_y = __builtin_amdgcn_make_buffer_rsrc(yout, 0, (int)((((long)a.B * a.H * a.W - 1) * a.ldy + a.Cout) * 2), 0x00020000);
   const int nl = (kp & 1) * 16 + (kp >> 1) * 8;
   const unsigned vst = (unsigned)(cl * a.ldy + nl) * 2u;
+  const __amdgpu_buffer_rsrc_t rs_raw = __builtin_amdgcn_make_buffer_rsrc(
+      const_cast<void*>(BNS ? a.bn_raw : a.y), 0, BNS ? (int)((((long)a.B * a.H * a.W - 1) * a.ldraw + a.Cout) * 2) : 0, 0x00020000);
+  const unsigned vraw = (unsigned)(cl * a.ldraw + nl) * 2u;
+  float* const kc = reinterpret_cast<float*>(smem + 2 * STAGE);
+  u32x4_t rawv[BNS ? MI : 1][BNS ? NI / 2 : 1];
+  auto raw_unit = [&](auto uc, const Tile& t) {
+    constexpr int u = decltype(uc)::value, mi = u / (NI / 2), pr = u % (NI / 2);
+    const int gy = t.y0 + wm * (WTM / TW) + mi / RB, gx0 = t.x0p + (mi % RB) * 16, nb = t.n0 + pr * 32;
+    const bool ok = gy < a.H && gx0 + cl < a.W && nb + nl < a.Cout;
+    rawv[mi][pr] = __builtin_amdgcn_raw_buffer_load_b128(rs_raw, ok ? vraw : OOB,
+                                                         (((t.img * a.H + gy) * a.W + gx0) * a.ldraw + nb) * 2, 0);
+  };
   auto store_unit = [&](auto uc, const Tile& t) {
     constexpr int u = decltype(uc)::value, mi = u / (NI / 2), pr = u % (NI / 2);
     const int gy = t.y0 + wm * (WTM / TW) + mi / RB, gx0 = t.x0p + (mi % RB) * 16, nb = t.n0 + pr * 32;
     const bool ok = gy < a.H && gx0 + cl < a.W && nb + nl < a.Cout;
-    if constexpr (STATS == 2) {
+    if constexpr (BNS) {
+      const uint4 zero = make_uint4(0u, 0u, 0u, 0u);
+      bnsum_accumulate<BN>(__builtin_bit_cast(bf16x8, ok ? outv[mi][pr] : zero), __builtin_bit_cast(bf16x8, rawv[mi][pr]),
+                           kc + nl + pr * 32, cs1[pr], cs2[pr]);
+    } else if constexpr (STATS == 2) {
       const bf16x8 val = __builtin_bit_cast(bf16x8, outv[mi][pr]);
 #pragma unroll
       for (int k = 0; k < 8; ++k) {
@@ -1353,6 +1484,7 @@
   dma_weights(cur.n0, 0, 0);
   if constexpr (RESIDENT) dma_weights(cur.n0, a.nchunk > 1 ? 1 : 0, 1);
   load_affine(cur.n0);
+  if constexpr (BNS) bnsum_stage_consts<BN, 512>(a, kc, cur.n0, tid);
   bool pend = false, pend_full = false;
   bool ynst = false;
   int st = 0;
@@ -1409,6 +1541,7 @@
         pend = true;
         pend_full = full;
       } else {
+        if constexpr (BNS) static_for<NST>([&](auto uc) { raw_unit(uc, prv); });
         static_for<NST>([&](auto uc) { store_unit(uc, prv); });
         ynst = full;
       }
@@ -1428,6 +1561,11 @@
         dma_weights(nxt.n0, a.nchunk > 1 ? 1 : 0, 1);
         ynst = false;
       }
+      if constexpr (BNS) {
+        if constexpr (!RESIDENT) __builtin_amdgcn_s_barrier();
+        bnsum_stage_consts<BN, 512>(a, kc, nxt.n0, tid);
+        ynst = false;
+      }
     }
     L += G;
     cur = nxt;
@@ -1450,7 +1588,9 @@
   if (!on || (a.c1 && a.c0 % 32) || (a.bias && !a.ep_scale) || (a.ep_scale && stats) || split || a.act || a.y2 ||
       (a.dbg & 64)) return 0;
   if ((double)a.B * a.H * a.W * a.ld0 * 2 >= 4.0e9 || (double)a.B * a.H * a.W * (a.c1 ? a.ld1 : 0) * 2 >= 4.0e9 ||
-      (double)a.B * a.H * a.W * a.ldy * 2 >= 2.0e9) return 0;
+      (double)a.B * a.H * a.W * a.ldy * 2 >= 2.0e9 ||
+      (a.bn_raw && (double)a.B * a.H * a.W * a.ldraw * 2 >= 2.0e9))
+    return 0;
   const long GX = (long)a.B * cdiv(a.H, 16) * cdiv(a.W, 32), GY = cdiv(a.Cout, 64);
   const long njobs = GX * GY;
   constexpr int slots = 256;
@@ -1467,6 +1607,16 @@
   a.tilesY = cdiv(a.H, 16);
   a.tilesX = cdiv(a.W, 32);
   const bool resident = p.family == kStageResident;
+  if (p.bns) {
+    constexpr int lds_bns = lds + 4 * 64 * 4;
+    static_assert(lds_bns <= 160 * 1024, "LDS budget");
+    auto kern_b = resident ? conv3x3_stage_kernel<2, false, true, false, true> : conv3x3_stage_kernel<2, false, false, false, true>;
+    static unsigned long long attr_b[2] = {0, 0};
+    if (int rc = s2s_allow_dyn_lds(reinterpret_cast<const void*>(kern_b), lds_bns, &attr_b[resident ? 1 : 0])) return rc;
+    hipLaunchKernelGGL(kern_b, dim3(p.grid), dim3(512), lds_bns, s, a, p.gx * p.gy, p.gx, p.gy);
+    S2S_LAUNCH_CHECK();
+    return S2S_OK;
+  }
   const int form = a.stat_part ? 1 : (a.ep_scale ? 2 : 0);
   auto kern = form == 1 ? (resident ? conv3x3_stage_kernel<2, false, true> : conv3x3_stage_kernel<2, false, false>)
             : form == 2 ? (resident ? conv3x3_stage_kernel<0, false, true, true> : conv3x3_stage_kernel<0, false, false, true>)
@@ -1488,6 +1638,18 @@
   static_assert(lds <= 160 * 1024, "LDS budget");
   a.tilesY = cdiv(a.H, TH);
   a.tilesX = cdiv(a.W, TW);
+  if constexpr (!bns_tile(c)) {
+    if (p.bns) return S2S_ERR_SHAPE;
+  } else if (p.bns) {
+    constexpr int lds_bns = lds + 4 * BN * 4;
+    static_assert(lds_bns <= 160 * 1024, "LDS budget");
+    auto kern_b = conv3x3_dma16_kernel<TH, TW, BN, WM, WN, NS, true>;
+    static unsigned long long attr_b = 0;
+    if (int rc = s2s_allow_dyn_lds(reinterpret_cast<const void*>(kern_b), lds_bns, &attr_b)) return rc;
+    hipLaunchKernelGGL(kern_b, dim3(p.gx, p.gy, 1), dim3(256), lds_bns, s, a);
+    S2S_LAUNCH_CHECK();
+    return S2S_OK;
+  }
   auto kern = conv3x3_dma16_kernel<TH, TW, BN, WM, WN, NS>;
   static unsigned long long attr_devs = 0;
   if (int rc = s2s_allow_dyn_lds(reinterpret_cast<const void*>(kern), lds, &attr_devs)) return rc;
@@ -2117,6 +2279,7 @@
   }
   if (a.kpart && !stats) p.ksplit = split_count((long)p.gx * p.gy, a.nchunk);
   const bool split = p.ksplit > 1;
+  const bool bns = a.bn_raw && stats && !a.bias && !a.ep_scale && !a.act && !a.y2 && !a.kpart;
   if (const int wg = stage_grid(a, stats, split)) {
     if (!stats || req == kAnyRows || req == (long)wg * 8) {
       p.family = a.c0 + a.c1 <= 64 ? kStageResident : kStageStream;
@@ -2125,6 +2288,7 @@
       p.grid = wg;
       p.xsp = p.gx % 8 == 0 ? 8 : 0;
       p.stat_rows = (long)wg * 8;
+      p.bns = bns;
       return p;
     }
   }
@@ -2142,6 +2306,7 @@
     static const int xcd_aware = [] { const char* e = getenv("S2S_CONV_XCD"); return e ? atoi(e) : 1; }();
     p.family = kTap;
     p.stat_rows = (long)p.gx * c.wm;
+    p.bns = bns && bns_tile(c);
     if (xcd_aware && !split && ((long)p.gx * p.gy) % 8 == 0) xcd_cut(a, p.gx, p.gy, p);
   }
   if (stats && req > 0 && req != p.stat_rows) p.rc = S2S_ERR_SHAPE;
@@ -2157,6 +2322,7 @@
 int dispatch(int dtype, Conv3x3Args& a, hipStream_t s) {
   const Conv3x3Plan p = conv3x3_plan(dtype, a);
   if (p.rc != S2S_OK) return p.rc;
+  if (a.bn_raw && !p.bns) return S2S_ERR_SHAPE;
   a.xsp = p.xsp; a.xsn = p.xsn; a.ksplit = p.ksplit; a.stat_rows = p.stat_rows;
   if (p.ksplit == 1) a.kpart = nullptr;
   switch (p.family) {
@@ -2297,6 +2463,44 @@
   const int v[9] = {p.family, p.cfg, p.gx, p.gy, p.grid, p.xsp, p.xsn, p.ksplit, (int)p.stat_rows};
   for (int i = 0; i < 9; ++i) out[i] = v[i];
   return S2S_OK;
+}
+
+static Conv3x3Plan conv3x3_query_bns(int dtype, int B, int H, int W, int Cout, int c0, int c1, int ld0, int ld1, int ldy,
+                                     int ldraw, int has_bias, int has_affine, int stats, int stat_rows, int kwork,
+                                     int bnsums) {
+  static float present;
+  Conv3x3Args a{};
+  conv3x3_fill_args(a, ld0, c0, ld1, c1, has_bias ? &present : nullptr, B, H, W, Cout);
+  a.ldy = ldy;
+  a.ep_scale = has_affine ? &present : nullptr;
+  a.ep_shift = a.ep_scale;
+  a.stat_part = stats ? &present : nullptr;
+  a.stat_rows_req = stat_rows;
+  a.kpart = kwork ? &present : nullptr;
+  a.bn_raw = bnsums ? &present : nullptr;
+  a.ldraw = ldraw;
+  return conv3x3_plan(dtype, a);
+}
+
+extern "C" int s2s_conv3x3_plan_bns(int dtype, int B, int H, int W, int Cout, int c0, int c1, int ld0, int ld1, int ldy,
+                                    int has_bias, int has_affine, int stats, int stat_rows, int kwork, int bnsums, int* out) {
+  if (!out) return S2S_ERR_NULL;
+  if (B <= 0 || H <= 0 || W <= 0 || Cout <= 0 || c0 <= 0 || c1 < 0) return S2S_ERR_SHAPE;
+  if (dtype != S2S_BF16 && dtype != S2S_F32) return S2S_ERR_DTYPE;
+  const Conv3x3Plan p = conv3x3_query_bns(dtype, B, H, W, Cout, c0, c1, ld0, ld1, ldy, Cout, has_bias, has_affine, stats,
+                                          stat_rows, kwork, bnsums);
+  if (p.rc != S2S_OK) return p.rc;
+  const int v[10] = {p.family, p.cfg, p.gx, p.gy, p.grid, p.xsp, p.xsn, p.ksplit, (int)p.stat_rows, p.bns ? 1 : 0};
+  for (int i = 0; i < 10; ++i) out[i] = v[i];
+  return S2S_OK;
+}
+
+extern "C" int s2s_conv3x3_bnsum_rows(int dtype, int B, int H, int W, int Cout, int c0, int ld0, int ldy, int ldraw) {
+  if (B <= 0 || H <= 0 || W <= 0 || Cout <= 0 || c0 <= 0) return S2S_ERR_SHAPE;
+  if (dtype != S2S_BF16 && dtype != S2S_F32) return S2S_ERR_DTYPE;
+  const Conv3x3Plan p = conv3x3_query_bns(dtype, B, H, W, Cout, c0, 0, ld0, 8, ldy, ldraw, 0, 0, 1, (int)kAnyRows, 0, 1);
+  if (p.rc != S2S_OK) return p.rc;
+  return p.bns ? (int)p.stat_rows : 0;
 }
 
 extern "C" int s2s_conv3x3_nhwc_k(int dtype, const void* x0, int ld0, int c0, const void* x1, int ld1, int c1,
@@ -2335,6 +2539,24 @@
   hipLaunchKernelGGL(convk_splitk_reduce_kernel<bf16_t>, dim3((unsigned)nb), dim3(256), 0, s, a, npix);
   S2S_LAUNCH_CHECK();
   return S2S_OK;
+}
+
+extern "C" int s2s_conv3x3_nhwc_bns(int dtype, const void* x0, int ld0, int c0, const void* w_packed, void* y, int ldy,
+                                    float* stat_part, int stat_rows, const void* raw, int ldraw, const float* scale,
+                                    const float* shift, const float* mean, const float* invstd, int B, int H, int W,
+                                    int Cout, void* stream) {
+  if (!x0 || !w_packed || !y || !stat_part || !raw || !scale || !shift || !mean || !invstd) return S2S_ERR_NULL;
+  if (B <= 0 || H <= 0 || W <= 0 || Cout <= 0 || c0 <= 0 || stat_rows <= 0) return S2S_ERR_SHAPE;
+  if ((c0 % 8) || (ld0 % 8) || (Cout % 8) || (ldy % 8) || ldy < Cout || (ldraw % 8) || ldraw < Cout) return S2S_ERR_SHAPE;
+  const uintptr_t al = 15;
+  if (((uintptr_t)x0 & al) || ((uintptr_t)w_packed & al) || ((uintptr_t)y & al) || ((uintptr_t)raw & al)) return S2S_ERR_ALIGN;
+  if (dtype != S2S_BF16) return dtype == S2S_F32 ? S2S_ERR_SHAPE : S2S_ERR_DTYPE;
+  Conv3x3Args a{};
+  conv3x3_fill_args(a, ld0, c0, 8, 0, nullptr, B, H, W, Cout);
+  a.x0 = x0; a.x1 = nullptr; a.w = w_packed; a.y = y; a.ldy = ldy;
+  a.stat_part = stat_part; a.stat_rows_req = stat_rows;
+  a.bn_raw = raw; a.ldraw = ldraw; a.bn_scale = scale; a.bn_shift = shift; a.bn_mean = mean; a.bn_invstd = invstd;
+  return dispatch(dtype, a, static_cast<hipStream_t>(stream));
 }
 extern "C" int s2s_convkxk_stat_blocks(int dtype, int B, int H, int W, int Cout, int ks) {
   if (B <= 0 || H <= 0 || W <= 0 || Cout <= 0 || (ks != 2 && ks != 4)) return S2S_ERR_SHAPE;
diff --git a/stain2stain_amd/csrc/norm_act.hip b/stain2stain_amd/csrc/norm_act.hip
--- a/stain2stain_amd/csrc/norm_act.hip
+++ b/stain2stain_amd/csrc/norm_act.hip
@@ -721,6 +721,37 @@
   return S2S_OK;
 }
 
+extern "C" int s2s_bn_relu_bwd_presummed(int dtype, const void* g1, int ldg1, const float* part, int nblk, const float* scale,
+                                         const float* shift, const void* x, int ldx, const float* mean, const float* invstd,
+                                         const float* gamma, float* dgamma, float* dbeta, float* dbias_conv, int accumulate,
+                                         void* dx, int lddx, float* work, int B, int H, int W, int C, void* stream) {
+  if (!g1 || !part || !scale || !shift || !x || !mean || !invstd || !gamma || !dgamma || !dbeta || !dx || !work) return S2S_ERR_NULL;
+  if (B <= 0 || H <= 0 || W <= 0 || C <= 0 || nblk <= 0 || (C % 8) || (ldx % 8) || (lddx % 8) || (ldg1 % 8)) return S2S_ERR_SHAPE;
+  if ((long)B * ((H + 1) / 2) * ((W + 1) / 2) >= (1L << 31) - (1 << 20)) return S2S_ERR_SHAPE;
+  if (dtype != S2S_BF16 && dtype != S2S_F32) return S2S_ERR_DTYPE;
+  const int nb = red_blocks(B, H, W, C);
+  float* c1 = work + (long)nb * 4 * C;
+  float* c2 = c1 + C;
+  const double count = (double)((long)B * H * W);
+  hipStream_t s = (hipStream_t)stream;
+  float* const dbias_zero = (dbias_conv && !accumulate) ? dbias_conv : nullptr;
+  if (finalize_tpc(nblk) == 256)
+    hipLaunchKernelGGL(bn_bwd_finalize_kernel<256>, dim3(C), dim3(256), 0, s, part, nblk, C, count, dgamma, dbeta,
+                       accumulate, c1, c2, dbias_zero);
+  else
+    hipLaunchKernelGGL(bn_bwd_finalize_kernel<64>, dim3(cdiv(C, 4)), dim3(256), 0, s, part, nblk, C, count, dgamma,
+                       dbeta, accumulate, c1, c2, dbias_zero);
+  dim3 grid(cdiv(C / 8, host_pcb(C)), nb);
+  if (dtype == S2S_BF16)
+    hipLaunchKernelGGL(bn_relu_bwd_apply_flat_kernel<bf16_t>, grid, dim3(256), 0, s, (const bf16_t*)g1, ldg1, scale, shift,
+                       (const bf16_t*)x, ldx, mean, invstd, gamma, c1, c2, (bf16_t*)dx, lddx, nullptr, (long)B * H * W, C, 1);
+  else
+    hipLaunchKernelGGL(bn_relu_bwd_apply_flat_kernel<float>, grid, dim3(256), 0, s, (const float*)g1, ldg1, scale, shift,
+                       (const float*)x, ldx, mean, invstd, gamma, c1, c2, (float*)dx, lddx, nullptr, (long)B * H * W, C, 1);
+  S2S_LAUNCH_CHECK();
+  return S2S_OK;
+}
+
 int s2s_internal_tail_bn_sums(int dtype, const void* raw, int ldx, const float* g_nchw, const float* w, const float* scale,
                               const float* shift, const float* mean, const float* invstd, float* work, float* dgamma,
                               float* dbeta, float* zero_out, int accumulate, int B, int H, int W, int C, int Cout,
diff --git a/stain2stain_amd/engine.py b/stain2stain_amd/engine.py
--- a/stain2stain_amd/engine.py
+++ b/stain2stain_amd/engine.py
@@ -351,14 +351,26 @@
         raise RuntimeError(f"stain2stain_amd: no gradient buffer for parameter {name!r}") from e
 
 
-def _conv_bn_relu_bwd(cb: ConvBN, lc: LayerCtx, g1, gp, grads, accumulate: bool, need_dx: bool, stem: bool = False):
+def _dgrad(cb: ConvBN, draw: torch.Tensor, consumer: Optional[LayerCtx]):
+    if consumer is not None and consumer.sync is None and draw.dtype == torch.bfloat16:
+        return ops.conv3x3(draw, None, cb.packed(draw.dtype)[1], None, cb.cin, bn_sums=(consumer.raw, consumer.stats))
+    dx, _ = ops.conv3x3(draw, None, cb.packed(draw.dtype)[1], None, cb.cin)
+    return dx, None
+
+
+def _conv_bn_relu_bwd(cb: ConvBN, lc: LayerCtx, g1, gp, grads, accumulate: bool, need_dx: bool, stem: bool = False,
+                      consumer: Optional[LayerCtx] = None, presummed: Optional[torch.Tensor] = None):
     p = cb.prefix
     i_conv, i_bn = cb.idx
     dgamma = _g(grads, f"{p}.{i_bn}.weight")
     dbeta = _g(grads, f"{p}.{i_bn}.bias")
     dbias = _g(grads, f"{p}.{i_conv}.bias") if cb.conv.bias is not None else None
-    draw = ops.bn_relu_bwd(g1, gp, lc.raw, lc.stats, cb.bn.weight.detach(), dgamma, dbeta, dbias, accumulate,
-                           exchange=lc.sync, count_total=lc.count)
+    if presummed is not None and gp is None and lc.sync is None:
+        draw = ops.bn_relu_bwd(g1, None, lc.raw, lc.stats, cb.bn.weight.detach(), dgamma, dbeta, dbias, accumulate,
+                               presummed=presummed)
+    else:
+        draw = ops.bn_relu_bwd(g1, gp, lc.raw, lc.stats, cb.bn.weight.detach(), dgamma, dbeta, dbias, accumulate,
+                               exchange=lc.sync, count_total=lc.count)
     dw = _g(grads, f"{p}.{i_conv}.weight")
     if stem:
         run_on_side(lambda: ops.stem_wgrad(draw, lc.x0, dw, None, accumulate), (draw,))
@@ -366,8 +378,8 @@
     run_on_side(lambda: ops.conv3x3_wgrad(draw, lc.x0, lc.x1, dw, accumulate), (draw,))
     if not need_dx:
         return None
-    dx, _ = ops.conv3x3(draw, None, cb.packed(draw.dtype)[1], None, cb.cin)
-    return dx
+    dx, part = _dgrad(cb, draw, consumer)
+    return (dx, part) if consumer is not None else dx
 
 
 def _conv_bn_tail(cb: ConvBN, x0, dtype):
@@ -394,13 +406,12 @@
     return loss, v
 
 
-def _conv_bn_tail_bwd(dec, cb: ConvBN, lc: LayerCtx, tail, grads, accumulate: bool):
+def _conv_bn_tail_bwd(dec, cb: ConvBN, lc: LayerCtx, tail, grads, accumulate: bool, consumer: Optional[LayerCtx] = None):
     g, work = tail
     draw = ops.tail_bwd_apply(lc.raw, lc.stats, dec.outc.weight.detach(), g, cb.bn.weight.detach(), work)
     dw = _g(grads, f"{cb.prefix}.{cb.idx[0]}.weight")
     run_on_side(lambda: ops.conv3x3_wgrad(draw, lc.x0, lc.x1, dw, accumulate), (draw,))
-    dx, _ = ops.conv3x3(draw, None, cb.packed(draw.dtype)[1], None, cb.cin)
-    return dx
+    return _dgrad(cb, draw, consumer)
 
 
 def encoder_forward(blocks: Sequence[Tuple[ConvBN, ConvBN]], x_nchw: torch.Tensor, dtype: torch.dtype,
@@ -423,7 +434,8 @@
 
 
 def encoder_backward(blocks: Sequence[Tuple[ConvBN, ConvBN]], ctx: EncCtx, dfeats: Sequence[Optional[torch.Tensor]],
-                     grads: Dict[str, torch.Tensor], accumulate: bool = False, on_group_done=None) -> None:
+                     grads: Dict[str, torch.Tensor], accumulate: bool = False, on_group_done=None,
+                     bn_sums: bool = False) -> None:
     gpool = None
     nlev = len(blocks)
     for l in range(len(blocks) - 1, -1, -1):
@@ -432,10 +444,13 @@
         g1 = dfeats[l]
         if g1 is None and gpool is None:
             raise RuntimeError("stain2stain_amd: encoder level without any incoming gradient")
-        ga1 = _conv_bn_relu_bwd(c2, lc2, g1, gpool, grads, accumulate, need_dx=True)
+        if bn_sums and l > 0:
+            ga1, part = _conv_bn_relu_bwd(c2, lc2, g1, gpool, grads, accumulate, need_dx=True, consumer=lc1)
+        else:
+            ga1, part = _conv_bn_relu_bwd(c2, lc2, g1, gpool, grads, accumulate, need_dx=True), None
         if on_group_done is not None:
             on_group_done()
-        gpool = _conv_bn_relu_bwd(c1, lc1, ga1, None, grads, accumulate, need_dx=(l > 0), stem=(l == 0))
+        gpool = _conv_bn_relu_bwd(c1, lc1, ga1, None, grads, accumulate, need_dx=(l > 0), stem=(l == 0), presummed=part)
         if on_group_done is not None:
             on_group_done()
 
@@ -479,7 +494,7 @@
 
 def decoder_backward(dec, ctx: DecCtx, dv: Optional[torch.Tensor], grads: Dict[str, torch.Tensor],
                      accumulate: bool = False, need_dt_emb: bool = False, on_group_done=None,
-                     g_head: Optional[torch.Tensor] = None):
+                     g_head: Optional[torch.Tensor] = None, bn_sums: bool = False):
     if ctx.tail is not None:
         g = None
     elif g_head is not None:
@@ -495,12 +510,14 @@
         c1, c2 = dec.up_blocks[i]
         lc1, lc2 = ctx.layers[i]
         if ctx.tail is not None and i == nup - 1:
-            ga1 = _conv_bn_tail_bwd(dec, c2, lc2, ctx.tail, grads, accumulate)
+            ga1, part = _conv_bn_tail_bwd(dec, c2, lc2, ctx.tail, grads, accumulate, lc1 if bn_sums else None)
+        elif bn_sums:
+            ga1, part = _conv_bn_relu_bwd(c2, lc2, g, None, grads, accumulate, need_dx=True, consumer=lc1)
         else:
-            ga1 = _conv_bn_relu_bwd(c2, lc2, g, None, grads, accumulate, need_dx=True)
+            ga1, part = _conv_bn_relu_bwd(c2, lc2, g, None, grads, accumulate, need_dx=True), None
         if on_group_done is not None:
             on_group_done()
-        dcat = _conv_bn_relu_bwd(c1, lc1, ga1, None, grads, accumulate, need_dx=True)
+        dcat = _conv_bn_relu_bwd(c1, lc1, ga1, None, grads, accumulate, need_dx=True, presummed=part)
         cs = ctx.skips[i].shape[3]
         dskips[i] = dcat[..., :cs]
         low = ctx.lows[i]
diff --git a/stain2stain_amd/multitask_trainer.py b/stain2stain_amd/multitask_trainer.py
--- a/stain2stain_amd/multitask_trainer.py
+++ b/stain2stain_amd/multitask_trainer.py
@@ -76,6 +76,7 @@
         self.overlap_wgrad = True
         self.fuse_tail = True
         self.lazy_up = True
+        self.dgrad_bn_sums = True
         self._group = 0
         self._eval_owner = object()
         self._generation = evaluation.GenerationEval()
@@ -134,12 +135,15 @@
         self._group = 0
         with engine.side_scope(self._side if self.overlap_wgrad else None):
             L = len(f1) - 1
-            dbs, dss, _ = engine.decoder_backward(sdec, dctx_s, dz, self.grads_seg, on_group_done=self._group_done)
+            sums = self.dgrad_bn_sums
+            dbs, dss, _ = engine.decoder_backward(sdec, dctx_s, dz, self.grads_seg, on_group_done=self._group_done,
+                                                  bn_sums=sums)
             dbf, dsf, _ = engine.decoder_backward(fdec, dctx_f, None, self.grads_flow, g_head=g_head,
-                                                  on_group_done=self._group_done)
-            engine.encoder_backward(enc._blocks, ectx2, [dss[L - 1 - l] for l in range(L)] + [dbs], self.grads_enc)
+                                                  on_group_done=self._group_done, bn_sums=sums)
+            engine.encoder_backward(enc._blocks, ectx2, [dss[L - 1 - l] for l in range(L)] + [dbs], self.grads_enc,
+                                    bn_sums=sums)
             engine.encoder_backward(enc._blocks, ectx1, [dsf[L - 1 - l] for l in range(L)] + [dbf], self.grads_enc,
-                                    accumulate=True, on_group_done=self._group_done)
+                                    accumulate=True, on_group_done=self._group_done, bn_sums=sums)
         second = "seg_ce" if self.num_classes is not None else "seg_bce"
         losses = {"total": total, "flow": flow, "seg": seg3[0], "seg_dice": seg3[1], second: seg3[2]}
         return losses, ({"v": v, "logits": logits} if want_outputs else None)
diff --git a/stain2stain_amd/ops.py b/stain2stain_amd/ops.py
--- a/stain2stain_amd/ops.py
+++ b/stain2stain_amd/ops.py
@@ -251,10 +251,33 @@
 @_timed("conv3x3_mfma", _conv_flops)
 def conv3x3(x0: torch.Tensor, x1: Optional[torch.Tensor], w_packed: torch.Tensor, bias: Optional[torch.Tensor],
             cout: int, *, want_stats: bool = False, scale: Optional[torch.Tensor] = None,
-            shift: Optional[torch.Tensor] = None, relu: bool = False, out: Optional[torch.Tensor] = None):
+            shift: Optional[torch.Tensor] = None, relu: bool = False, out: Optional[torch.Tensor] = None,
+            bn_sums: Optional[Tuple[torch.Tensor, torch.Tensor]] = None):
     B, H, W, c0 = x0.shape
     dt = _dt(x0)
     p0, ld0 = _nhwc(x0)
+    if bn_sums is not None:
+        raw, st = bn_sums
+        if raw.shape != (B, H, W, cout) or raw.dtype != x0.dtype or st.shape != (4, cout) or st.dtype != torch.float32:
+            raise RuntimeError("stain2stain_amd: conv3x3 bn_sums operands do not match the output")
+        plain = x1 is None and bias is None and scale is None and shift is None and not relu and not want_stats
+        praw, ldraw = _nhwc(raw)
+        ldy = cout if out is None else _nhwc(out)[1]
+        nb = _L().s2s_conv3x3_bnsum_rows(dt, B, H, W, cout, c0, ld0, ldy, ldraw) if plain else 0
+        _native.check(min(nb, 0), "conv3x3_bnsum_rows")
+        if nb > 0:
+            if w_packed.dtype != x0.dtype or w_packed.numel() != _L().s2s_pack_conv3x3_fwd_elems(cout, c0):
+                raise RuntimeError("stain2stain_amd: packed weight does not match (cout, cin, dtype)")
+            if out is None:
+                out = torch.empty((B, H, W, cout), dtype=x0.dtype, device=x0.device)
+            elif out.shape != (B, H, W, cout) or out.dtype != x0.dtype:
+                raise RuntimeError("stain2stain_amd: conv3x3 output buffer mismatch")
+            part = torch.empty((2, cout, nb), dtype=torch.float32, device=x0.device)
+            rc = _L().s2s_conv3x3_nhwc_bns(dt, p0, ld0, c0, _ptr(w_packed), _nhwc(out)[0], ldy, _f32(part), nb, praw, ldraw,
+                                           st[2].data_ptr(), st[3].data_ptr(), st[0].data_ptr(), st[1].data_ptr(),
+                                           B, H, W, cout, _stream())
+            _native.check(rc, "conv3x3_bns")
+            return out, part
     p1, ld1, c1 = 0, 8, 0
     if x1 is not None:
         if x1.shape[:3] != x0.shape[:3] or x1.dtype != x0.dtype:
@@ -289,8 +312,15 @@
 
 def conv3x3_plan(dtype: torch.dtype, B: int, H: int, W: int, c0: int, c1: int, cout: int, *, ld0: Optional[int] = None,
                  ld1: Optional[int] = None, ldy: Optional[int] = None, bias: bool = False, affine: bool = False,
-                 stats: bool = False, stat_rows: int = -1, kwork: bool = False) -> dict:
+                 stats: bool = False, stat_rows: int = -1, kwork: bool = False, bn_sums: bool = False) -> dict:
     dt = BF16 if dtype == torch.bfloat16 else F32
+    if bn_sums:
+        out = (ctypes.c_int * (len(CONV3X3_PLAN_FIELDS) + 1))()
+        rc = _L().s2s_conv3x3_plan_bns(dt, B, H, W, cout, c0, c1, c0 if ld0 is None else ld0,
+                                       max(c1, 8) if ld1 is None else ld1, cout if ldy is None else ldy, int(bias),
+                                       int(affine), 1, stat_rows, int(kwork), 1, ctypes.cast(out, ctypes.c_void_p))
+        _native.check(rc, "conv3x3_plan")
+        return dict(zip(CONV3X3_PLAN_FIELDS + ("bn_sums",), (int(v) for v in out)))
     out = (ctypes.c_int * len(CONV3X3_PLAN_FIELDS))()
     rc = _L().s2s_conv3x3_plan(dt, B, H, W, cout, c0, c1, c0 if ld0 is None else ld0, max(c1, 8) if ld1 is None else ld1,
                                cout if ldy is None else ldy, int(bias), int(affine), int(stats),
@@ -578,7 +608,7 @@
 def bn_relu_bwd(g1: Optional[torch.Tensor], gp: Optional[torch.Tensor], x: torch.Tensor,
                 stats: torch.Tensor, gamma: torch.Tensor, dgamma: torch.Tensor, dbeta: torch.Tensor,
                 dbias_conv: Optional[torch.Tensor], accumulate: bool = False, exchange=None,
-                count_total: Optional[int] = None) -> torch.Tensor:
+                count_total: Optional[int] = None, presummed: Optional[torch.Tensor] = None) -> torch.Tensor:
     B, H, W, C = x.shape
     px, ldx = _nhwc(x)
     p1, ld1 = (0, 8) if g1 is None else _nhwc(g1)
@@ -586,6 +616,17 @@
     dx = torch.empty((B, H, W, C), dtype=x.dtype, device=x.device)
     nb = _L().s2s_bn_bwd_blocks(B, H, W, C)
     work = torch.empty((4 * nb * C + 2 * C,), dtype=torch.float32, device=x.device)
+    if presummed is not None:
+        if g1 is None or gp is not None or exchange is not None:
+            raise RuntimeError("stain2stain_amd: presummed BatchNorm backward takes one plain gradient and no exchange")
+        if presummed.dim() != 3 or presummed.shape[:2] != (2, C):
+            raise RuntimeError("stain2stain_amd: presummed partial sums are not [2, C, rows]")
+        rc = _L().s2s_bn_relu_bwd_presummed(_dt(x), p1, ld1, _f32(presummed), presummed.shape[2], stats[2].data_ptr(),
+                                            stats[3].data_ptr(), px, ldx, stats[0].data_ptr(), stats[1].data_ptr(),
+                                            _f32(gamma), _f32(dgamma), _f32(dbeta), _f32(dbias_conv), int(accumulate),
+                                            dx.data_ptr(), C, _f32(work), B, H, W, C, _stream())
+        _native.check(rc, "bn_relu_bwd_presummed")
+        return dx
     if exchange is not None:
         for phase in (1, 2):
             rc = _L().s2s_bn_relu_bwd_phase(_dt(x), p1, ld1, p2, ld2, stats[2].data_ptr(), stats[3].data_ptr(), px, ldx,
diff --git a/stain2stain_amd/trainer.py b/stain2stain_amd/trainer.py
--- a/stain2stain_amd/trainer.py
+++ b/stain2stain_amd/trainer.py
@@ -89,6 +89,7 @@
         self.overlap_wgrad = True
         self.fuse_tail = True
         self.lazy_up = True
+        self.dgrad_bn_sums = True
         self.graph = graph
         self._graph_step = CapturedStep()
         self._ema = None
@@ -145,10 +146,11 @@
         self._group = 0
         with engine.side_scope(self._side if self.overlap_wgrad else None):
             dbott, dskips, _ = engine.decoder_backward(dec, dctx, None, self.grads_dec, g_head=g_head,
-                                                       on_group_done=self._group_done)
+                                                       on_group_done=self._group_done, bn_sums=self.dgrad_bn_sums)
             L = len(feats) - 1
             dfeats = [dskips[L - 1 - l] for l in range(L)] + [dbott]
-            engine.encoder_backward(enc._blocks, ectx, dfeats, self.grads_enc, on_group_done=self._group_done)
+            engine.encoder_backward(enc._blocks, ectx, dfeats, self.grads_enc, on_group_done=self._group_done,
+                                    bn_sums=self.dgrad_bn_sums)
         return loss, dctx.v
 
     def _group_done(self) -> None:
```

New measurement: 2357 (median of 6 runs). Within noise of the previous version (+0.3%).
